# turpaultn/DCASE2019_task4

Measured on AMD Instinct MI355X. Metric: 10-s clips/sec mean-teacher train step (64-mel x 628), higher is better.
Workload: dtype f32

## Files before the change

dcase2019_task4_amd/csrc/common.h:

```cpp
#pragma once
#include <hip/hip_runtime.h>
#include <stdint.h>
#include <stddef.h>
#include "../../include/dcase_sed.h"

typedef __attribute__((ext_vector_type(16))) float f32x16;
typedef __attribute__((ext_vector_type(4))) float f32x4;

#define SED_C 64
#define SED_HID 64
#define SED_WAVE 64

void sed_set_error(const char* fmt, ...);
#define SED_CHECK_ARG(cond, msg)                                   \
    do {                                                           \
        if (!(cond)) {                                             \
            sed_set_error("%s:%d: %s", __FILE__, __LINE__, msg);   \
            return SED_ERR_BAD_ARG;                                \
        }                                                          \
    } while (0)
#define SED_CHECK_HIP(expr)                                                                 \
    do {                                                                                    \
        hipError_t _e = (expr);                                                             \
        if (_e != hipSuccess) {                                                             \
            sed_set_error("%s:%d: %s -> %s", __FILE__, __LINE__, #expr, hipGetErrorString(_e)); \
            return SED_ERR_LAUNCH;                                                          \
        }                                                                                   \
    } while (0)
#define SED_CHECK_LAUNCH() SED_CHECK_HIP(hipGetLastError())
struct SedAttrOnce {
    bool done[64] = {};
    bool need() {
        int d = 0;
        if (hipGetDevice(&d) != hipSuccess || d < 0 || d >= 64) return true;
        if (done[d]) return false;
        done[d] = true;
        return true;
    }
};
#define SED_TRY(expr)               \
    do {                            \
        int _s = (expr);            \
        if (_s != SED_OK) return _s; \
    } while (0)

struct Geo {
    int B, T, F, C, H, NC, L;
    int mode;
    bool f16;
    bool generic;
    int H1, W1;
    int H2, W2;
    int T3;
    float p, eps, mom;
};
static inline Geo make_geo(const sed_dims* d) {
    Geo g;
    g.B = d->B; g.T = d->T; g.F = d->F; g.C = d->C; g.H = d->H; g.NC = d->nclass; g.L = d->n_layers_rnn;
    g.f16 = d->dtype == SED_DTYPE_F16;
    g.mode = g.f16 ? SED_DTYPE_BF16 : d->dtype;
    g.generic = !(d->C == 64 && d->H == 64 && d->dtype == SED_DTYPE_F32);
    g.H1 = g.T / 2; g.W1 = g.F / 4;
    g.H2 = g.H1 / 2; g.W2 = g.W1 / 4;
    g.T3 = g.H2 / 2;
    g.p = d->p_drop; g.eps = d->bn_eps; g.mom = d->bn_momentum;
    return g;
}
int sed_validate_dims(const sed_dims* d);

struct ParamOff {
    int64_t conv_w[3], conv_b[3], bn_g[3], bn_b[3], glu_w[3], glu_b[3];
    int64_t w_ih[2][2], w_hh[2][2], b_ih[2][2], b_hh[2][2];
    int64_t dense_w, dense_b, soft_w, soft_b;
    int64_t total;
    int count;
};
ParamOff make_param_off(const Geo& g, int64_t* offsets_out );

struct CtxLayout {
    size_t acc0;
    size_t mom0, wz0, wl0, bn0;
    size_t mompart;
    size_t wpkT1, wpkT2;
    size_t p0;
    size_t wpk1, y1, stat1, bn1, p1;
    size_t wpk2, y2, stat2, bn2, p2;
    size_t gates[2], out[2];
    size_t logits_s, strong_sv, weak_sv, den_sv;
    size_t mask0, mask1, mask2;
    size_t total;
};
CtxLayout make_ctx_layout(const Geo& g);

struct WsLayout {
    size_t d_out, dgi[2], dgh[2], hprev[2], d_in, heads_part;
    size_t dz2, dp1, dz1, dp0, dp2;
    size_t bwd_acc;
    size_t bnb, gluacc1, gluacc2, coef[3], wg_part, de0, gemm_part;
    size_t total;
    int wgrad_blocks;
};
WsLayout make_ws_layout(const Geo& g);
#define SED_WGRAD_MAX_BLOCKS 256
#ifndef SED_GRU_SPLITK
#define SED_GRU_SPLITK 16
#endif
#define SED_GLUACC_N 4296
#define SED_WINO_OFF (9 * 4096)

__device__ __forceinline__ float wave_sum(float v) {
#pragma unroll
    for (int o = 32; o > 0; o >>= 1) v += __shfl_xor(v, o);
    return v;
}
__device__ __forceinline__ float wave_max(float v) {
#pragma unroll
    for (int o = 32; o > 0; o >>= 1) v = fmaxf(v, __shfl_xor(v, o));
    return v;
}
__device__ __forceinline__ void lds_barrier() { asm volatile("s_waitcnt lgkmcnt(0)\n\ts_barrier" ::: "memory"); }
__device__ __forceinline__ float rcp_fast(float x) { return __builtin_amdgcn_rcpf(x); }
__device__ __forceinline__ float sigmoidf_fast(float x) { return rcp_fast(1.0f + __expf(-x)); }
#define SED_NEG_LOG2E (-1.4426950408889634f)
__device__ __forceinline__ float sigmoid_from_scaled(float e) { return rcp_fast(1.0f + __builtin_amdgcn_exp2f(e)); }
struct TileWalk { int first, end, step; };
__device__ __forceinline__ TileWalk xcd_walk(int n_tiles) {
    const int w = blockIdx.x, g = (int)gridDim.x;
#ifndef SED_NO_XCD_ORDER
    if ((g & 7) == 0) {
        const int chunk = (n_tiles + 7) >> 3, lo = (w & 7) * chunk, hi = lo + chunk < n_tiles ? lo + chunk : n_tiles;
        return {lo + (w >> 3), hi, g >> 3};
    }
#endif
    return {w, n_tiles, g};
}
extern int g_sed_debug;

__device__ __forceinline__ f32x16 mfma32(float a, float b, f32x16 c) {
    return __builtin_amdgcn_mfma_f32_32x32x2f32(a, b, c, 0, 0, 0);
}
__device__ __forceinline__ int mfma32_row(int r, int lane) { return (r & 3) + 8 * (r >> 2) + 4 * (lane >> 5); }


#ifdef SED_TS
#define SED_TS_DEFINE(tag)                                                                                          \
    static __device__ unsigned long long g_ts[1024 * 16];                                                           \
    extern "C" int sed_debug_ts_##tag(unsigned long long* out, int n) {                                             \
        return (int)hipMemcpyFromSymbol(out, HIP_SYMBOL(g_ts), sizeof(unsigned long long) * (n < 1024 * 16 ? n : 1024 * 16)); \
    }
#define TS(k) do { if (threadIdx.x == 0 && blockIdx.x < 1024 && blockIdx.y == 0) g_ts[blockIdx.x * 16 + (k)] = wall_clock64(); } while (0)
#define TSC(k) do { if (threadIdx.x == 0 && blockIdx.x < 1024 && blockIdx.y == 0) g_ts[blockIdx.x * 16 + (k)] = clock64(); } while (0)
#else
#define SED_TS_DEFINE(tag)
#define TS(k) do { } while (0)
#define TSC(k) do { } while (0)
#endif
```

dcase2019_task4_amd/csrc/conv.hip:

```cpp
#include <type_traits>
#include "common.h"
#include "kernels.h"
SED_TS_DEFINE(conv)

template <int TW>
struct ConvCfg {
    static constexpr int TH = 128 / TW;
    static constexpr int HW = TW + 2;
    static constexpr int HH = TH + 2;
    static constexpr int PS = 65;
    static constexpr int RS = HW * PS + (((TW - HW * PS) % 32) + 32) % 32;
    static constexpr int HALO_FLOATS = HH * RS;
    static constexpr int W_FLOATS = 64 * 64;
    static constexpr size_t LDS_BYTES = (size_t)(HALO_FLOATS + 2 * W_FLOATS) * 4;
};

__global__ __launch_bounds__(256) void k_conv_pack(ConvPackArgs a) { conv_pack_body(a, blockIdx.x * 256 + threadIdx.x); }

template <int TW, int MODE, int NS>
__global__ __launch_bounds__(256) void k_conv3x3(const float* __restrict__ in0, const float* __restrict__ in1,
                                                  const float* __restrict__ coef, const float* __restrict__ wpk,
                                                  const float* __restrict__ bias, float* __restrict__ out,
                                                  double* __restrict__ stat, int B, int H, int tiles_per_clip) {
    using Cfg = ConvCfg<TW>;
    constexpr int TH = Cfg::TH, HW = Cfg::HW, HH = Cfg::HH, PS = Cfg::PS, RS = Cfg::RS;
    extern __shared__ __attribute__((aligned(16))) float smem[];
    float* halo = smem;
    float* Ws = smem + Cfg::HALO_FLOATS;
    const int tid = threadIdx.x, lane = tid & 63, wv = tid >> 6;
    const int n = lane & 31, kh = lane >> 5;
    const int b = blockIdx.x / tiles_per_clip, y0 = (blockIdx.x % tiles_per_clip) * TH;
    const int W = TW;
    const int nh = (NS == 2) ? blockIdx.y : 0;

    for (int f = tid; f < HH * HW * 16; f += 256) {
        const int pix = f >> 4, c4 = (f & 15) * 4;
        const int hy = pix / HW, hx = pix % HW;
        const int iy = y0 - 1 + hy, ix = hx - 1;
        float4 v = make_float4(0.f, 0.f, 0.f, 0.f);
        if (iy >= 0 && iy < H && ix >= 0 && ix < W) {
            const size_t g = (((size_t)b * H + iy) * W + ix) * 64 + c4;
            v = *(const float4*)(in0 + g);
            if (MODE == 1) {
                const float4 yv = *(const float4*)(in1 + g);
                const float4 ca = *(const float4*)(coef + c4);
                const float4 cb = *(const float4*)(coef + 64 + c4);
                const float4 cc = *(const float4*)(coef + 128 + c4);
                v.x = ca.x * v.x + cb.x * yv.x + cc.x;
                v.y = ca.y * v.y + cb.y * yv.y + cc.y;
                v.z = ca.z * v.z + cb.z * yv.z + cc.z;
                v.w = ca.w * v.w + cb.w * yv.w + cc.w;
            }
        }
        float* dst = halo + hy * RS + hx * PS + c4;
        dst[0] = v.x; dst[1] = v.y; dst[2] = v.z; dst[3] = v.w;
    }
#pragma unroll
    for (int it = 0; it < 4; ++it) {
        const int f = tid + 256 * it;
        *(float4*)(Ws + f * 4) = *(const float4*)(wpk + f * 4);
    }
    __syncthreads();

    const int m = 32 * wv + n;
    const int ty = m / TW, tx = m % TW;
    const float* Ab = halo + (ty + 1) * RS + (tx + 1) * PS + kh;
    f32x16 acc0, acc1;
#pragma unroll
    for (int r = 0; r < 16; ++r) { acc0[r] = 0.f; acc1[r] = 0.f; }

    for (int tap = 0; tap < 9; ++tap) {
        float4 pre[4];
        if (tap < 8) {
#pragma unroll
            for (int it = 0; it < 4; ++it) pre[it] = *(const float4*)(wpk + (tap + 1) * 4096 + (tid + 256 * it) * 4);
        }
        const int dy = tap / 3 - 1, dx = tap % 3 - 1;
        const float* A = Ab + dy * RS + dx * PS;
        const float* Bw = Ws + (tap & 1) * 4096 + kh * 64 + n + 32 * nh;
#pragma unroll
        for (int s = 0; s < 32; ++s) {
            const float a = A[2 * s];
            const float b0 = Bw[2 * s * 64];
            acc0 = mfma32(a, b0, acc0);
            if (NS == 1) {
                const float b1 = Bw[2 * s * 64 + 32];
                acc1 = mfma32(a, b1, acc1);
            }
        }
        if (tap < 8) {
            float* Wn = Ws + ((tap + 1) & 1) * 4096;
#pragma unroll
            for (int it = 0; it < 4; ++it) *(float4*)(Wn + (tid + 256 * it) * 4) = pre[it];
        }
        lds_barrier();
    }

    float s1[2] = {0.f, 0.f}, s2[2] = {0.f, 0.f};
    const float bia0 = (MODE == 0) ? bias[32 * nh + n] : 0.f, bia1 = (MODE == 0 && NS == 1) ? bias[32 + n] : 0.f;
#pragma unroll
    for (int r = 0; r < 16; ++r) {
        const int mm = 32 * wv + mfma32_row(r, lane);
        const int yy = y0 + mm / TW, xx = mm % TW;
        if (yy < H) {
            const size_t g = (((size_t)b * H + yy) * W + xx) * 64;
            const float v0 = acc0[r] + bia0, v1 = acc1[r] + bia1;
            out[g + 32 * nh + n] = v0;
            if (NS == 1) out[g + 32 + n] = v1;
            if (MODE == 0) { s1[0] += v0; s2[0] += v0 * v0; s1[1] += v1; s2[1] += v1 * v1; }
        }
    }
    if (MODE == 0 && stat != nullptr) {
        float* red = smem;
#pragma unroll
        for (int h = 0; h < 2; ++h) {
            float a = s1[h] + __shfl_xor(s1[h], 32);
            float q = s2[h] + __shfl_xor(s2[h], 32);
            if (kh == 0) { red[(wv * 2 + 0) * 64 + 32 * h + n] = a; red[(wv * 2 + 1) * 64 + 32 * h + n] = q; }
        }
        __syncthreads();
        if (tid < 128) {
            const int which = tid >> 6, c = tid & 63;
            double v = 0;
#pragma unroll
            for (int w2 = 0; w2 < 4; ++w2) v += (double)red[(w2 * 2 + which) * 64 + c];
            if (NS == 1) atomicAdd(&stat[which * 64 + c], v);
            else if (c < 32) atomicAdd(&stat[which * 64 + 32 * nh + c], v);
        }
    }
}


typedef float f32x4_t __attribute__((ext_vector_type(4)));
struct Ws16 {
    static constexpr int TH = 8, TW = 16, HW = 18, HH = 10, PS = 66, RS = HW * PS;
    static constexpr int HALO_FLOATS = HH * RS;
    static constexpr size_t LDS_BYTES = (size_t)2 * HALO_FLOATS * 4;
};
struct Ws16x2 {
    static constexpr int NLD = (Ws16::HH * Ws16::HW * 16 + 511) / 512;
};
template <int MODE>
__global__ __launch_bounds__(512, 1) void k_conv16_ws2(const float* __restrict__ in0, const float* __restrict__ in1,
                                                       const float* __restrict__ coef, const float* __restrict__ wpk,
                                                       const float* __restrict__ bias, float* __restrict__ out,
                                                       double* __restrict__ stat, int H, int tiles_per_clip, int n_tiles) {
    using C = Ws16;
    constexpr int NLD = Ws16x2::NLD;
    extern __shared__ __attribute__((aligned(16))) float smem[];
    const int tid = threadIdx.x, lane = tid & 63, wave = tid >> 6;
    const int cg = wave & 3, rh = wave >> 2;
    const int p16 = lane & 15, kq = lane >> 4;
    float st1 = 0.f, st2 = 0.f;
    constexpr int NH = (MODE == 1) ? NLD / 2 : NLD;
    f32x4_t pre0[NH], pre1[MODE == 1 ? NH : 1];
// ... 717 lines not shown
            Vd[(4 * i2 + 3) * 64] = T[i2][1] - T[i2][3];
        }
    };
    auto transform_m = [&](int y0, int ks, int slot, float* Ms) {
        float dy[4];
#pragma unroll
        for (int q = 0; q < 4; ++q) {
            const float v = fmaf(ca, dzr[slot][q], fmaf(cb, yr[slot][q], cc));
            dy[q] = v * ((y0 + 2 * (C::br_ks(ks) + cg_br) + (q >> 1) < H) ? 1.f : 0.f);
        }
        const float R[4][2] = {{dy[0], dy[1]}, {dy[0] + dy[2], dy[1] + dy[3]}, {dy[0] - dy[2], dy[1] - dy[3]}, {-dy[2], -dy[3]}};
        float* Md = Ms + cg * C::SM + 4 * (lane & 15) + (lane >> 4);
#pragma unroll
        for (int i2 = 0; i2 < 4; ++i2) {
            Md[(4 * i2 + 0) * 64] = R[i2][0];
            Md[(4 * i2 + 1) * 64] = R[i2][0] + R[i2][1];
            Md[(4 * i2 + 2) * 64] = R[i2][0] - R[i2][1];
            Md[(4 * i2 + 3) * 64] = -R[i2][1];
        }
    };
    auto mma = [&](const float* Vs, const float* Ms) {
        const float* Ab = Ms + kq * C::SM + 4 * i16 + 256 * (1 + ph);
        const float* Bb = Vs + kq * C::SV + 16 * cg + i16 + 256 * (1 + ph);
        const int xo = ph ? 256 : -256;
#pragma unroll
        for (int p8 = 0; p8 < 8; ++p8) {
            const int po = (p8 < 4 ? xo : 0) + (p8 & 3) * 64;
            const f32x4_t a4 = *(const f32x4_t*)(Ab + po);
            const float bv = Bb[po];
#pragma unroll
            for (int m = 0; m < 4; ++m) acc[p8][m] = __builtin_amdgcn_mfma_f32_16x16x4f32(a4[m], bv, acc[p8][m], 0, 0, 0);
        }
    };
    const TileWalk walk = xcd_walk(n_tiles);
    int tile = walk.first;
    TS(0);
    int it_ts = 0;
    int tb = tile / tiles_per_clip, ty0 = (tile % tiles_per_clip) * C::TH;
    if (tile < walk.end) {
        f32x4_t first[NITEMS];
#pragma unroll
        for (int hy = 0; hy < NITEMS; ++hy) load_row(tb, ty0, hy, first[hy]);
        if (ph) { load_dy(tb, ty0, 0, 0); load_dy(tb, ty0, 1, 1); }
#pragma unroll
        for (int hy = 0; hy < NITEMS; ++hy) store_row(smem, ty0, hy, first[hy]);
    }
    __syncthreads();
    if (tile < walk.end) {
        if (ph == 0) transform_v(smem, 0, ops);
        else transform_m(ty0, 0, 0, ops + 4 * C::SV);
    }
    __syncthreads();
    TS(1);
#pragma unroll
    for (int p8 = 0; p8 < 8; ++p8)
#pragma unroll
        for (int m = 0; m < 4; ++m) acc[p8][m] = (f32x4_t){0.f, 0.f, 0.f, 0.f};
    int cur = 0;
    for (; tile < walk.end; tile += walk.step) {
        const int nxt = (tile + walk.step < walk.end) ? tile + walk.step : tile;
        const int nb_ = nxt / tiles_per_clip, ny0 = (nxt % tiles_per_clip) * C::TH;
        const float* halo = smem + cur * C::HALO_FLOATS;
        float* halo_nxt = smem + (cur ^ 1) * C::HALO_FLOATS;
        constexpr int NKS = C::NKS, NPIECE = (NITEMS + NH - 1) / NH;
#pragma unroll
        for (int ks = 0; ks < NKS; ++ks) {
            f32x4_t held[NH];
            if (ks >= 1 && ks <= NPIECE) {
#pragma unroll
                for (int k2 = 0; k2 < NH; ++k2) held[k2] = pre[k2];
            }
            if (ks < NPIECE) {
#pragma unroll
                for (int k2 = 0; k2 < NH; ++k2)
                    if (NH * ks + k2 < NITEMS) load_row(nb_, ny0, NH * ks + k2, pre[k2]);
            }
            float* nb = ops + ((ks + 1) & 1) * C::OPS_FLOATS;
            const float* cb2 = ops + (ks & 1) * C::OPS_FLOATS;
            if (ph == 0) {
                if (ks < NKS - 1) transform_v(halo, ks + 1, nb); else transform_v(halo_nxt, 0, nb);
            }
            if (it_ts == 0 && ks == 2) { TS(3); TSW4(7); }
            mma(cb2, cb2 + 4 * C::SV);
            if (it_ts == 0 && ks == 2) { TS(4); TSW4(8); }
            if (ph == 1) {
                if (ks < NKS - 2) load_dy(tb, ty0, ks + 2, ks & 1); else load_dy(nb_, ny0, ks - (NKS - 2), ks & 1);
                if (ks < NKS - 1) transform_m(ty0, ks + 1, (ks + 1) & 1, nb + 4 * C::SV); else transform_m(ny0, 0, 0, nb + 4 * C::SV);
            }
            if (ks >= 1 && ks <= NPIECE) {
#pragma unroll
                for (int k2 = 0; k2 < NH; ++k2)
                    if (NH * (ks - 1) + k2 < NITEMS) store_row(halo_nxt, ny0, NH * (ks - 1) + k2, held[k2]);
            }
            if (it_ts == 0 && ks == 2) { TS(5); TSW4(9); }
            lds_barrier();
            if (it_ts == 0 && ks == 1) { TS(2); TSW4(6); }
        }
        if (it_ts == 0) TS(10);
        ++it_ts;
        cur ^= 1;
        tb = nb_; ty0 = ny0;
    }
    TS(11);
    __syncthreads();
    float* ob = smem;
#pragma unroll
    for (int round = 0; round < 2; ++round) {
        if (ph == round) {
#pragma unroll
            for (int m = 0; m < 4; ++m)
#pragma unroll
                for (int r = 0; r < 4; ++r) {
                    float wx[3], wy[3];
                    {
                        const float u0 = acc[0][m][r], u1 = acc[1][m][r], u2 = acc[2][m][r], u3 = acc[3][m][r];
                        const float h = 0.5f * (u1 + u2);
                        wx[0] = u0 + h; wx[1] = 0.5f * (u1 - u2); wx[2] = h + u3;
                    }
                    {
                        const float u0 = acc[4][m][r], u1 = acc[5][m][r], u2 = acc[6][m][r], u3 = acc[7][m][r];
                        const float h = 0.5f * (u1 + u2);
                        wy[0] = 0.5f * (u0 + h); wy[1] = 0.25f * (u1 - u2); wy[2] = 0.5f * (h + u3);
                    }
                    float* o = ob + (16 * m + 4 * kq + r) * C::OUT_STRIDE + 16 * cg + i16;
#pragma unroll
                    for (int b2 = 0; b2 < 3; ++b2) {
                        const float g0 = ph ? wy[b2] : wx[b2] + wy[b2];
                        const float g1 = ph ? -wy[b2] : wy[b2];
                        const float g2 = ph ? wx[b2] + wy[b2] : wy[b2];
                        if (round == 0) {
                            o[(0 + b2) * 64 * C::OUT_STRIDE] = g0; o[(3 + b2) * 64 * C::OUT_STRIDE] = g1; o[(6 + b2) * 64 * C::OUT_STRIDE] = g2;
                        } else {
                            o[(0 + b2) * 64 * C::OUT_STRIDE] += g0; o[(3 + b2) * 64 * C::OUT_STRIDE] += g1; o[(6 + b2) * 64 * C::OUT_STRIDE] += g2;
                        }
                    }
                }
        }
        __syncthreads();
    }
    TS(12);
    float* dst = part + (size_t)blockIdx.x * 9 * 4096;
    for (int idx = tid; idx < 9 * 64 * 16; idx += 512) {
        const int row = idx >> 4, c4 = (idx & 15) * 4;
        *(f32x4_t*)(dst + row * 64 + c4) = *(const f32x4_t*)(ob + row * C::OUT_STRIDE + c4);
    }
    TS(13);
}

#define WG4_RUNS 64
struct Wg4Os {
    static constexpr int SV4 = 4 * 64 + 16, SM4 = 4 * 64, OPS4 = 4 * SV4 + 4 * SM4;
    static constexpr size_t LDS_BYTES = (size_t)(2 * WgW<4>::HALO_FLOATS + 2 * OPS4) * 4;
};
__global__ __launch_bounds__(512, 1) void k_wgrad4_os(const float* __restrict__ dz, const float* __restrict__ yin,
                                                       const float* __restrict__ coef, const float* __restrict__ xin,
                                                       float* __restrict__ part, int H, int tiles_per_clip, int n_tiles, int n_runs,
                                                       BnBwdPrepArgs prep) {
    using C = WgW<4>;
    constexpr int SV4 = Wg4Os::SV4, SM4 = Wg4Os::SM4, OPS4 = Wg4Os::OPS4;
    extern __shared__ __attribute__((aligned(16))) float smem[];
    float* ops = smem + 2 * C::HALO_FLOATS;
    const int tid = threadIdx.x, lane = tid & 63, wave = __builtin_amdgcn_readfirstlane(tid >> 6);
    const int cg = wave & 3, jh = wave >> 2;
    const int w = blockIdx.x, run = (w & 7) + 8 * (w >> 5), ti = (w >> 3) & 3;
    const int cg_br = cg >> 1, cg_bc = cg & 1;
    const int i16 = lane & 15, kq = lane >> 4;
    const int vp = (ti == 0) ? 0 : (ti == 2 ? 2 : 1), vq = (ti == 3) ? 3 : (ti == 2 ? 1 : 2);
    const float sv = (ti == 1) ? 1.f : -1.f;
    const float ma = (ti == 3) ? 0.f : 1.f, mb = (ti == 0) ? 0.f : (ti == 1 ? 1.f : -1.f);
    float ca, cb, cc;
    if (prep.acc != nullptr) bn_bwd_coef(prep, lane, ca, cb, cc);
    else { ca = coef[lane]; cb = coef[64 + lane]; cc = coef[128 + lane]; }
    constexpr int NITEMS = C::NITEMS, NH = 2;
    f32x4_t pre[NH];
    const int td = tid < C::RPI * C::RW ? tid : tid - 480;
    const int r_in = td / C::RW, hx = (td % C::RW) >> 4, c4 = (td & 15) * 4;
    const int ixc = hx - 1 < 0 ? 0 : (hx - 1 > C::TW - 1 ? C::TW - 1 : hx - 1);
    const uint32_t goff4 = (uint32_t)(ixc * 64 + c4) * 4u;
    const bool colok = hx >= 1 && hx <= C::TW;
    const int lds_off = hx * C::PS + c4;
    auto load_row = [&](int b, int y0, int it, f32x4_t& d0) {
        const int hy = it * C::RPI + r_in < C::HH ? it * C::RPI + r_in : C::HH - 1;
        const int iy = y0 - 1 + hy;
        const int iyc = iy < 0 ? 0 : (iy > H - 1 ? H - 1 : iy);
        const float* rowp = xin + (size_t)(b * H + iyc) * (C::TW * 64);
        d0 = *(const f32x4_t*)((const char*)rowp + goff4);
    };
    auto store_row = [&](float* halo, int y0, int it, const f32x4_t& s0) {
        const int hy = it * C::RPI + r_in < C::HH ? it * C::RPI + r_in : C::HH - 1;
        const int iy = y0 - 1 + hy;
        const bool ok = colok && iy >= 0 && iy < H;
        const f32x4_t z4 = {0.f, 0.f, 0.f, 0.f};
        const f32x4_t v = ok ? s0 : z4;
        float* d = halo + hy * C::RS + lds_off;
        *(float2*)d = make_float2(v[0], v[1]);
        *(float2*)(d + 2) = make_float2(v[2], v[3]);
    };
    f32x4_t acc[2][4];
    float dzr[2][4], yr[2][4];
    const int img_bytes = (n_tiles / tiles_per_clip) * H * (C::TW * 64 * 4);
    const auto rs_dz = __builtin_amdgcn_make_buffer_rsrc((void*)dz, (short)0, img_bytes, 0x00020000);
    const auto rs_y = __builtin_amdgcn_make_buffer_rsrc((void*)yin, (short)0, img_bytes, 0x00020000);
    const int lane4 = 4 * lane;
    auto load_dy = [&](int b, int y0, int ks, int slot) {
#pragma unroll
        for (int q = 0; q < 4; ++q) {
            const int yy = y0 + 2 * (C::br_ks(ks) + cg_br) + (q >> 1), xx = 2 * (C::bc_ks(ks) + cg_bc) + (q & 1);
            const int yc = yy < H ? yy : H - 1;
            const int so = ((b * H + yc) * C::TW + xx) * 256;
            dzr[slot][q] = __uint_as_float(__builtin_amdgcn_raw_buffer_load_b32(rs_dz, lane4, so, 0));
            yr[slot][q] = __uint_as_float(__builtin_amdgcn_raw_buffer_load_b32(rs_y, lane4, so, 0));
        }
    };
    auto transform_v = [&](const float* halo, int ks, float* Vs) {
        const float* P = halo + (2 * cg_br) * C::RS + (2 * cg_bc) * C::PS + lane + ((2 * C::br_ks(ks)) * C::RS + (2 * C::bc_ks(ks)) * C::PS);
        const float* Pp = P + vp * C::RS;
        const float* Pq = P + vq * C::RS;
        float T[4];
#pragma unroll
        for (int b2 = 0; b2 < 4; ++b2) T[b2] = fmaf(sv, Pq[b2 * C::PS], Pp[b2 * C::PS]);
        float* Vd = Vs + cg * SV4 + lane;
        Vd[0] = T[0] - T[2]; Vd[64] = T[1] + T[2]; Vd[128] = T[2] - T[1]; Vd[192] = T[1] - T[3];
    };
    auto transform_m = [&](int y0, int ks, int slot, float* Ms) {
        float dy[4];
#pragma unroll
        for (int q = 0; q < 4; ++q) {
            const float v = fmaf(ca, dzr[slot][q], fmaf(cb, yr[slot][q], cc));
            dy[q] = v * ((y0 + 2 * (C::br_ks(ks) + cg_br) + (q >> 1) < H) ? 1.f : 0.f);
        }
        const float R0 = ma * dy[0] + mb * dy[2], R1 = ma * dy[1] + mb * dy[3];
        float* Md = Ms + cg * SM4 + 4 * (lane & 15) + (lane >> 4);
        Md[0] = R0; Md[64] = R0 + R1; Md[128] = R0 - R1; Md[192] = -R1;
    };
    auto mma = [&](const float* Vs, const float* Ms) {
        const float* Ab = Ms + kq * SM4 + 4 * i16 + 128 * jh;
        const float* Bb = Vs + kq * SV4 + 16 * cg + i16 + 128 * jh;
#pragma unroll
        for (int j2 = 0; j2 < 2; ++j2) {
            const f32x4_t a4 = *(const f32x4_t*)(Ab + 64 * j2);
            const float bv = Bb[64 * j2];
#pragma unroll
            for (int m = 0; m < 4; ++m) acc[j2][m] = __builtin_amdgcn_mfma_f32_16x16x4f32(a4[m], bv, acc[j2][m], 0, 0, 0);
        }
    };
    int tile = run;
    int tb = tile / tiles_per_clip, ty0 = (tile % tiles_per_clip) * C::TH;
    if (tile < n_tiles) {
        f32x4_t first[NITEMS];
#pragma unroll
        for (int hy = 0; hy < NITEMS; ++hy) load_row(tb, ty0, hy, first[hy]);
        if (jh) { load_dy(tb, ty0, 0, 0); load_dy(tb, ty0, 1, 1); }
#pragma unroll
        for (int hy = 0; hy < NITEMS; ++hy) store_row(smem, ty0, hy, first[hy]);
    }
    __syncthreads();
    if (tile < n_tiles) {
        if (jh == 0) transform_v(smem, 0, ops);
        else transform_m(ty0, 0, 0, ops + 4 * SV4);
    }
    __syncthreads();
#pragma unroll
    for (int j2 = 0; j2 < 2; ++j2)
#pragma unroll
        for (int m = 0; m < 4; ++m) acc[j2][m] = (f32x4_t){0.f, 0.f, 0.f, 0.f};
    int cur = 0;
    for (; tile < n_tiles; tile += n_runs) {
        const int nxt = (tile + n_runs < n_tiles) ? tile + n_runs : tile;
        const int nb_ = nxt / tiles_per_clip, ny0 = (nxt % tiles_per_clip) * C::TH;
        const float* halo = smem + cur * C::HALO_FLOATS;
        float* halo_nxt = smem + (cur ^ 1) * C::HALO_FLOATS;
        constexpr int NKS = C::NKS, NPIECE = (NITEMS + NH - 1) / NH;
#pragma unroll
        for (int ks = 0; ks < NKS; ++ks) {
            f32x4_t held[NH];
            if (ks >= 1 && ks <= NPIECE) {
#pragma unroll
                for (int k2 = 0; k2 < NH; ++k2) held[k2] = pre[k2];
            }
            if (ks < NPIECE) {
#pragma unroll
                for (int k2 = 0; k2 < NH; ++k2)
                    if (NH * ks + k2 < NITEMS) load_row(nb_, ny0, NH * ks + k2, pre[k2]);
            }
            float* nb = ops + ((ks + 1) & 1) * OPS4;
            const float* cb2 = ops + (ks & 1) * OPS4;
            if (jh == 0) {
                if (ks < NKS - 1) transform_v(halo, ks + 1, nb); else transform_v(halo_nxt, 0, nb);
            }
            mma(cb2, cb2 + 4 * SV4);
            if (jh == 1) {
                if (ks < NKS - 2) load_dy(tb, ty0, ks + 2, ks & 1); else load_dy(nb_, ny0, ks - (NKS - 2), ks & 1);
                if (ks < NKS - 1) transform_m(ty0, ks + 1, (ks + 1) & 1, nb + 4 * SV4); else transform_m(ny0, 0, 0, nb + 4 * SV4);
            }
            if (ks >= 1 && ks <= NPIECE) {
#pragma unroll
                for (int k2 = 0; k2 < NH; ++k2)
                    if (NH * (ks - 1) + k2 < NITEMS) store_row(halo_nxt, ny0, NH * (ks - 1) + k2, held[k2]);
            }
            lds_barrier();
        }
        cur ^= 1;
        tb = nb_; ty0 = ny0;
    }
    __syncthreads();
    float* xb = smem + (size_t)cg * 48 * 64 + lane;
    if (jh == 1) {
#pragma unroll
        for (int m = 0; m < 4; ++m)
#pragma unroll
            for (int r = 0; r < 4; ++r) {
                const float u2 = acc[0][m][r], u3 = acc[1][m][r];
                xb[((m * 4 + r) * 3 + 0) * 64] = 0.5f * u2;
                xb[((m * 4 + r) * 3 + 1) * 64] = -0.5f * u2;
                xb[((m * 4 + r) * 3 + 2) * 64] = 0.5f * u2 + u3;
            }
    }
    __syncthreads();
    if (jh == 0) {
        float* dst = part + ((size_t)run * 4 + ti) * 3 * 4096 + 16 * cg + i16;
#pragma unroll
        for (int m = 0; m < 4; ++m)
#pragma unroll
            for (int r = 0; r < 4; ++r) {
                const float u0 = acc[0][m][r], u1 = acc[1][m][r];
                const int co = 16 * m + 4 * kq + r;
                dst[(0 * 64 + co) * 64] = (u0 + 0.5f * u1) + xb[((m * 4 + r) * 3 + 0) * 64];
                dst[(1 * 64 + co) * 64] = 0.5f * u1 + xb[((m * 4 + r) * 3 + 1) * 64];
                dst[(2 * 64 + co) * 64] = 0.5f * u1 + xb[((m * 4 + r) * 3 + 2) * 64];
            }
    }
}

__global__ __launch_bounds__(256) void k_wgrad4_os_reduce(const float* __restrict__ part, int n_runs, float* __restrict__ g_w) {
    __shared__ __attribute__((aligned(16))) float red[16][12][64];
    __shared__ float S[12][64];
    const int c = threadIdx.x & 15, grp = threadIdx.x >> 4;
    const f32x4_t* P = (const f32x4_t*)part + blockIdx.x * 16 + c;
    f32x4_t s[12];
#pragma unroll
    for (int pl = 0; pl < 12; ++pl) s[pl] = (f32x4_t){0.f, 0.f, 0.f, 0.f};
    for (int r = grp; r < n_runs; r += 16) {
#pragma unroll
        for (int pl = 0; pl < 12; ++pl) s[pl] += P[((size_t)r * 12 + pl) * 1024];
    }
#pragma unroll
    for (int pl = 0; pl < 12; ++pl) *(f32x4_t*)&red[grp][pl][4 * c] = s[pl];
    __syncthreads();
    for (int o = threadIdx.x; o < 12 * 64; o += 256) {
        const int pl = o >> 6, e = o & 63;
        float v = 0.f;
#pragma unroll
        for (int g2 = 0; g2 < 16; ++g2) v += red[g2][pl][e];
        S[pl][e] = v;
    }
    __syncthreads();
    for (int o = threadIdx.x; o < 64 * 9; o += 256) {
        const int e = o / 9, tap = o % 9, a = tap / 3, b = tap % 3;
        const float w0 = S[0 + b][e], w1 = S[3 + b][e], w2 = S[6 + b][e], w3 = S[9 + b][e];
        const float v = a == 0 ? w0 + 0.5f * (w1 + w2) : (a == 1 ? 0.5f * (w1 - w2) : 0.5f * (w1 + w2) + w3);
        g_w[(size_t)blockIdx.x * 64 * 9 + o] = v;
    }
}

__global__ __launch_bounds__(256) void k_wgrad_reduce(const float* __restrict__ part, int n_blocks, float* __restrict__ g_w) {
    __shared__ __attribute__((aligned(16))) float red[16][64];
    const int c = threadIdx.x & 15, grp = threadIdx.x >> 4;
    const int i4 = blockIdx.x * 16 + c;
    const f32x4_t* P = (const f32x4_t*)part + i4;
    constexpr int SLAB4 = 9 * 4096 / 4;
    f32x4_t s[8];
#pragma unroll
    for (int u = 0; u < 8; ++u) s[u] = (f32x4_t){0.f, 0.f, 0.f, 0.f};
    int k = grp;
    for (; k + 16 * 7 < n_blocks; k += 16 * 8) {
#pragma unroll
        for (int u = 0; u < 8; ++u) s[u] += P[(size_t)(k + 16 * u) * SLAB4];
    }
    for (; k < n_blocks; k += 16) s[0] += P[(size_t)k * SLAB4];
    *(f32x4_t*)&red[grp][4 * c] = ((s[0] + s[1]) + (s[2] + s[3])) + ((s[4] + s[5]) + (s[6] + s[7]));
    __syncthreads();
    if (threadIdx.x < 64) {
        float v = 0.f;
#pragma unroll
        for (int g2 = 0; g2 < 16; ++g2) v += red[g2][threadIdx.x];
        const int i = blockIdx.x * 64 + threadIdx.x;
        const int tap = i / 4096, co = (i / 64) % 64, ci = i % 64;
        g_w[(co * 64 + ci) * 9 + tap] = v;
    }
}

int launch_conv_pack(const ConvPackArgs& a, hipStream_t st) {
    k_conv_pack<<<SED_PACK_BLOCKS, 256, 0, st>>>(a);
    SED_CHECK_LAUNCH();
    return SED_OK;
}

template <int TW, int MODE, int NS>
static int conv_launch_t(const float* in0, const float* in1, const float* coef, const float* wpk, const float* bias,
                         float* out, double* stat, int B, int H, hipStream_t st) {
    using Cfg = ConvCfg<TW>;
    static thread_local SedAttrOnce attr_done;
    if (attr_done.need()) {
        SED_CHECK_HIP(hipFuncSetAttribute((const void*)k_conv3x3<TW, MODE, NS>, hipFuncAttributeMaxDynamicSharedMemorySize,
                                          (int)Cfg::LDS_BYTES));
    }
    const int tpc = (H + Cfg::TH - 1) / Cfg::TH;
    k_conv3x3<TW, MODE, NS><<<dim3(B * tpc, NS), 256, Cfg::LDS_BYTES, st>>>(in0, in1, coef, wpk, bias, out, stat, B, H, tpc);
    SED_CHECK_LAUNCH();
    return SED_OK;
}

#ifdef SED_AB
#define SED_AB_FLAGS(mask) (g_sed_debug & (mask))
#else
#define SED_AB_FLAGS(mask) 0
#endif
extern "C" int sed_build_flags(void) {
#ifdef SED_AB
    return 1;
#else
    return 0;
#endif
}

int launch_conv_fwd(const float* in, const float* wpk, const float* bias, float* y, double* stat, int zero_stat, int B,
                    int H, int W, hipStream_t st) {
    if (stat && zero_stat) SED_CHECK_HIP(hipMemsetAsync(stat, 0, 128 * sizeof(double), st));
#ifdef SED_AB
    const bool direct = (g_sed_debug & (2 | 64)) != 0;
    if (direct && W == 16) return (g_sed_debug & 2) ? conv_launch_t<16, 0, 1>(in, nullptr, nullptr, wpk, bias, y, stat, B, H, st)
                                                    : conv16_ws_launch<0>(in, nullptr, nullptr, wpk, bias, y, stat, B, H, st);
    if (direct && W == 4) return conv_launch_t<4, 0, 2>(in, nullptr, nullptr, wpk, bias, y, stat, B, H, st);
#endif
    if (W == 16) return conv_wino_launch<16, 0>(in, nullptr, nullptr, wpk, bias, y, stat, B, H, nullptr, st);
    if (W == 4) return conv_wino_launch<4, 0>(in, nullptr, nullptr, wpk, bias, y, stat, B, H, nullptr, st);
    sed_set_error("conv: unsupported width %d", W);
    return SED_ERR_UNSUPPORTED;
}

int launch_conv_dgrad(const float* dz, const float* yin, const float* coef, const float* wpkT, float* dx, int B, int H,
                      int W, const BnBwdPrepArgs* prep, hipStream_t st) {
#ifdef SED_AB
    const bool direct = (g_sed_debug & (4 | 64)) != 0;
    SED_CHECK_ARG(!(direct && prep), "conv dgrad: in-kernel BatchNorm-backward coefficients need the Winograd kernel");
    if (direct && W == 16) return (g_sed_debug & 4) ? conv_launch_t<16, 1, 1>(dz, yin, coef, wpkT, nullptr, dx, nullptr, B, H, st)
                                                    : conv16_ws_launch<1>(dz, yin, coef, wpkT, nullptr, dx, nullptr, B, H, st);
    if (direct && W == 4) return conv_launch_t<4, 1, 2>(dz, yin, coef, wpkT, nullptr, dx, nullptr, B, H, st);
#endif
    if (W == 16) return conv_wino_launch<16, 1>(dz, yin, coef, wpkT, nullptr, dx, nullptr, B, H, prep, st);
    if (W == 4) return conv_wino_launch<4, 1>(dz, yin, coef, wpkT, nullptr, dx, nullptr, B, H, prep, st);
    sed_set_error("conv dgrad: unsupported width %d", W);
    return SED_ERR_UNSUPPORTED;
}

template <int TW, int TS>
static int wgrad_launch_t(const float* dz, const float* yin, const float* coef, const float* xin, float* part,
                          int n_blocks, float* g_w, int B, int H, const BnBwdPrepArgs* prep, hipStream_t st) {
    BnBwdPrepArgs pa = {};
    if (prep) pa = *prep;
#ifdef SED_AB
    using Cfg = WgCfg<TW>;
    static thread_local SedAttrOnce attr_done;
    if (attr_done.need()) {
        SED_CHECK_HIP(hipFuncSetAttribute((const void*)k_conv3x3_wgrad<TW, TS>, hipFuncAttributeMaxDynamicSharedMemorySize,
                                          (int)Cfg::LDS_BYTES));
    }
    const int tpc = (H + Cfg::TH - 1) / Cfg::TH, nt = B * tpc;
    int nb = nt < n_blocks ? nt : n_blocks;
#else
    int nb = 0;
#endif
    if (TW == 4 && !SED_AB_FLAGS(8 | 128) && !(g_sed_debug & 67108864)) {
        using CW = WgW<4>;
        static thread_local SedAttrOnce attro;
        if (attro.need()) {
            SED_CHECK_HIP(hipFuncSetAttribute((const void*)k_wgrad4_os, hipFuncAttributeMaxDynamicSharedMemorySize, (int)Wg4Os::LDS_BYTES));
        }
        SED_CHECK_ARG((size_t)B * H * TW * 64 < ((size_t)1 << 31), "wgrad: image too large for 32-bit offsets");
        const int tpcw = (H + CW::TH - 1) / CW::TH, ntw = B * tpcw;
        int n_runs = (ntw + 7) & ~7;
        if (n_runs > WG4_RUNS) n_runs = WG4_RUNS;
        SED_CHECK_ARG(n_runs * 4 <= n_blocks * 3, "wgrad: partial buffer too small");
        k_wgrad4_os<<<4 * n_runs, 512, Wg4Os::LDS_BYTES, st>>>(dz, yin, coef, xin, part, H, tpcw, ntw, n_runs, pa);
        SED_CHECK_LAUNCH();
        k_wgrad4_os_reduce<<<4096 / 64, 256, 0, st>>>(part, n_runs, g_w);
        SED_CHECK_LAUNCH();
        return SED_OK;
    }
    if (!SED_AB_FLAGS(8 | 128)) {
        using CW = WgW<TW>;
        static thread_local SedAttrOnce attrw;
        if (attrw.need()) {
            SED_CHECK_HIP(hipFuncSetAttribute((const void*)k_wgrad_wino<TW>, hipFuncAttributeMaxDynamicSharedMemorySize, (int)CW::LDS_BYTES));
        }
        SED_CHECK_ARG((size_t)B * H * TW * 64 < ((size_t)1 << 31), "wgrad: image too large for 32-bit offsets");
        const int tpcw = (H + CW::TH - 1) / CW::TH, ntw = B * tpcw;
        nb = ntw < n_blocks ? ntw : n_blocks;
        k_wgrad_wino<TW><<<nb, 512, CW::LDS_BYTES, st>>>(dz, yin, coef, xin, part, H, tpcw, ntw, pa);
    }
#ifdef SED_AB
    else if (TW == 16 && TS == 1 && !(g_sed_debug & 8)) {
        static thread_local SedAttrOnce attr16;
        if (attr16.need()) {
            SED_CHECK_HIP(hipFuncSetAttribute((const void*)k_wgrad16_db, hipFuncAttributeMaxDynamicSharedMemorySize, (int)Wg16::LDS_BYTES));
        }
        k_wgrad16_db<<<nb, 256, Wg16::LDS_BYTES, st>>>(dz, yin, coef, xin, part, H, tpc, nt);
    } else {
        k_conv3x3_wgrad<TW, TS><<<dim3(nb, TS), 256, Cfg::LDS_BYTES, st>>>(dz, yin, coef, xin, part, B, H, tpc, nt, pa);
    }
#endif
    SED_CHECK_LAUNCH();
    k_wgrad_reduce<<<9 * 4096 / 64, 256, 0, st>>>(part, nb, g_w);
    SED_CHECK_LAUNCH();
    return SED_OK;
}

int launch_conv_wgrad(const float* dz, const float* yin, const float* coef, const float* xin, float* part, int n_blocks,
                      float* g_w, int B, int H, int W, const BnBwdPrepArgs* prep, hipStream_t st) {
    SED_CHECK_ARG(!(prep && W == 16 && SED_AB_FLAGS(8 | 128)), "conv wgrad: in-kernel BatchNorm-backward coefficients need the default kernels");
    if (W == 16) return wgrad_launch_t<16, 1>(dz, yin, coef, xin, part, n_blocks, g_w, B, H, prep, st);
    if (W == 4) return wgrad_launch_t<4, 3>(dz, yin, coef, xin, part, n_blocks, g_w, B, H, prep, st);
    sed_set_error("conv wgrad: unsupported width %d", W);
    return SED_ERR_UNSUPPORTED;
}
```

dcase2019_task4_amd/csrc/crnn.hip:

```cpp
#include <stdarg.h>
#include <map>
#include <mutex>
#include <utility>
#include <stdio.h>
#include <string.h>
#include "common.h"
#include "kernels.h"
#include "gkernels.h"

static thread_local char g_err[512] = "";
void sed_set_error(const char* fmt, ...) {
    va_list ap;
    va_start(ap, fmt);
    vsnprintf(g_err, sizeof(g_err), fmt, ap);
    va_end(ap);
}
extern "C" const char* sed_last_error(void) { return g_err; }
extern "C" int sed_version(void) { return 100; }
int g_sed_debug = 0;
extern "C" int sed_debug_set(int flags) { const int old = g_sed_debug; g_sed_debug = flags; return old; }

int sed_validate_dims(const sed_dims* d) {
    SED_CHECK_ARG(d != nullptr, "null dims");
    if (d->F != 64 || (d->C != 64 && d->C != 128) || (d->H != 64 && d->H != 256) ||
        (d->dtype != SED_DTYPE_F32 && d->dtype != SED_DTYPE_BF16 && d->dtype != SED_DTYPE_BF16X3 && d->dtype != SED_DTYPE_F16)) {
        sed_set_error("supported: F = 64, C in {64, 128}, H in {64, 256}, dtype in {f32, bf16, bf16x3, f16} (got F=%d C=%d H=%d dtype=%d)",
                      d->F, d->C, d->H, d->dtype);
        return SED_ERR_UNSUPPORTED;
    }
    SED_CHECK_ARG(d->B >= 1 && d->T >= 16, "need B >= 1 and T >= 16");
    SED_CHECK_ARG(d->nclass >= 1 && d->nclass <= 16, "nclass must be in [1, 16]");
    SED_CHECK_ARG(d->n_layers_rnn == 1 || d->n_layers_rnn == 2, "n_layers_rnn must be 1 or 2");
    SED_CHECK_ARG(d->p_drop >= 0.f && d->p_drop < 1.f, "p_drop must be in [0, 1)");
    SED_CHECK_ARG((int64_t)d->B * d->T * d->F * d->C < (1ll << 31), "batch too large for 32-bit pixel indices");
    return SED_OK;
}

ParamOff make_param_off(const Geo& g, int64_t* out) {
    ParamOff P;
    int64_t o = 0;
    int k = 0;
    auto put = [&](int64_t& field, int64_t n) {
        field = o;
        if (out) out[k] = o;
        ++k;
        o += n;
    };
    for (int i = 0; i < 3; ++i) {
        const int cin = (i == 0) ? 1 : g.C;
        put(P.conv_w[i], (int64_t)g.C * cin * 9);
        put(P.conv_b[i], g.C);
        put(P.bn_g[i], g.C);
        put(P.bn_b[i], g.C);
        put(P.glu_w[i], (int64_t)g.C * g.C);
        put(P.glu_b[i], g.C);
    }
    for (int l = 0; l < g.L; ++l) {
        const int nin = (l == 0) ? g.C : 2 * g.H;
        for (int dir = 0; dir < 2; ++dir) {
            put(P.w_ih[l][dir], (int64_t)3 * g.H * nin);
            put(P.w_hh[l][dir], (int64_t)3 * g.H * g.H);
            put(P.b_ih[l][dir], 3 * g.H);
            put(P.b_hh[l][dir], 3 * g.H);
        }
    }
    put(P.dense_w, (int64_t)g.NC * 2 * g.H);
    put(P.dense_b, g.NC);
    put(P.soft_w, (int64_t)g.NC * 2 * g.H);
    put(P.soft_b, g.NC);
    P.total = o;
    P.count = k;
    if (out) out[k] = o;
    return P;
}

static inline size_t al(size_t x) { return (x + 255) & ~(size_t)255; }

CtxLayout make_ctx_layout(const Geo& g) {
    CtxLayout L;
    size_t o = 0;
    auto put = [&](size_t& f, size_t bytes) { f = o; o = al(o + bytes); };
    const size_t n0 = (size_t)g.B * g.H1 * g.W1 * 64, n1 = (size_t)g.B * g.H2 * g.W2 * 64, n2 = (size_t)g.B * g.T3 * 64;
    put(L.acc0, 320 * sizeof(double));
    L.mom0 = L.acc0; L.stat1 = L.acc0 + 64 * sizeof(double); L.stat2 = L.acc0 + 192 * sizeof(double);
    put(L.wz0, 64 * 12 * 4); put(L.wl0, 64 * 12 * 4); put(L.bn0, 256 * 4);
    put(L.mompart, (size_t)x_moments_parts(g) * 54 * sizeof(double));
    put(L.p0, n0 * 4);
    put(L.wpk1, (9 + 16) * 4096 * 4); put(L.wpkT1, (9 + 16) * 4096 * 4); put(L.y1, n0 * 4); put(L.bn1, 256 * 4); put(L.p1, n1 * 4);
    put(L.wpk2, (9 + 16) * 4096 * 4); put(L.wpkT2, (9 + 16) * 4096 * 4); put(L.y2, n1 * 4); put(L.bn2, 256 * 4); put(L.p2, n2 * 4);
    const size_t bt = (size_t)g.B * g.T3;
    for (int l = 0; l < 2; ++l) {
        put(L.gates[l], bt * 512 * 4); put(L.out[l], bt * 128 * 4);
    }
    put(L.logits_s, bt * g.NC * 4); put(L.strong_sv, bt * g.NC * 4);
    put(L.weak_sv, (size_t)g.B * g.NC * 4); put(L.den_sv, (size_t)g.B * g.NC * 4);
    auto mask_bytes = [](size_t Q) { return ((Q + 3) / 4) * 2 * 64 * sizeof(uint16_t); };
    put(L.mask0, mask_bytes((size_t)g.B * g.H1 * g.W1)); put(L.mask1, mask_bytes((size_t)g.B * g.H2 * g.W2));
    put(L.mask2, mask_bytes((size_t)g.B * g.T3));
    L.total = o;
    return L;
}

WsLayout make_ws_layout(const Geo& g) {
    WsLayout W;
    size_t o = 0;
    auto put = [&](size_t& f, size_t bytes) { f = o; o = al(o + bytes); };
    const size_t n0 = (size_t)g.B * g.H1 * g.W1 * 64, n1 = (size_t)g.B * g.H2 * g.W2 * 64, bt = (size_t)g.B * g.T3;
    put(W.d_out, bt * 128 * 4);
    for (int l = 0; l < 2; ++l) { put(W.dgi[l], bt * 384 * 4); put(W.dgh[l], bt * 384 * 4); put(W.hprev[l], bt * 128 * 4); }
    put(W.d_in, 2 * bt * 128 * 4); put(W.heads_part, (size_t)g.B * 2 * (g.NC * 128 + g.NC) * 4);
    put(W.dp2, 2 * bt * 64 * 4); put(W.dz2, n1 * 4); put(W.dp1, n1 * 4); put(W.dz1, n0 * 4); put(W.dp0, n0 * 4);
    put(W.bnb, 256 * sizeof(double)); W.coef[0] = 0; put(W.coef[1], 192 * 4); put(W.coef[2], 192 * 4);
    put(W.bwd_acc, (2 * SED_GLUACC_N + 2 * 64 * 10) * sizeof(double));
    W.gluacc1 = W.bwd_acc; W.gluacc2 = W.bwd_acc + SED_GLUACC_N * sizeof(double); W.de0 = W.bwd_acc + 2 * SED_GLUACC_N * sizeof(double);
    W.wgrad_blocks = SED_WGRAD_MAX_BLOCKS;
    put(W.wg_part, (size_t)W.wgrad_blocks * 9 * 4096 * 4);
    put(W.gemm_part, gemm_part_floats(4, SED_GRU_SPLITK, 192, 129) * 4);
    W.total = o;
    return W;
}

extern "C" int sed_param_count(const sed_dims* d) {
    if (sed_validate_dims(d) != SED_OK) return -1;
    const Geo g = make_geo(d);
    return make_param_off(g, nullptr).count;
}
extern "C" int sed_param_layout(const sed_dims* d, int64_t* offsets) {
    SED_TRY(sed_validate_dims(d));
    SED_CHECK_ARG(offsets != nullptr, "null offsets");
    const Geo g = make_geo(d);
    make_param_off(g, offsets);
    return SED_OK;
}
extern "C" size_t sed_crnn_ctx_bytes(const sed_dims* d) {
    if (sed_validate_dims(d) != SED_OK) return 0;
    const Geo g = make_geo(d);
    return g.generic ? gen_ctx_bytes(g) : make_ctx_layout(g).total;
}
extern "C" size_t sed_crnn_bwd_ws_bytes(const sed_dims* d) {
    if (sed_validate_dims(d) != SED_OK) return 0;
    const Geo g = make_geo(d);
    return g.generic ? gen_ws_bytes(g) : make_ws_layout(g).total;
}

extern "C" int sed_crnn_buffers_init(const sed_dims* d, void* ctx, size_t ctx_bytes, void* ws, size_t ws_bytes, void* stream) {
    SED_TRY(sed_validate_dims(d));
    const Geo g = make_geo(d);
    if (g.generic) return gen_buffers_init(g, ctx, ctx_bytes, ws, ws_bytes, (hipStream_t)stream);
    return SED_OK;
}

extern "C" int sed_crnn_ctx_view(const sed_dims* d, const char* name, size_t* offset, size_t* bytes) {
    SED_TRY(sed_validate_dims(d));
    SED_CHECK_ARG(name && offset && bytes, "null argument");
    const Geo g = make_geo(d);
    if (g.generic) return gen_ctx_view(g, name, offset, bytes);
    const CtxLayout L = make_ctx_layout(g);
    const size_t n0 = (size_t)g.B * g.H1 * g.W1 * 64 * 4, n1 = (size_t)g.B * g.H2 * g.W2 * 64 * 4, bt = (size_t)g.B * g.T3;
    struct { const char* n; size_t o, b; } tab[] = {
        {"mom0", L.mom0, 64 * 8}, {"wz0", L.wz0, 64 * 12 * 4}, {"wl0", L.wl0, 64 * 12 * 4}, {"bn0", L.bn0, 1024},
        {"p0", L.p0, n0}, {"y1", L.y1, n0}, {"stat1", L.stat1, 1024}, {"bn1", L.bn1, 1024}, {"p1", L.p1, n1},
        {"y2", L.y2, n1}, {"stat2", L.stat2, 1024}, {"bn2", L.bn2, 1024}, {"p2", L.p2, bt * 64 * 4},
        {"gates0", L.gates[0], bt * 512 * 4}, {"gates1", L.gates[1], bt * 512 * 4},
        {"gru0", L.out[0], bt * 128 * 4}, {"gru1", L.out[1], bt * 128 * 4},
        {"logits_s", L.logits_s, bt * g.NC * 4}, {"den", L.den_sv, (size_t)g.B * g.NC * 4},
    };
    for (auto& t : tab)
        if (strcmp(t.n, name) == 0) { *offset = t.o; *bytes = t.b; return SED_OK; }
    sed_set_error("sed_crnn_ctx_view: unknown buffer '%s'", name);
    return SED_ERR_BAD_ARG;
}

struct SideStream {
    hipStream_t s = nullptr;
    hipEvent_t fork = nullptr, join = nullptr;
    hipStream_t s2 = nullptr;
    hipEvent_t join2 = nullptr;
    bool ok = false;
};
static std::mutex g_side_mu;
static std::map<std::pair<int, hipStream_t>, SideStream*> g_side;
struct ForkHook { void (*fn)(void*) = nullptr; void* user = nullptr; };
static std::map<std::pair<int, hipStream_t>, ForkHook> g_fork_hooks;
static SideStream& side_stream(hipStream_t caller) {
    static SideStream none;
    int dev = 0;
    if (hipGetDevice(&dev) != hipSuccess) return none;
    std::lock_guard<std::mutex> lk(g_side_mu);
    SideStream*& slot = g_side[std::make_pair(dev, caller)];
    if (slot == nullptr) {
        slot = new SideStream();
        if (hipStreamCreateWithFlags(&slot->s, hipStreamNonBlocking) == hipSuccess &&
            hipEventCreateWithFlags(&slot->fork, hipEventDisableTiming) == hipSuccess &&
            hipEventCreateWithFlags(&slot->join, hipEventDisableTiming) == hipSuccess &&
            hipStreamCreateWithFlags(&slot->s2, hipStreamNonBlocking) == hipSuccess &&
            hipEventCreateWithFlags(&slot->join2, hipEventDisableTiming) == hipSuccess)
            slot->ok = true;
    }
    return *slot;
}
extern "C" int sed_stream_prepare(void* stream) {
    SideStream& sd = side_stream((hipStream_t)stream);
    if (!sd.ok) {
        sed_set_error("sed_stream_prepare: could not create the helper stream / events");
        return SED_ERR_LAUNCH;
    }
    return SED_OK;
}
extern "C" int sed_stream_release(void* stream) {
    int dev = 0;
    SED_CHECK_HIP(hipGetDevice(&dev));
    SideStream* sd = nullptr;
    {
        std::lock_guard<std::mutex> lk(g_side_mu);
        const auto key = std::make_pair(dev, (hipStream_t)stream);
        auto it = g_side.find(key);
        if (it != g_side.end()) { sd = it->second; g_side.erase(it); }
        g_fork_hooks.erase(key);
    }
    if (sd == nullptr) return SED_OK;
    int rc = SED_OK;
    auto note = [&](hipError_t e) { if (e != hipSuccess && rc == SED_OK) { sed_set_error("sed_stream_release: %s", hipGetErrorString(e)); rc = SED_ERR_LAUNCH; } };
    if (sd->s) { note(hipStreamSynchronize(sd->s)); note(hipStreamDestroy(sd->s)); }
    if (sd->s2) { note(hipStreamSynchronize(sd->s2)); note(hipStreamDestroy(sd->s2)); }
    if (sd->fork) note(hipEventDestroy(sd->fork));
    if (sd->join) note(hipEventDestroy(sd->join));
    if (sd->join2) note(hipEventDestroy(sd->join2));
    delete sd;
    return rc;
}
extern "C" int sed_crnn_fork_callback(void* stream, void (*fn)(void*), void* user) {
    int dev = 0;
    SED_CHECK_HIP(hipGetDevice(&dev));
    std::lock_guard<std::mutex> lk(g_side_mu);
    const auto key = std::make_pair(dev, (hipStream_t)stream);
    if (fn == nullptr) { g_fork_hooks.erase(key); return SED_OK; }
    ForkHook& h = g_fork_hooks[key];
    h.fn = fn;
    h.user = user;
    return SED_OK;
}
int sed_fork_point(hipStream_t st) {
    int dev = 0;
    if (hipGetDevice(&dev) != hipSuccess) return SED_OK;
    ForkHook h;
    {
        std::lock_guard<std::mutex> lk(g_side_mu);
        auto it = g_fork_hooks.find(std::make_pair(dev, st));
        if (it == g_fork_hooks.end()) return SED_OK;
        h = it->second;
        g_fork_hooks.erase(it);
    }
    if (h.fn) h.fn(h.user);
    return SED_OK;
}
#define SIDE_FORK(main_st)                                          \
    do {                                                            \
        SED_CHECK_HIP(hipEventRecord(sd.fork, (main_st)));          \
        SED_CHECK_HIP(hipStreamWaitEvent(sd.s, sd.fork, 0));        \
    } while (0)
#define SIDE_JOIN(main_st)                                          \
    do {                                                            \
        SED_CHECK_HIP(hipEventRecord(sd.join, sd.s));               \
        SED_CHECK_HIP(hipStreamWaitEvent((main_st), sd.join, 0));   \
    } while (0)

#define CTXF(off) ((float*)((char*)ctx + (off)))
#define CTXD(off) ((double*)((char*)ctx + (off)))
#define WSF(off) ((float*)((char*)ws + (off)))
#define WSD(off) ((double*)((char*)ws + (off)))
#define CTXM(off) ((uint16_t*)((char*)ctx + (off)))

extern "C" int sed_crnn_forward(const sed_dims* d, const float* params, float* bn_running, int64_t* bn_tracked,
                                const float* x, int train, int update_bn, const uint64_t* seed_dev, void* ctx,
                                size_t ctx_bytes, float* strong, float* weak, void* stream) {
    SED_TRY(sed_validate_dims(d));
    SED_CHECK_ARG(params && bn_running && x && ctx, "sed_crnn_forward: null argument");
    const int mom_ready = (train & 4) ? 1 : 0;
    train &= 3;
    SED_CHECK_ARG((strong && weak) || (!strong && !weak && train), "sed_crnn_forward: strong and weak must both be given (or both NULL in train mode: heads deferred)");
    const Geo g = make_geo(d);
    const ParamOff P = make_param_off(g, nullptr);
    if (g.generic) {
        SED_CHECK_ARG(!(train && g.p > 0.f) || seed_dev, "sed_crnn_forward: dropout enabled but seed_dev is null");
        hipStream_t st0 = (hipStream_t)stream;
        SideStream& sd0 = side_stream(st0);
        return gen_forward(g, P, params, bn_running, bn_tracked, x, train | (mom_ready ? 4 : 0), update_bn, seed_dev, ctx, ctx_bytes, strong,
                           weak, st0, sd0.ok ? sd0.s : st0, sd0.fork, sd0.join);
    }
    const CtxLayout L = make_ctx_layout(g);
    if (ctx_bytes < L.total) {
        sed_set_error("sed_crnn_forward: ctx has %zu bytes, needs %zu", ctx_bytes, L.total);
        return SED_ERR_WORKSPACE;
    }
    const int use_drop = (train && g.p > 0.f) ? 1 : 0;
    SED_CHECK_ARG(!use_drop || seed_dev, "sed_crnn_forward: dropout enabled but seed_dev is null");
    hipStream_t st = (hipStream_t)stream;
    const int upd = (train && update_bn) ? 1 : 0;
    int64_t* trk[3] = {bn_tracked ? bn_tracked + 0 : nullptr, bn_tracked ? bn_tracked + 1 : nullptr,
                       bn_tracked ? bn_tracked + 2 : nullptr};

    const ConvPackArgs pack = {params + P.conv_w[1], params + P.conv_w[2], CTXF(L.wpk1), CTXF(L.wpk2),
                               train ? CTXF(L.wpkT1) : nullptr, train ? CTXF(L.wpkT2) : nullptr, CTXD(L.stat1), train ? 256 : 0};
    SED_TRY(launch_blk0_forward(g, x, params + P.conv_w[0], params + P.conv_b[0], params + P.bn_g[0], params + P.bn_b[0],
                                params + P.glu_w[0], params + P.glu_b[0], bn_running + 0, bn_running + 64, trk[0], train,
                                upd, seed_dev, CTXD(L.mom0), CTXD(L.mompart), CTXF(L.wz0), CTXF(L.wl0), CTXF(L.bn0), CTXF(L.p0),
                                use_drop ? CTXM(L.mask0) : nullptr, train ? &pack : nullptr, st, 0, nullptr, nullptr, mom_ready));
    if (!train) SED_TRY(launch_conv_pack(pack, st));
    const float* in = CTXF(L.p0);
    const size_t wpk[3] = {0, L.wpk1, L.wpk2}, yo[3] = {0, L.y1, L.y2}, so[3] = {0, L.stat1, L.stat2},
                 bo[3] = {0, L.bn1, L.bn2}, po[3] = {0, L.p1, L.p2}, mo[3] = {L.mask0, L.mask1, L.mask2};
    const int Hs[3] = {0, g.H1, g.H2}, Ws[3] = {0, g.W1, g.W2};
    for (int i = 1; i <= 2; ++i) {
        SED_TRY(launch_conv_fwd(in, CTXF(wpk[i]), params + P.conv_b[i], CTXF(yo[i]), train ? CTXD(so[i]) : nullptr, 0, g.B,
                                Hs[i], Ws[i], st));
        SED_TRY(launch_glu_pool_fwd(CTXF(yo[i]), CTXD(so[i]), (double)g.B * Hs[i] * Ws[i], params + P.bn_g[i], params + P.bn_b[i],
                                    bn_running + (2 * i) * 64, bn_running + (2 * i + 1) * 64, trk[i], train, upd, g.eps, g.mom,
                                    CTXF(bo[i]), params + P.glu_w[i], params + P.glu_b[i], CTXF(po[i]), g.B, Hs[i], Ws[i], i,
                                    use_drop, g.p, seed_dev, use_drop ? CTXM(mo[i]) : nullptr, st));
        in = CTXF(po[i]);
    }
    SED_TRY(sed_fork_point(st));
    int nin = 64;
    for (int l = 0; l < g.L; ++l) {
        SED_TRY(launch_gru_fwd(in, nin, params + P.w_ih[l][0], params + P.w_ih[l][1], params + P.b_ih[l][0], params + P.b_ih[l][1],
                               params + P.w_hh[l][0], params + P.w_hh[l][1], params + P.b_hh[l][0], params + P.b_hh[l][1],
                               CTXF(L.out[l]), train ? CTXF(L.gates[l]) : nullptr, g.B, g.T3, st));
        in = CTXF(L.out[l]);
        nin = 128;
    }
    if (strong == nullptr) return SED_OK;
    SED_TRY(launch_heads_fwd(in, params + P.dense_w, params + P.dense_b, params + P.soft_w, params + P.soft_b, strong, weak,
                             train ? CTXF(L.strong_sv) : nullptr, train ? CTXF(L.weak_sv) : nullptr, CTXF(L.logits_s),
                             CTXF(L.den_sv), g.B, g.T3, g.NC, use_drop, g.p, seed_dev, st));
    return SED_OK;
}

extern "C" int sed_crnn_moments(const sed_dims* d, const float* x, void* ctx, size_t ctx_bytes, void* stream) {
    SED_TRY(sed_validate_dims(d));
    SED_CHECK_ARG(x && ctx, "sed_crnn_moments: null argument");
    const Geo g = make_geo(d);
    double* mompart = nullptr;
    if (g.generic) {
        SED_TRY(gen_mompart(g, ctx, ctx_bytes, &mompart));
    } else {
        const CtxLayout L = make_ctx_layout(g);
        if (ctx_bytes < L.total) {
            sed_set_error("sed_crnn_moments: ctx has %zu bytes, needs %zu", ctx_bytes, L.total);
            return SED_ERR_WORKSPACE;
        }
        mompart = CTXD(L.mompart);
    }
    return launch_x_moments(g, x, mompart, nullptr, (hipStream_t)stream);
}

static int crnn_backward_impl(const sed_dims* d, const float* params, const float* x, const uint64_t* seed_dev,
                              void* ctx, size_t ctx_bytes, const float* d_strong, const float* d_weak, float* grads,
                              void* ws, size_t ws_bytes, int parts, void* stream, const HeadsLoss* hl,
                              const HeadsOut* ho = nullptr) {
    SED_TRY(sed_validate_dims(d));
    SED_CHECK_ARG(params && x && ctx && (hl || (d_strong && d_weak)) && grads && ws, "sed_crnn_backward: null argument");
    SED_CHECK_ARG(parts == 1 || parts == 2 || parts == 3 || parts == 5 || parts == 8,
                  "sed_crnn_backward: parts must be 1, 2, 3, 5 or 8");
    const Geo g = make_geo(d);
    const ParamOff P = make_param_off(g, nullptr);
    if (g.generic) {
        SED_CHECK_ARG(!(g.p > 0.f) || seed_dev, "sed_crnn_backward: dropout enabled but seed_dev is null");
        hipStream_t st0 = (hipStream_t)stream;
        SideStream& sd0 = side_stream(st0);
        return gen_backward(g, P, params, x, seed_dev, ctx, ctx_bytes, d_strong, d_weak, grads, ws, ws_bytes, parts, st0,
                            (sd0.ok && !(g_sed_debug & 1073741824)) ? sd0.s : st0, sd0.fork, sd0.join, (sd0.ok && (g_sed_debug & 2048)) ? sd0.s2 : nullptr, sd0.join2, hl, ho);
    }
    const CtxLayout L = make_ctx_layout(g);
    const WsLayout W = make_ws_layout(g);
    if (ctx_bytes < L.total || ws_bytes < W.total) {
        sed_set_error("sed_crnn_backward: ctx %zu/%zu bytes, ws %zu/%zu bytes", ctx_bytes, L.total, ws_bytes, W.total);
        return SED_ERR_WORKSPACE;
    }
    const int use_drop = (g.p > 0.f) ? 1 : 0;
    SED_CHECK_ARG(!use_drop || seed_dev, "sed_crnn_backward: dropout enabled but seed_dev is null");
    hipStream_t st = (hipStream_t)stream;
    const int BT = g.B * g.T3;
    SideStream& sd = side_stream(st);
    hipStream_t ss = (sd.ok && !(g_sed_debug & 1073741824)) ? sd.s : st;
    const bool defer_gru_w = (parts & 4) != 0;
    bool forked = false, forked2 = false;

    auto gru_weight_grads_layer = [&](int l, hipStream_t s2) -> int {
        const int nin = (l == 0) ? 64 : 128;
        const float* input = (l == 0) ? CTXF(L.p2) : CTXF(L.out[l - 1]);
        GemmBatch gb;
        gb.n_prob = 4; gb.splits = SED_GRU_SPLITK; gb.part = WSF(W.gemm_part); gb.part_floats = gemm_part_floats(4, SED_GRU_SPLITK, 192, 129); gb.part_stride = 0;
        for (int dir = 0; dir < 2; ++dir) {
            gb.p[2 * dir] = gemm_prob(WSF(W.dgi[l]) + dir * 192, 1, 384, input, nin, 1, grads + P.w_ih[l][dir], nin, 192, nin, BT);
            gb.p[2 * dir].Cones = grads + P.b_ih[l][dir];
            gb.p[2 * dir + 1] = gemm_prob(WSF(W.dgh[l]) + dir * 192, 1, 384, WSF(W.hprev[l]) + dir * 64, 128, 1,
                                          grads + P.w_hh[l][dir], 64, 192, 64, BT);
            gb.p[2 * dir + 1].Cones = grads + P.b_hh[l][dir];
        }
        return launch_gemm_batch(gb, s2);
    };
    auto gru_weight_grads = [&](hipStream_t s2) -> int {
        for (int l = g.L - 1; l >= 0; --l) SED_TRY(gru_weight_grads_layer(l, s2));
        return SED_OK;
    };
    const bool early_gru_w = parts == 3 && sd.ok && (g_sed_debug & 16384);

    const int head_cols = 2 * (g.NC * 128 + g.NC);
    const bool fuse = ho && hl && (parts & 1) && heads_fusable(64, g.T3) && !(g_sed_debug & 16777216) && !hl->d_strong_out && !hl->d_weak_out;
    auto heads_colsum = [&](hipStream_t s2) -> int {
        if (fuse) return launch_heads_fin(WSF(W.heads_part), grads + P.dense_w, g.B, g.T3, g.NC, head_cols, *hl, s2);
        return launch_heads_colsum(WSF(W.heads_part), grads + P.dense_w, g.B, g.NC, s2);
    };
    const bool defer_colsum = ((parts & 2) && sd.ok) || defer_gru_w;
    if (parts & 1) {
    const float* h_last = CTXF(L.out[g.L - 1]);
    if (ho && !fuse)
        SED_TRY(launch_heads_fwd(h_last, params + P.dense_w, params + P.dense_b, params + P.soft_w, params + P.soft_b, ho->strong, ho->weak,
                                 CTXF(L.strong_sv), CTXF(L.weak_sv), CTXF(L.logits_s), CTXF(L.den_sv), g.B, g.T3, g.NC, use_drop, g.p,
                                 seed_dev, st));
    if (!fuse)
    SED_TRY(launch_heads_bwd(h_last, params + P.dense_w, params + P.soft_w, CTXF(L.strong_sv), CTXF(L.weak_sv),
                             CTXF(L.logits_s), CTXF(L.den_sv), d_strong, d_weak, WSF(W.d_out), WSF(W.heads_part),
                             grads + P.dense_w, grads + P.dense_b, grads + P.soft_w, grads + P.soft_b, g.B, g.T3, g.NC,
                             use_drop, g.p, seed_dev, (parts & 2) ? WSD(W.bwd_acc) : nullptr, 2 * SED_GLUACC_N + 2 * 64 * 10,
                             defer_colsum ? 1 : 0, hl, st));
    const float* d_cur = WSF(W.d_out);
    const float* d_cur2 = nullptr;
    for (int l = g.L - 1; l >= 0; --l) {
        const int nin = (l == 0) ? 64 : 128;
        float* d_in = (l == 0) ? WSF(W.dp2) : WSF(W.d_in);
        if (fuse && l == g.L - 1) {
            HeadsFuse hf = {};
            hf.wd = params + P.dense_w; hf.strong = ho->strong; hf.weak = ho->weak; hf.part = WSF(W.heads_part);
            hf.NC = g.NC; hf.use_drop = use_drop; hf.p_drop = g.p; hf.seed = seed_dev;
            hf.zero = (parts & 2) ? WSD(W.bwd_acc) : nullptr; hf.n_zero = (parts & 2) ? 2 * SED_GLUACC_N + 2 * 64 * 10 : 0;
            hf.hl = *hl;
            SED_TRY(launch_gru_bwd_heads(CTXF(L.out[l]), CTXF(L.gates[l]), params + P.w_hh[l][0], params + P.w_hh[l][1],
                                         params + P.w_ih[l][0], params + P.w_ih[l][1], nin, WSF(W.dgi[l]), WSF(W.dgh[l]),
                                         WSF(W.hprev[l]), d_in, g.B, g.T3, hf, st));
            if (!defer_colsum) SED_TRY(heads_colsum(st));
            else if (defer_gru_w) SED_TRY(launch_heads_fin(WSF(W.heads_part), grads + P.dense_w, g.B, g.T3, g.NC, 0, *hl, st));
        } else
        SED_TRY(launch_gru_bwd(d_cur, d_cur2, CTXF(L.out[l]), CTXF(L.gates[l]), params + P.w_hh[l][0], params + P.w_hh[l][1],
                               params + P.w_ih[l][0], params + P.w_ih[l][1], nin, WSF(W.dgi[l]), WSF(W.dgh[l]),
                               WSF(W.hprev[l]), d_in, g.B, g.T3, st));
        d_cur = d_in;
        d_cur2 = d_in + (size_t)BT * nin;
        if (early_gru_w) {
            SIDE_FORK(st);
            forked = true;
            if (l == g.L - 1) SED_TRY(heads_colsum(ss));
            SED_TRY(gru_weight_grads_layer(l, ss));
        }
    }
    }
    if (parts == 1) SED_TRY(gru_weight_grads(st));
    if (parts == 8) {
        SED_TRY(launch_heads_colsum(WSF(W.heads_part), grads + P.dense_w, g.B, g.NC, st));
        SED_TRY(gru_weight_grads(st));
        return SED_OK;
    }
    if (!(parts & 2)) {
        if (forked) SIDE_JOIN(st);
        return SED_OK;
    }
    const size_t wpkT[3] = {0, L.wpkT1, L.wpkT2}, yo[3] = {0, L.y1, L.y2}, bo[3] = {0, L.bn1, L.bn2};
    const size_t pin[3] = {0, L.p0, L.p1}, gacc[3] = {0, W.gluacc1, W.gluacc2}, mo[3] = {L.mask0, L.mask1, L.mask2};
    const size_t dzo[3] = {0, W.dz1, W.dz2}, dpo[3] = {W.dp0, W.dp1, W.dp2};
    const int Hs[3] = {0, g.H1, g.H2}, Wd[3] = {0, g.W1, g.W2};
    if (!(parts & 1)) SED_CHECK_HIP(hipMemsetAsync(WSD(W.bwd_acc), 0, (2 * SED_GLUACC_N + 2 * 64 * 10) * sizeof(double), st));
#ifdef SED_AB
    const bool fuse_prep = (g_sed_debug & (4 | 8 | 64 | 128 | 512)) == 0;
#else
    const bool fuse_prep = (g_sed_debug & 512) == 0;
#endif
    BnBwdPrepArgs prep[3] = {};
    for (int i = 2; i >= 1; --i) {
        const BnBwdPrepArgs* pp = fuse_prep ? &prep[i] : nullptr;
        SED_TRY(launch_glu_pool_bwd(CTXF(yo[i]), CTXF(bo[i]), params + P.glu_w[i], params + P.glu_b[i], WSF(dpo[i]),
                                    i == 2 ? WSF(dpo[i]) + (size_t)BT * 64 : nullptr,
                                    WSF(dzo[i]), WSD(gacc[i]), 0, g.B, Hs[i], Wd[i], i, use_drop, g.p, CTXM(mo[i]),
                                    params + P.bn_g[i], WSF(W.coef[i]), grads + P.bn_g[i], grads + P.bn_b[i],
                                    grads + P.glu_w[i], grads + P.glu_b[i], grads + P.conv_b[i], fuse_prep ? &prep[i] : nullptr, st));
        if (i == 2) {
            if (sd.ok) SED_CHECK_HIP(hipEventRecord(sd.fork, st));
            SED_TRY(launch_conv_dgrad(WSF(dzo[i]), CTXF(yo[i]), WSF(W.coef[i]), CTXF(wpkT[i]), WSF(dpo[i - 1]), g.B, Hs[i], Wd[i], pp, st));
            if (sd.ok) { SED_CHECK_HIP(hipStreamWaitEvent(sd.s, sd.fork, 0)); forked = true; }
            SED_TRY(launch_conv_wgrad(WSF(dzo[i]), CTXF(yo[i]), WSF(W.coef[i]), CTXF(pin[i]), WSF(W.wg_part), W.wgrad_blocks,
                                      grads + P.conv_w[i], g.B, Hs[i], Wd[i], pp, ss));
            if (parts == 3 && !early_gru_w) {
                hipStream_t sg = ss;
                if (sd.ok && (g_sed_debug & 2048)) {
                    SED_CHECK_HIP(hipStreamWaitEvent(sd.s2, sd.fork, 0));
                    sg = sd.s2;
                    forked2 = true;
                }
                if (sd.ok) SED_TRY(heads_colsum(sg));
                SED_TRY(gru_weight_grads(sg));
            }
        } else {
            if (sd.ok) { SIDE_FORK(st); forked = true; }
            SED_TRY(launch_conv_dgrad(WSF(dzo[i]), CTXF(yo[i]), WSF(W.coef[i]), CTXF(wpkT[i]), WSF(dpo[i - 1]), g.B, Hs[i], Wd[i], pp, st));
            SED_TRY(launch_conv_wgrad(WSF(dzo[i]), CTXF(yo[i]), WSF(W.coef[i]), CTXF(pin[i]), WSF(W.wg_part), W.wgrad_blocks,
                                      grads + P.conv_w[i], g.B, Hs[i], Wd[i], pp, ss));
        }
    }
    SED_TRY(launch_blk0_backward(g, x, params + P.conv_w[0], params + P.conv_b[0], params + P.bn_g[0], params + P.bn_b[0],
                                 params + P.glu_w[0], CTXM(L.mask0), CTXD(L.mom0), CTXF(L.wz0), CTXF(L.wl0), CTXF(L.bn0),
                                 WSF(W.dp0), WSD(W.de0), 0, grads + P.conv_w[0], grads + P.conv_b[0], grads + P.bn_g[0],
                                 grads + P.bn_b[0], grads + P.glu_w[0], grads + P.glu_b[0], st));
    if (forked) SIDE_JOIN(st);
    if (forked2) {
        SED_CHECK_HIP(hipEventRecord(sd.join2, sd.s2));
        SED_CHECK_HIP(hipStreamWaitEvent(st, sd.join2, 0));
    }
    return SED_OK;
}

extern "C" int sed_crnn_backward(const sed_dims* d, const float* params, const float* x, const uint64_t* seed_dev,
                                 void* ctx, size_t ctx_bytes, const float* d_strong, const float* d_weak, float* grads,
                                 void* ws, size_t ws_bytes, int parts, void* stream) {
    return crnn_backward_impl(d, params, x, seed_dev, ctx, ctx_bytes, d_strong, d_weak, grads, ws, ws_bytes, parts, stream, nullptr);
}

extern "C" int sed_mt_loss_backward(const sed_dims* d, const float* params, const float* x, const uint64_t* seed_dev,
                                    void* ctx, size_t ctx_bytes, const float* strong_ema, const float* weak_ema,
                                    const float* target, int weak_lo, int weak_hi, int strong_lo, int strong_hi,
                                    sed_step_state* state_dev, int advance_state, float* losses, float* d_strong,
                                    float* d_weak, float* grads, void* ws, size_t ws_bytes, int parts, void* stream) {
    SED_CHECK_ARG(d && strong_ema && weak_ema && target && state_dev && losses, "sed_mt_loss_backward: null argument");
    SED_CHECK_ARG(parts == 1 || parts == 3 || parts == 5, "sed_mt_loss_backward: parts must include the heads (1, 3 or 5)");
    SED_CHECK_ARG(weak_lo >= 0 && weak_hi <= d->B && weak_lo <= weak_hi && strong_lo >= 0 && strong_hi <= d->B &&
                      strong_lo <= strong_hi, "sed_mt_loss_backward: bad mask range");
    HeadsLoss hl = {strong_ema, weak_ema, target, weak_lo, weak_hi, strong_lo, strong_hi, state_dev, losses, d_strong, d_weak,
                    advance_state ? state_dev : nullptr};
    return crnn_backward_impl(d, params, x, seed_dev, ctx, ctx_bytes, nullptr, nullptr, grads, ws, ws_bytes, parts, stream, &hl);
}

extern "C" int sed_mt_step_backward(const sed_dims* d, const float* params, const float* x, const uint64_t* seed_dev,
                                    void* ctx, size_t ctx_bytes, float* strong, float* weak, const float* strong_ema,
                                    const float* weak_ema, const float* target, int weak_lo, int weak_hi, int strong_lo,
                                    int strong_hi, sed_step_state* state_dev, int advance_state, float* losses, float* d_strong,
                                    float* d_weak, float* grads, void* ws, size_t ws_bytes, int parts, void* stream) {
    SED_CHECK_ARG(d && strong && weak && strong_ema && weak_ema && target && state_dev && losses, "sed_mt_step_backward: null argument");
    SED_CHECK_ARG(parts == 1 || parts == 3 || parts == 5, "sed_mt_step_backward: parts must include the heads (1, 3 or 5)");
    SED_CHECK_ARG(weak_lo >= 0 && weak_hi <= d->B && weak_lo <= weak_hi && strong_lo >= 0 && strong_hi <= d->B &&
                      strong_lo <= strong_hi, "sed_mt_step_backward: bad mask range");
    HeadsLoss hl = {strong_ema, weak_ema, target, weak_lo, weak_hi, strong_lo, strong_hi, state_dev, losses, d_strong, d_weak,
                    advance_state ? state_dev : nullptr};
    HeadsOut ho = {strong, weak};
    return crnn_backward_impl(d, params, x, seed_dev, ctx, ctx_bytes, nullptr, nullptr, grads, ws, ws_bytes, parts, stream, &hl, &ho);
}

extern "C" int sed_kernel_replay(const char* name, const sed_dims* d, const float* params, const float* x,
                                 const uint64_t* seed_dev, void* ctx, size_t ctx_bytes, float* grads, void* ws,
                                 size_t ws_bytes, void* stream) {
    SED_TRY(sed_validate_dims(d));
    SED_CHECK_ARG(name && params && x && ctx && grads && ws, "sed_kernel_replay: null argument");
    const Geo g = make_geo(d);
    if (g.generic) {
        sed_set_error("sed_kernel_replay: only the C = 64 / H = 64 / fp32 kernel set is replayable");
        return SED_ERR_UNSUPPORTED;
    }
    const ParamOff P = make_param_off(g, nullptr);
    const CtxLayout L = make_ctx_layout(g);
    const WsLayout W = make_ws_layout(g);
    if (ctx_bytes < L.total || ws_bytes < W.total) {
        sed_set_error("sed_kernel_replay: buffers too small");
        return SED_ERR_WORKSPACE;
    }
    hipStream_t st = (hipStream_t)stream;
    const int use_drop = (g.p > 0.f) ? 1 : 0;
    const int BT = g.B * g.T3;
    const size_t wpk[3] = {0, L.wpk1, L.wpk2}, wpkT[3] = {0, L.wpkT1, L.wpkT2}, yo[3] = {0, L.y1, L.y2},
                 so[3] = {0, L.stat1, L.stat2}, bo[3] = {0, L.bn1, L.bn2}, po[3] = {L.p0, L.p1, L.p2},
                 mo[3] = {L.mask0, L.mask1, L.mask2};
    const size_t dzo[3] = {0, W.dz1, W.dz2}, dpo[3] = {W.dp0, W.dp1, W.dp2}, gacc[3] = {0, W.gluacc1, W.gluacc2};
    const int Hs[3] = {0, g.H1, g.H2}, Wd[3] = {0, g.W1, g.W2};
    auto is = [&](const char* n) { return strcmp(name, n) == 0; };
    if (is("x_moments")) return launch_x_moments(g, x, CTXD(L.mompart), nullptr, st);
    if (is("blk0_fwd")) {
        const int tpc = (g.H1 + 3) / 4;
        (void)tpc;
        return launch_blk0_forward(g, x, params + P.conv_w[0], params + P.conv_b[0], params + P.bn_g[0], params + P.bn_b[0],
                                   params + P.glu_w[0], params + P.glu_b[0], WSF(W.coef[1]), WSF(W.coef[1]) + 64, nullptr, 1, 0,
                                   seed_dev, CTXD(L.mom0), CTXD(L.mompart), CTXF(L.wz0), CTXF(L.wl0), CTXF(L.bn0), CTXF(L.p0),
                                   use_drop ? CTXM(L.mask0) : nullptr, nullptr, st, 1);
    }
    for (int i = 1; i <= 2; ++i) {
        char nm[32];
        snprintf(nm, sizeof nm, "conv%d_fwd", i);
        if (is(nm)) return launch_conv_fwd(CTXF(po[i - 1]), CTXF(wpk[i]), params + P.conv_b[i], CTXF(yo[i]), CTXD(so[i]), 1, g.B, Hs[i], Wd[i], st);
        snprintf(nm, sizeof nm, "glu%d_fwd", i);
        if (is(nm)) return launch_glu_pool_fwd(CTXF(yo[i]), CTXD(so[i]), (double)g.B * Hs[i] * Wd[i], params + P.bn_g[i], params + P.bn_b[i],
                                               WSF(W.coef[1]), WSF(W.coef[1]) + 64, nullptr, 1, 0, g.eps, g.mom, CTXF(bo[i]),
                                               params + P.glu_w[i], params + P.glu_b[i], CTXF(po[i]), g.B, Hs[i], Wd[i], i, use_drop,
                                               g.p, seed_dev, use_drop ? CTXM(mo[i]) : nullptr, st);
        snprintf(nm, sizeof nm, "glu%d_bwd", i);
        if (is(nm)) return launch_glu_pool_bwd(CTXF(yo[i]), CTXF(bo[i]), params + P.glu_w[i], params + P.glu_b[i], WSF(dpo[i]), i == 2 ? WSF(dpo[i]) + (size_t)BT * 64 : nullptr, WSF(dzo[i]), WSD(gacc[i]), 1, g.B, Hs[i], Wd[i], i, use_drop, g.p, CTXM(mo[i]),
                                               params + P.bn_g[i], WSF(W.coef[i]), grads + P.bn_g[i], grads + P.bn_b[i], grads + P.glu_w[i], grads + P.glu_b[i], grads + P.conv_b[i], nullptr, st);
        snprintf(nm, sizeof nm, "conv%d_wgrad", i);
        if (is(nm)) return launch_conv_wgrad(WSF(dzo[i]), CTXF(yo[i]), WSF(W.coef[i]), CTXF(po[i - 1]), WSF(W.wg_part), W.wgrad_blocks, grads + P.conv_w[i], g.B, Hs[i], Wd[i], nullptr, st);
        snprintf(nm, sizeof nm, "conv%d_dgrad", i);
        if (is(nm)) return launch_conv_dgrad(WSF(dzo[i]), CTXF(yo[i]), WSF(W.coef[i]), CTXF(wpkT[i]), WSF(dpo[i - 1]), g.B, Hs[i], Wd[i], nullptr, st);
    }
    for (int l = 0; l < g.L; ++l) {
        char nm[32];
        snprintf(nm, sizeof nm, "gru%d_fwd", l);
        if (is(nm)) return launch_gru_fwd(l == 0 ? CTXF(L.p2) : CTXF(L.out[l - 1]), l == 0 ? 64 : 128, params + P.w_ih[l][0], params + P.w_ih[l][1],
                                          params + P.b_ih[l][0], params + P.b_ih[l][1], params + P.w_hh[l][0], params + P.w_hh[l][1],
                                          params + P.b_hh[l][0], params + P.b_hh[l][1], CTXF(L.out[l]), CTXF(L.gates[l]), g.B, g.T3, st);
        snprintf(nm, sizeof nm, "gru%d_bwd", l);
        if (is(nm)) {
            const int nin = (l == 0) ? 64 : 128;
            const bool top = (l == g.L - 1);
            return launch_gru_bwd(top ? WSF(W.d_out) : WSF(W.d_in), top ? nullptr : WSF(W.d_in) + (size_t)BT * 128, CTXF(L.out[l]),
                                  CTXF(L.gates[l]), params + P.w_hh[l][0], params + P.w_hh[l][1], params + P.w_ih[l][0],
                                  params + P.w_ih[l][1], nin, WSF(W.dgi[l]), WSF(W.dgh[l]), WSF(W.hprev[l]),
                                  l == 0 ? WSF(W.dp2) : WSF(W.d_in), g.B, g.T3, st);
        }
    }
    if (is("heads_fwd"))
        return launch_heads_fwd(CTXF(L.out[g.L - 1]), params + P.dense_w, params + P.dense_b, params + P.soft_w, params + P.soft_b,
                                CTXF(L.strong_sv), CTXF(L.weak_sv), nullptr, nullptr, CTXF(L.logits_s), CTXF(L.den_sv), g.B, g.T3, g.NC,
                                use_drop, g.p, seed_dev, st);
    if (is("blk0_bwd"))
        return launch_blk0_backward(g, x, params + P.conv_w[0], params + P.conv_b[0], params + P.bn_g[0], params + P.bn_b[0],
                                    params + P.glu_w[0], CTXM(L.mask0), CTXD(L.mom0), CTXF(L.wz0), CTXF(L.wl0), CTXF(L.bn0), WSF(W.dp0),
                                    WSD(W.de0), 1, grads + P.conv_w[0], grads + P.conv_b[0], grads + P.bn_g[0], grads + P.bn_b[0],
                                    grads + P.glu_w[0], grads + P.glu_b[0], st);
    (void)BT;
    sed_set_error("sed_kernel_replay: unknown kernel '%s'", name);
    return SED_ERR_BAD_ARG;
}
```

dcase2019_task4_amd/csrc/gemm.hip:

```cpp
#include "common.h"
#include "kernels.h"
SED_TS_DEFINE(gemm)

#define GT_M 64
#define GT_N 64
#define GT_K 64

typedef __attribute__((ext_vector_type(8))) __bf16 gemm_bf16x8;
__device__ __forceinline__ int prob_nx(const GemmProb& p) { return p.N + (p.Cones ? 1 : 0); }

template <int BF>
__global__ __launch_bounds__(256) void k_gemm_batched(GemmBatch gb) {
    extern __shared__ __attribute__((aligned(16))) float gsm[];
    float* As = gsm;
    float* Bs = gsm + GT_M * (GT_K + 1);
    int bx = blockIdx.x, by = blockIdx.y, bz = blockIdx.z;
#ifndef SED_NO_XCD_ORDER
    {
        const int gx = gridDim.x, gy = gridDim.y, total = gx * gy * (int)gridDim.z;
        if ((total & 7) == 0) {
            const int lin = bx + gx * (by + gy * bz), l2 = (lin & 7) * (total >> 3) + (lin >> 3);
            bx = l2 % gx; by = (l2 / gx) % gy; bz = l2 / (gx * gy);
        }
    }
#endif
    const int pi = bz / gb.splits, split = bz % gb.splits;
    const GemmProb& d = gb.p[pi];
    const int Nx = prob_nx(d);
    const int m0 = by * GT_M, n0 = bx * GT_N;
    if (m0 >= d.M || n0 >= d.N) return;
    const int tid = threadIdx.x, lane = tid & 63, wv = tid >> 6;
    const int n = lane & 31, kh = lane >> 5;
    const int wm = wv >> 1, wn = wv & 1;
    const bool ones_here = d.Cones != nullptr && bx == 0;
    float rowsum = 0.f;
    int kbeg = 0, kend = d.K;
    if (gb.splits > 1) {
        const int chunk = ((d.K + gb.splits - 1) / gb.splits + GT_K - 1) / GT_K * GT_K;
        kbeg = split * chunk;
        kend = min(d.K, kbeg + chunk);
    }
    f32x16 acc;
#pragma unroll
    for (int r = 0; r < 16; ++r) acc[r] = 0.f;
    constexpr int NG = (GT_M * GT_K) / 256 / 4;
    int am[NG], ak[NG], bk[NG], bn[NG];
    const bool a_kc = (d.sAk == 1), b_nc = (d.sBn == 1);
#pragma unroll
    for (int it = 0; it < NG; ++it) {
        const int e4 = (tid + 256 * it) * 4;
        if (a_kc) { am[it] = e4 / GT_K; ak[it] = e4 % GT_K; } else { am[it] = e4 % GT_M; ak[it] = e4 / GT_M; }
        if (b_nc) { bk[it] = e4 / GT_N; bn[it] = e4 % GT_N; } else { bk[it] = e4 % GT_K; bn[it] = e4 / GT_K; }
    }
    float ra[NG][4], rb[NG][4];
    const bool interior = d.vec_ok && m0 + GT_M <= d.M && n0 + GT_N <= d.N;
    (void)Nx;
    auto load_tile = [&](int k0) {
        if (interior && k0 + GT_K <= kend && (d.B2 == nullptr || k0 >= d.k2 || k0 + GT_K <= d.k2)) {
            const float* bbase = (d.B2 != nullptr && k0 >= d.k2) ? d.B2 - (int64_t)d.k2 * d.sBk : d.B;
#pragma unroll
            for (int it = 0; it < NG; ++it) {
                const f32x4 va = *(const f32x4*)(d.A + (int64_t)(m0 + am[it]) * d.sAm + (int64_t)(k0 + ak[it]) * d.sAk);
                const f32x4 vb = *(const f32x4*)(bbase + (int64_t)(k0 + bk[it]) * d.sBk + (int64_t)(n0 + bn[it]) * d.sBn);
#pragma unroll
                for (int q = 0; q < 4; ++q) { ra[it][q] = va[q]; rb[it][q] = vb[q]; }
            }
            return;
        }
#pragma unroll
        for (int it = 0; it < NG; ++it) {
            {
                const int m = m0 + am[it], k = k0 + ak[it];
                const float* p = d.A + (int64_t)m * d.sAm + (int64_t)k * d.sAk;
                const bool full = a_kc ? (m < d.M && k + 3 < kend) : (m + 3 < d.M && k < kend);
                if (full && (((uintptr_t)p & 15) == 0)) {
                    const float4 v = *(const float4*)p;
                    ra[it][0] = v.x; ra[it][1] = v.y; ra[it][2] = v.z; ra[it][3] = v.w;
                } else {
#pragma unroll
                    for (int q = 0; q < 4; ++q) {
                        const int mm = a_kc ? m : m + q, kk = a_kc ? k + q : k;
                        ra[it][q] = (mm < d.M && kk < kend) ? d.A[(int64_t)mm * d.sAm + (int64_t)kk * d.sAk] : 0.f;
                    }
                }
            }
            {
                const int kk0 = k0 + bk[it], nn0 = n0 + bn[it];
                const bool two = d.B2 != nullptr;
                const float* base = (two && kk0 >= d.k2) ? d.B2 - (int64_t)d.k2 * d.sBk : d.B;
                const float* p = base + (int64_t)kk0 * d.sBk + (int64_t)nn0 * d.sBn;
                const bool same_src = !two || b_nc || (kk0 >= d.k2) == (kk0 + 3 >= d.k2);
                const bool full = same_src && (b_nc ? (kk0 < kend && nn0 + 3 < d.N) : (kk0 + 3 < kend && nn0 < d.N));
                if (full && (((uintptr_t)p & 15) == 0)) {
                    const float4 v = *(const float4*)p;
                    rb[it][0] = v.x; rb[it][1] = v.y; rb[it][2] = v.z; rb[it][3] = v.w;
                } else {
#pragma unroll
                    for (int q = 0; q < 4; ++q) {
                        const int kk = b_nc ? kk0 : kk0 + q, nn = b_nc ? nn0 + q : nn0;
                        float w = 0.f;
                        if (kk < kend) {
                            if (nn < d.N) {
                                w = (two && kk >= d.k2) ? d.B2[(int64_t)(kk - d.k2) * d.sBk + (int64_t)nn * d.sBn]
                                                        : d.B[(int64_t)kk * d.sBk + (int64_t)nn * d.sBn];
                            }
                        }
                        rb[it][q] = w;
                    }
                }
            }
        }
    };
    if (kbeg < kend) load_tile(kbeg);
    for (int k0 = kbeg; k0 < kend; k0 += GT_K) {
#pragma unroll
        for (int it = 0; it < NG; ++it)
#pragma unroll
            for (int q = 0; q < 4; ++q) {
                As[(a_kc ? am[it] : am[it] + q) * (GT_K + 1) + (a_kc ? ak[it] + q : ak[it])] = ra[it][q];
                Bs[(b_nc ? bk[it] : bk[it] + q) * (GT_N + 1) + (b_nc ? bn[it] + q : bn[it])] = rb[it][q];
            }
        lds_barrier();
        if (k0 + GT_K < kend) load_tile(k0 + GT_K);
        if (ones_here) {
            const float* ar = As + (tid >> 2) * (GT_K + 1) + 16 * (tid & 3);
#pragma unroll
            for (int kk = 0; kk < 16; ++kk) rowsum += ar[kk];
        }
        if constexpr (BF != 0) {
#pragma unroll
            for (int s = 0; s < GT_K / 16; ++s) {
                gemm_bf16x8 a, b, al, bl;
#pragma unroll
                for (int e = 0; e < 8; ++e) {
                    const float av = As[(32 * wm + n) * (GT_K + 1) + 16 * s + 8 * kh + e];
                    const float bv = Bs[(16 * s + 8 * kh + e) * (GT_N + 1) + 32 * wn + n];
                    a[e] = (__bf16)av;
                    b[e] = (__bf16)bv;
                    if constexpr (BF == 2) { al[e] = (__bf16)(av - (float)a[e]); bl[e] = (__bf16)(bv - (float)b[e]); }
                }
                acc = __builtin_amdgcn_mfma_f32_32x32x16_bf16(a, b, acc, 0, 0, 0);
                if constexpr (BF == 2) {
                    acc = __builtin_amdgcn_mfma_f32_32x32x16_bf16(a, bl, acc, 0, 0, 0);
                    acc = __builtin_amdgcn_mfma_f32_32x32x16_bf16(al, b, acc, 0, 0, 0);
                }
            }
        } else {
#pragma unroll
            for (int s = 0; s < GT_K / 2; ++s) {
                const float a = As[(32 * wm + n) * (GT_K + 1) + 2 * s + kh];
                const float b = Bs[(2 * s + kh) * (GT_N + 1) + 32 * wn + n];
                acc = mfma32(a, b, acc);
            }
        }
        lds_barrier();
    }
    if (ones_here) {
        rowsum += __shfl_xor(rowsum, 1);
        rowsum += __shfl_xor(rowsum, 2);
        const int row = m0 + (tid >> 2);
        if ((tid & 3) == 0 && row < d.M) {
            if (gb.splits > 1) gb.part[(size_t)bz * gb.part_stride + (size_t)row * Nx + d.N] = rowsum;
            else d.Cones[row] = rowsum;
        }
    }
    const int col = n0 + 32 * wn + n;
    if (col >= d.N) return;
    if (gb.splits > 1) {
        float* P = gb.part + ((size_t)bz * gb.part_stride);
#pragma unroll
        for (int r = 0; r < 16; ++r) {
            const int row = m0 + 32 * wm + mfma32_row(r, lane);
            if (row < d.M) P[(size_t)row * Nx + col] = acc[r];
        }
        return;
    }
#pragma unroll
    for (int r = 0; r < 16; ++r) {
        const int row = m0 + 32 * wm + mfma32_row(r, lane);
        if (row >= d.M) continue;
        float* c = d.C + (int64_t)row * d.ldc + col;
        float v = acc[r] + (d.bias ? d.bias[col] : 0.f);
        if (d.accumulate) v += *c;
        *c = v;
    }
}

#define GP_M 32
#define GP_N 64
#define GP_KMAX 384
__global__ __launch_bounds__(256) void k_gemm_panel(GemmBatch gb) {
    extern __shared__ __attribute__((aligned(16))) float gsm[];
    const GemmProb& d = gb.p[blockIdx.z];
    const int m0 = blockIdx.y * GP_M, n0 = blockIdx.x * GP_N;
    if (m0 >= d.M || n0 >= d.N) return;
    const int K = d.K, SA = K + 1;
    float* As = gsm;
    float* Bs = gsm + GP_M * SA;
    const int tid = threadIdx.x, lane = tid & 63, wv = tid >> 6;
    const int n = lane & 31, kh = lane >> 5;
    const bool a_kc = (d.sAk == 1), b_nc = (d.sBn == 1);
    constexpr int NGA = GP_M * GP_KMAX / 4 / 256, NGB = GP_KMAX * GP_N / 4 / 256;
    const int nga = GP_M * K / 4 / 256, ngb = K * GP_N / 4 / 256;
    f32x4 ra[NGA], rb[NGB];
    const f32x4 z4 = {0.f, 0.f, 0.f, 0.f};
    TS(0); TSC(14);
#pragma unroll
    for (int it = 0; it < NGA; ++it) {
        ra[it] = z4;
        if (it < nga) {
            int m = m0 + (a_kc ? (tid >> 3) : (tid & 7) * 4);
            const int k = a_kc ? ((tid & 7) + 8 * it) * 4 : (tid >> 3) + 32 * it;
            if (a_kc) m = min(m, d.M - 1); else m = min(m, d.M - 4);
            ra[it] = *(const f32x4*)(d.A + (int64_t)m * d.sAm + (int64_t)k * d.sAk);
        }
    }
#pragma unroll
    for (int it = 0; it < NGB; ++it) {
        rb[it] = z4;
        if (it < ngb) {
            const int k = b_nc ? (tid >> 4) + 16 * it : ((tid & 3) + 4 * it) * 4, nn = n0 + (b_nc ? (tid & 15) * 4 : (tid >> 2));
            const float* base = (d.B2 != nullptr && k >= d.k2) ? d.B2 - (int64_t)d.k2 * d.sBk : d.B;
            rb[it] = *(const f32x4*)(base + (int64_t)k * d.sBk + (int64_t)nn * d.sBn);
        }
    }
#pragma unroll
    for (int it = 0; it < NGA; ++it) {
        if (it < nga) {
            const int ml = a_kc ? (tid >> 3) : (tid & 7) * 4, k = a_kc ? ((tid & 7) + 8 * it) * 4 : (tid >> 3) + 32 * it;
#pragma unroll
            for (int q = 0; q < 4; ++q) As[(a_kc ? ml : ml + q) * SA + (a_kc ? k + q : k)] = ra[it][q];
        }
    }
#pragma unroll
    for (int it = 0; it < NGB; ++it) {
        if (it < ngb) {
            const int k = b_nc ? (tid >> 4) + 16 * it : ((tid & 3) + 4 * it) * 4, nl = b_nc ? (tid & 15) * 4 : (tid >> 2);
#pragma unroll
            for (int q = 0; q < 4; ++q) Bs[(b_nc ? k : k + q) * (GP_N + 1) + (b_nc ? nl + q : nl)] = rb[it][q];
        }
    }
    TS(1);
    __syncthreads();
    TS(2);
    const int sub = wv & 1, khalf = wv >> 1;
    f32x16 acc;
#pragma unroll
    for (int r = 0; r < 16; ++r) acc[r] = 0.f;
    {
        const int kb = khalf * (K / 2);
        const float* Ap = As + n * SA + kb + kh;
        const float* Bp = Bs + (kb + kh) * (GP_N + 1) + 32 * sub + n;
        const int steps = K / 4;
        for (int s8 = 0; s8 < steps; s8 += 8) {
            float av[8], bv[8];
#pragma unroll
            for (int u = 0; u < 8; ++u) { av[u] = Ap[2 * (s8 + u)]; bv[u] = Bp[2 * (s8 + u) * (GP_N + 1)]; }
#pragma unroll
            for (int u = 0; u < 8; ++u) acc = mfma32(av[u], bv[u], acc);
        }
    }
    TS(3);
    __syncthreads();
    float* red = gsm;
    if (khalf == 1) {
#pragma unroll
        for (int r = 0; r < 16; ++r) red[(sub * 32 + mfma32_row(r, lane)) * 33 + n] = acc[r];
    }
    __syncthreads();
    if (khalf == 0) {
        const int col = n0 + 32 * sub + n;
        if (col < d.N) {
            const float bias = d.bias ? d.bias[col] : 0.f;
#pragma unroll
            for (int r = 0; r < 16; ++r) {
                const int rl = mfma32_row(r, lane), row = m0 + rl;
                if (row < d.M) {
                    float* c = d.C + (int64_t)row * d.ldc + col;
                    float v = acc[r] + red[(sub * 32 + rl) * 33 + n] + bias;
                    if (d.accumulate) v += *c;
                    *c = v;
                }
            }
        }
    }
    TS(4); TSC(15);
}

__global__ __launch_bounds__(256) void k_gemm_reduce(GemmBatch gb) {
    const int pi = blockIdx.y;
    const GemmProb& d = gb.p[pi];
    const int Nx = prob_nx(d);
    const int i = blockIdx.x * blockDim.x + threadIdx.x;
    if (i >= d.M * Nx) return;
    const float* P = gb.part + (size_t)pi * gb.splits * gb.part_stride + i;
    float s0 = 0.f, s1 = 0.f, s2 = 0.f, s3 = 0.f;
    int z = 0;
    for (; z + 4 <= gb.splits; z += 4) {
        s0 += P[(size_t)(z + 0) * gb.part_stride];
        s1 += P[(size_t)(z + 1) * gb.part_stride];
        s2 += P[(size_t)(z + 2) * gb.part_stride];
        s3 += P[(size_t)(z + 3) * gb.part_stride];
    }
    for (; z < gb.splits; ++z) s0 += P[(size_t)z * gb.part_stride];
    float v = (s0 + s1) + (s2 + s3);
    const int row = i / Nx, col = i % Nx;
    if (col < d.N) {
        float* c = d.C + (int64_t)row * d.ldc + col;
        v += d.bias ? d.bias[col] : 0.f;
        if (d.accumulate) v += *c;
        *c = v;
    } else {
        d.Cones[row] = v;
    }
}

__global__ __launch_bounds__(256) void k_colsum(const float* __restrict__ A, int M, int N, int64_t lda, float* __restrict__ out) {
    __shared__ float red[4][64];
    const int c = threadIdx.x & 63, r = threadIdx.x >> 6;
    const int col = blockIdx.x * 64 + c;
    float s = 0.f;
    if (col < N)
        for (int m = r; m < M; m += 4) s += A[(int64_t)m * lda + col];
    red[r][c] = s;
    __syncthreads();
    if (r == 0 && col < N) out[col] = red[0][c] + red[1][c] + red[2][c] + red[3][c];
}

size_t gemm_part_floats(int n_prob, int splits, int max_m, int max_nx) {
    return (size_t)n_prob * splits * max_m * max_nx;
}

int launch_gemm_batch(GemmBatch& gb, hipStream_t st) {
    int maxM = 0, maxNx = 0;
    for (int i = 0; i < gb.n_prob; ++i) {
        const int nx = gb.p[i].N + (gb.p[i].Cones ? 1 : 0);
        maxM = gb.p[i].M > maxM ? gb.p[i].M : maxM;
        maxNx = nx > maxNx ? nx : maxNx;
    }
    if (gb.splits < 1) gb.splits = 1;
    bool panel = (gb.splits == 1) && !gb.bf16;
    int maxK = 0, maxN = 0;
    for (int i = 0; i < gb.n_prob; ++i) {
        const GemmProb& q = gb.p[i];
        const bool a_kc = (q.sAk == 1), b_nc = (q.sBn == 1);
        panel = panel && q.K <= GP_KMAX && (q.K % 32) == 0 && q.Cones == nullptr && (q.B2 == nullptr || (q.k2 % 4) == 0) &&
                (q.N % GP_N) == 0 && q.M >= 4 && (q.M % 4) == 0 &&
                (a_kc ? (q.sAm % 4) == 0 : (q.sAm == 1 && (q.sAk % 4) == 0)) &&
                (b_nc ? (q.sBk % 4) == 0 : (q.sBk == 1 && (q.sBn % 4) == 0)) &&
                ((uintptr_t)q.A % 16) == 0 && ((uintptr_t)q.B % 16) == 0 && (q.B2 == nullptr || ((uintptr_t)q.B2 % 16) == 0);
        maxK = q.K > maxK ? q.K : maxK;
        maxN = q.N > maxN ? q.N : maxN;
    }
    if (panel) {
        const size_t lds = (size_t)(GP_M * (maxK + 1) + maxK * (GP_N + 1)) * sizeof(float);
        static size_t lds_set = 0;
        if (lds > lds_set) {
            SED_CHECK_HIP(hipFuncSetAttribute((const void*)k_gemm_panel, hipFuncAttributeMaxDynamicSharedMemorySize, (int)lds));
            lds_set = lds;
        }
        dim3 grid((maxN + GP_N - 1) / GP_N, (maxM + GP_M - 1) / GP_M, gb.n_prob);
        k_gemm_panel<<<grid, 256, lds, st>>>(gb);
        SED_CHECK_LAUNCH();
        return SED_OK;
    }
    for (int i = 0; i < gb.n_prob; ++i) {
        GemmProb& q = gb.p[i];
        const bool a_kc = (q.sAk == 1), b_nc = (q.sBn == 1);
        q.vec_ok = (a_kc ? (q.sAm % 4) == 0 : (q.sAm == 1 && (q.sAk % 4) == 0)) &&
                   (b_nc ? (q.sBk % 4) == 0 : (q.sBk == 1 && (q.sBn % 4) == 0)) &&
                   ((uintptr_t)q.A % 16) == 0 && ((uintptr_t)q.B % 16) == 0 && (q.B2 == nullptr || ((uintptr_t)q.B2 % 16) == 0);
    }
    if (gb.splits > 1) {
        SED_CHECK_ARG(gb.part != nullptr, "split-K gemm needs a partial buffer");
        gb.part_stride = (size_t)maxM * maxNx;
        if ((size_t)gb.n_prob * gb.splits * gb.part_stride > gb.part_floats) {
            sed_set_error("split-K gemm: partial buffer holds %zu floats, the batch needs %zu", gb.part_floats,
                          (size_t)gb.n_prob * gb.splits * gb.part_stride);
            return SED_ERR_WORKSPACE;
        }
    }
    dim3 grid((maxN + GT_N - 1) / GT_N, (maxM + GT_M - 1) / GT_M, gb.n_prob * gb.splits);
    const size_t lds = (size_t)(GT_M * (GT_K + 1) + GT_K * (GT_N + 1)) * sizeof(float);
    static thread_local SedAttrOnce attr_done;
    if (attr_done.need()) {
        SED_CHECK_HIP(hipFuncSetAttribute((const void*)k_gemm_batched<0>, hipFuncAttributeMaxDynamicSharedMemorySize, (int)lds));
        SED_CHECK_HIP(hipFuncSetAttribute((const void*)k_gemm_batched<1>, hipFuncAttributeMaxDynamicSharedMemorySize, (int)lds));
        SED_CHECK_HIP(hipFuncSetAttribute((const void*)k_gemm_batched<2>, hipFuncAttributeMaxDynamicSharedMemorySize, (int)lds));
    }
    if (gb.bf16 == 2) k_gemm_batched<2><<<grid, 256, lds, st>>>(gb);
    else if (gb.bf16) k_gemm_batched<1><<<grid, 256, lds, st>>>(gb);
    else k_gemm_batched<0><<<grid, 256, lds, st>>>(gb);
    SED_CHECK_LAUNCH();
    if (gb.splits > 1) {
        dim3 g2((maxM * maxNx + 255) / 256, gb.n_prob);
        k_gemm_reduce<<<g2, 256, 0, st>>>(gb);
        SED_CHECK_LAUNCH();
    }
    return SED_OK;
}

int launch_colsum(const float* A, int M, int N, int64_t lda, float* out, hipStream_t st) {
    k_colsum<<<(N + 63) / 64, 256, 0, st>>>(A, M, N, lda, out);
    SED_CHECK_LAUNCH();
    return SED_OK;
}
```

dcase2019_task4_amd/csrc/heads.hip:

```cpp
#include "common.h"
#include "philox.h"
#include "kernels.h"
#include "hfuse.h"

#define HD_THREADS 1024
#define HD_CONSTS(HF) constexpr int HD_F = (HF), HD_TC = ((HF) == 128 ? 128 : 32), HD_SF = (HF) + 4, HD_SB = (HF) + 16, HD_GPF = (HF) / 16; \
    (void)HD_F; (void)HD_TC; (void)HD_SF; (void)HD_SB; (void)HD_GPF
#define HD_MAXO 32
#define HD_SD 33

__device__ __forceinline__ f32x4 mfma16(float a, float b, f32x4 c) { return __builtin_amdgcn_mfma_f32_16x16x4f32(a, b, c, 0, 0, 0); }

template <int HF, int STRIDE>
__device__ __forceinline__ uint32_t heads_stage(const float* __restrict__ h, float* xs, int b, int T, int t0, int use_drop,
                                                uint64_t seed, uint32_t thr, float ks, int tid) {
    HD_CONSTS(HF);
    const int tl = tid / HD_GPF, f0 = (tid % HD_GPF) * 16, t = t0 + tl;
    float v[16];
    uint32_t keep = 0;
    if (t < T) {
        const size_t ge = (size_t)(b * T + t) * HD_F + f0;
#pragma unroll
        for (int q = 0; q < 4; ++q) {
            const float4 u = *(const float4*)(h + ge + 4 * q);
            v[4 * q] = u.x; v[4 * q + 1] = u.y; v[4 * q + 2] = u.z; v[4 * q + 3] = u.w;
        }
        keep = 0xffffu;
        if (use_drop) keep = philox_keep16(philox_stream((uint32_t)(ge >> 4), 8u, seed), thr);
    } else {
#pragma unroll
        for (int i = 0; i < 16; ++i) v[i] = 0.f;
    }
#pragma unroll
    for (int i = 0; i < 16; ++i) xs[tl * STRIDE + f0 + i] = ((keep >> i) & 1u) ? v[i] * ks : 0.f;
    return keep;
}
template <int HF, int STRIDE>
__device__ __forceinline__ void heads_stage_w(const float* __restrict__ wd, const float* __restrict__ ws, float* wsm, int NC, int tid) {
    HD_CONSTS(HF);
    constexpr int N4 = HD_MAXO * HD_F / 4, TRIPS = (N4 + HD_THREADS - 1) / HD_THREADS;
    f32x4 v[TRIPS];
#pragma unroll
    for (int i = 0; i < TRIPS; ++i) {
        const int e4 = tid + HD_THREADS * i, o = (4 * e4) / HD_F, f = (4 * e4) % HD_F;
        const int oc = o < 2 * NC ? o : 2 * NC - 1;
        const float* row = oc < NC ? wd + (size_t)oc * HD_F : ws + (size_t)(oc - NC) * HD_F;
        v[i] = *(const f32x4*)(row + (e4 < N4 ? f : 0));
    }
#pragma unroll
    for (int i = 0; i < TRIPS; ++i) {
        const int e4 = tid + HD_THREADS * i, o = (4 * e4) / HD_F, f = (4 * e4) % HD_F;
        if (e4 < N4) *(f32x4*)&wsm[o * STRIDE + f] = o < 2 * NC ? v[i] : (f32x4){0.f, 0.f, 0.f, 0.f};
    }
}

template <int HF>
__global__ __launch_bounds__(HD_THREADS) void k_heads_fwd(const float* __restrict__ h, const float* __restrict__ wd,
                                                    const float* __restrict__ bd, const float* __restrict__ ws,
                                                    const float* __restrict__ bs, float* __restrict__ strong,
                                                    float* __restrict__ weak, float* __restrict__ strong_sv,
                                                    float* __restrict__ weak_sv, float* __restrict__ logits_s,
                                                    float* __restrict__ den_out, int T, int NC, int use_drop, float p_drop,
                                                    const uint64_t* __restrict__ seed_ptr) {
    HD_CONSTS(HF);
    extern __shared__ __attribute__((aligned(16))) float hsm[];
    float* xs = hsm;
    float* wsm = xs + HD_TC * HD_SF;
    float* lg = wsm + HD_MAXO * HD_SF;
    float (*nums)[16] = (float (*)[16])(lg + HD_TC * HD_MAXO);
    float (*dens)[16] = (float (*)[16])(lg + HD_TC * HD_MAXO + HD_TC * 16);
    float* num_acc = lg + HD_TC * HD_MAXO + 2 * HD_TC * 16;
    float* den_acc = num_acc + 16;
    const int tid = threadIdx.x, b = blockIdx.x, lane = tid & 63, wv = tid >> 6;
    const uint64_t seed = use_drop ? seed_ptr[0] : 0ull;
    const uint32_t thr = drop_thresh8(p_drop);
    const float ks = use_drop ? drop_scale8(p_drop) : 1.0f;
    heads_stage_w<HF, HD_SF>(wd, ws, wsm, NC, tid);
    if (tid < 16) { num_acc[tid] = 0.f; den_acc[tid] = 0.f; }
    for (int t0 = 0; t0 < T; t0 += HD_TC) {
        __syncthreads();
        heads_stage<HF, HD_SF>(h, xs, b, T, t0, use_drop, seed, thr, ks, tid);
        __syncthreads();
        if (wv < 2 * (HD_TC / 16)) {
            const int rt = wv >> 1, ct = wv & 1, i = lane & 15, kq = lane >> 4;
            const float* A = xs + (16 * rt + i) * HD_SF + kq;
            const float* Bp = wsm + (16 * ct + i) * HD_SF + kq;
            f32x4 acc0 = {0.f, 0.f, 0.f, 0.f}, acc1 = {0.f, 0.f, 0.f, 0.f};
#pragma unroll 16
            for (int s4 = 0; s4 < HD_F / 4; s4 += 2) {
                acc0 = mfma16(A[4 * s4], Bp[4 * s4], acc0);
                acc1 = mfma16(A[4 * s4 + 4], Bp[4 * s4 + 4], acc1);
            }
            const int o = 16 * ct + i;
            const float bias = (o < NC) ? bd[o] : (o < 2 * NC ? bs[o - NC] : 0.f);
#pragma unroll
            for (int r = 0; r < 4; ++r) lg[(16 * rt + 4 * kq + r) * HD_MAXO + o] = acc0[r] + acc1[r] + bias;
        }
        __syncthreads();
        {
            const int tl = tid >> 3, sub = tid & 7, t = t0 + tl;
            auto red8_sum = [](float v) {
                v += __builtin_bit_cast(float, __builtin_amdgcn_update_dpp(0, __builtin_bit_cast(int, v), 0xB1, 0xF, 0xF, true));
                v += __builtin_bit_cast(float, __builtin_amdgcn_update_dpp(0, __builtin_bit_cast(int, v), 0x4E, 0xF, 0xF, true));
                v += __builtin_bit_cast(float, __builtin_amdgcn_update_dpp(0, __builtin_bit_cast(int, v), 0x141, 0xF, 0xF, true));
                return v;
            };
            auto red8_max = [](float v) {
                v = fmaxf(v, __builtin_bit_cast(float, __builtin_amdgcn_update_dpp(0, __builtin_bit_cast(int, v), 0xB1, 0xF, 0xF, true)));
                v = fmaxf(v, __builtin_bit_cast(float, __builtin_amdgcn_update_dpp(0, __builtin_bit_cast(int, v), 0x4E, 0xF, 0xF, true)));
                v = fmaxf(v, __builtin_bit_cast(float, __builtin_amdgcn_update_dpp(0, __builtin_bit_cast(int, v), 0x141, 0xF, 0xF, true)));
                return v;
            };
            const bool has[2] = {sub < NC, sub + 8 < NC};
            if (tl >= HD_TC) {
            } else if (t < T) {
                float ls[2], ex[2];
#pragma unroll
                for (int q = 0; q < 2; ++q) ls[q] = has[q] ? lg[tl * HD_MAXO + NC + sub + 8 * q] : -3.0e38f;
                const float mx = red8_max(fmaxf(ls[0], ls[1]));
#pragma unroll
                for (int q = 0; q < 2; ++q) ex[q] = has[q] ? __expf(ls[q] - mx) : 0.f;
                const float inv = rcp_fast(red8_sum(ex[0] + ex[1]));
#pragma unroll
                for (int q = 0; q < 2; ++q)
                    if (has[q]) {
                        const int c = sub + 8 * q;
                        const float sof = fminf(fmaxf(ex[q] * inv, 1e-7f), 1.0f);
                        const float sv = sigmoidf_fast(lg[tl * HD_MAXO + c]);
                        strong[(size_t)(b * T + t) * NC + c] = sv;
                        if (strong_sv) strong_sv[(size_t)(b * T + t) * NC + c] = sv;
                        logits_s[(size_t)(b * T + t) * NC + c] = ls[q];
                        nums[tl][c] = sv * sof;
                        dens[tl][c] = sof;
                    }
            } else {
#pragma unroll
                for (int q = 0; q < 2; ++q)
                    if (has[q]) { nums[tl][sub + 8 * q] = 0.f; dens[tl][sub + 8 * q] = 0.f; }
            }
        }
        __syncthreads();
        if (wv < NC) {
            float a = 0.f, d2 = 0.f;
#pragma unroll
            for (int tl2 = lane; tl2 < HD_TC; tl2 += 64) { a += nums[tl2][wv]; d2 += dens[tl2][wv]; }
            a = wave_sum(a); d2 = wave_sum(d2);
            if (lane == 0) { num_acc[wv] += a; den_acc[wv] += d2; }
        }
    }
    __syncthreads();
    if (tid < NC) {
        const float wk = num_acc[tid] / den_acc[tid];
        weak[b * NC + tid] = wk;
        if (weak_sv) weak_sv[b * NC + tid] = wk;
        den_out[b * NC + tid] = den_acc[tid];
    }
// ... 179 lines not shown
#pragma unroll
    for (int q = 0; q < TPW; ++q) {
        const int tile = wv * TPW + q, ot = tile / HD_GPF, ft = tile % HD_GPF, f = 16 * ft + i16;
#pragma unroll
        for (int r = 0; r < 4; ++r) {
            const int o = 16 * ot + 4 * kq + r;
            if (o < NC) pr[o * HD_F + f] = wacc[q][r];
            else if (o < NO) pr[NC * HD_F + NC + (o - NC) * HD_F + f] = wacc[q][r];
        }
    }
    if (tid < NC) pr[NC * HD_F + tid] = bacc;
    else if (tid < NO) pr[2 * NC * HD_F + NC + (tid - NC)] = bacc;
    if (!fused) return;
    __syncthreads();
    float* red = dl;
#pragma unroll
    for (int k = 0; k < 6; ++k) {
        const float v = wave_sum(lacc[k]);
        if (lane == 0) red[wv * 8 + k] = v;
    }
    __syncthreads();
    const int NP = B * NY;
    float* lpart = NY == 1 ? hl.losses + 8 : part + (size_t)NP * (2 * (NC * HD_F + NC));
    unsigned int* ticket = (unsigned int*)(hl.losses + 8 + 8 * B);
    __shared__ int is_last;
    if (tid < 6) {
        float s2 = 0.f;
        for (int w2 = 0; w2 < HD_THREADS / 64; ++w2) s2 += red[w2 * 8 + tid];
        lpart[8 * (b * NY + cy) + tid] = s2;
        __threadfence();
    }
    __syncthreads();
    if (tid == 0) is_last = (atomicAdd(ticket, 1u) == (unsigned int)(NP - 1));
    __syncthreads();
    if (!is_last) return;
    __threadfence();
    {
        float* stage = dl + 128;
        const bool staged = 8 * NP <= HD_TC * HD_SD - 128;
        if (staged)
            for (int e = tid; e < 8 * NP; e += HD_THREADS) stage[e] = __builtin_nontemporal_load(&lpart[e]);
        __syncthreads();
        if (tid < 6) {
            float s2 = 0.f;
            if (staged) for (int bb = 0; bb < NP; ++bb) s2 += stage[8 * bb + tid];
            else for (int bb = 0; bb < NP; ++bb) s2 += __builtin_nontemporal_load(&lpart[8 * bb + tid]);
            red[tid] = s2;
        }
    }
    __syncthreads();
    if (tid == 0) {
        const float wb = red[0] * inv_wb, sb = red[1] * inv_sb;
        const float cs = cw * red[2] * inv_nS, cwk = cw * red[3] * inv_nW;
        hl.losses[0] = wb + sb + cs + cwk;
        hl.losses[1] = wb; hl.losses[2] = sb; hl.losses[3] = cs; hl.losses[4] = cwk;
        hl.losses[5] = red[4] * inv_wb; hl.losses[6] = red[5] * inv_sb; hl.losses[7] = cw;
        *ticket = 0u;
        if (hl.advance) step_state_advance_early(hl.advance);
    }
}


#define LOSS_THREADS 1024
__global__ __launch_bounds__(LOSS_THREADS) void k_mt_loss(const float* __restrict__ strong, const float* __restrict__ weak,
                                                  const float* __restrict__ strong_ema, const float* __restrict__ weak_ema,
                                                  const float* __restrict__ target, int B, int T, int NC, int wlo, int whi,
                                                  int slo, int shi, const sed_step_state* __restrict__ state,
                                                  float* __restrict__ losses, float* __restrict__ d_strong,
                                                  float* __restrict__ d_weak) {
    __shared__ float red[LOSS_THREADS / 64][8];
    __shared__ float tmax[16];
    __shared__ int is_last;
    const int tid = threadIdx.x, lane = tid & 63, wv = tid >> 6, b = blockIdx.x;
    const float cw = state->cons_weight;
    float acc[6] = {0.f, 0.f, 0.f, 0.f, 0.f, 0.f};
    const float inv_nS = 1.0f / (float)(B * T * NC), inv_nW = 1.0f / (float)(B * NC);
    const float inv_sb = (shi > slo) ? 1.0f / (float)((shi - slo) * T * NC) : 0.f;
    const float inv_wb = (whi > wlo) ? 1.0f / (float)((whi - wlo) * NC) : 0.f;
    const bool in_s = (b >= slo && b < shi), in_w = (b >= wlo && b < whi);
    const size_t base = (size_t)b * T * NC;
    if (in_w && wv < NC) {
        float t = -3.0e38f;
        for (int tt = lane; tt < T; tt += 64) t = fmaxf(t, target[base + (size_t)tt * NC + wv]);
        t = wave_max(t);
        if (lane == 0) tmax[wv] = t;
    }
    for (int e = tid; e < T * NC; e += LOSS_THREADS) {
        const float p = strong[base + e], pe = strong_ema[base + e];
        const float diff = p - pe;
        acc[2] += diff * diff;
        float g = cw * 2.0f * diff * inv_nS;
        if (in_s) {
            const float t = target[base + e];
            acc[1] += bce_term(p, t);
            acc[5] += bce_term(pe, t);
            g += bce_grad(p, t) * inv_sb;
        }
        d_strong[base + e] = g;
    }
    __syncthreads();
    if (tid < NC) {
        const int e = b * NC + tid;
        const float p = weak[e], pe = weak_ema[e];
        const float diff = p - pe;
        acc[3] += diff * diff;
        float g = cw * 2.0f * diff * inv_nW;
        if (in_w) {
            const float t = tmax[tid];
            acc[0] += bce_term(p, t);
            acc[4] += bce_term(pe, t);
            g += bce_grad(p, t) * inv_wb;
        }
        d_weak[e] = g;
    }
#pragma unroll
    for (int k = 0; k < 6; ++k) {
        const float v = wave_sum(acc[k]);
        if (lane == 0) red[wv][k] = v;
    }
    __syncthreads();
    float* part = losses + 8;
    unsigned int* ticket = (unsigned int*)(losses + 8 + 8 * B);
    if (tid < 6) {
        float s2 = 0.f;
        for (int w2 = 0; w2 < LOSS_THREADS / 64; ++w2) s2 += red[w2][tid];
        part[8 * b + tid] = s2;
        __threadfence();
    }
    __syncthreads();
    if (tid == 0) is_last = (atomicAdd(ticket, 1u) == (unsigned int)(B - 1));
    __syncthreads();
    if (!is_last) return;
    __threadfence();
    if (tid < 6) {
        float s2 = 0.f;
        for (int bb = 0; bb < B; ++bb) s2 += __builtin_nontemporal_load(&part[8 * bb + tid]);
        red[0][tid] = s2;
    }
    __syncthreads();
    if (tid == 0) {
        const float* s6 = red[0];
        const float wb = s6[0] * inv_wb, sb = s6[1] * inv_sb;
        const float cs = cw * s6[2] * inv_nS, cwk = cw * s6[3] * inv_nW;
        losses[0] = wb + sb + cs + cwk;
        losses[1] = wb; losses[2] = sb; losses[3] = cs; losses[4] = cwk;
        losses[5] = s6[4] * inv_wb; losses[6] = s6[5] * inv_sb; losses[7] = cw;
        *ticket = 0u;
    }
}

__global__ __launch_bounds__(256) void k_heads_fin(const float* __restrict__ part, int B, int N, float* __restrict__ out, HeadsLoss hl,
                                                   int T, int NC) {
    __shared__ float red[4][64];
    if (blockIdx.x + 1 < gridDim.x) {
        const int c = threadIdx.x & 63, r = threadIdx.x >> 6;
        const int col = blockIdx.x * 64 + c;
        float s = 0.f;
        if (col < N)
            for (int m = r; m < B; m += 4) s += part[(int64_t)m * N + col];
        red[r][c] = s;
        __syncthreads();
        if (r == 0 && col < N) out[col] = red[0][c] + red[1][c] + red[2][c] + red[3][c];
        return;
    }
    const int tid = threadIdx.x;
    const float* lpart = hl.losses + 8;
    if (tid < 6) {
        float s2 = 0.f;
        for (int bb = 0; bb < B; ++bb) s2 += lpart[8 * bb + tid];
        red[0][tid] = s2;
    }
    __syncthreads();
    if (tid == 0) {
        const float cw = hl.state->cons_weight;
        const float inv_nS = 1.0f / (float)(B * T * NC), inv_nW = 1.0f / (float)(B * NC);
        const float inv_sb = (hl.shi > hl.slo) ? 1.0f / (float)((hl.shi - hl.slo) * T * NC) : 0.f;
        const float inv_wb = (hl.whi > hl.wlo) ? 1.0f / (float)((hl.whi - hl.wlo) * NC) : 0.f;
        const float* s6 = red[0];
        const float wb = s6[0] * inv_wb, sb = s6[1] * inv_sb;
        const float cs = cw * s6[2] * inv_nS, cwk = cw * s6[3] * inv_nW;
        hl.losses[0] = wb + sb + cs + cwk;
        hl.losses[1] = wb; hl.losses[2] = sb; hl.losses[3] = cs; hl.losses[4] = cwk;
        hl.losses[5] = s6[4] * inv_wb; hl.losses[6] = s6[5] * inv_sb; hl.losses[7] = cw;
        if (hl.advance) step_state_advance_early(hl.advance);
    }
}
int launch_heads_fin(const float* part, float* g_wd, int B, int T, int NC, int n_cols, const HeadsLoss& hl, hipStream_t st) {
    k_heads_fin<<<(n_cols + 63) / 64 + 1, 256, 0, st>>>(part, B, n_cols, g_wd, hl, T, NC);
    SED_CHECK_LAUNCH();
    return SED_OK;
}

template <int HF>
static int heads_fwd_launch(const float* h, const float* wd, const float* bd, const float* ws, const float* bs, float* strong,
                            float* weak, float* strong_sv, float* weak_sv, float* logits_s, float* den, int B, int T, int NC,
                            int use_drop, float p_drop, const uint64_t* seed, hipStream_t st) {
    HD_CONSTS(HF);
    const size_t lds = (size_t)(HD_TC * HD_SF + HD_MAXO * HD_SF + HD_TC * HD_MAXO + 2 * HD_TC * 16 + 32) * sizeof(float);
    static thread_local SedAttrOnce attr_done;
    if (attr_done.need()) {
        SED_CHECK_HIP(hipFuncSetAttribute((const void*)k_heads_fwd<HF>, hipFuncAttributeMaxDynamicSharedMemorySize, (int)lds));
    }
    k_heads_fwd<HF><<<B, HD_THREADS, lds, st>>>(h, wd, bd, ws, bs, strong, weak, strong_sv, weak_sv, logits_s, den, T, NC, use_drop,
                                                p_drop, seed);
    SED_CHECK_LAUNCH();
    return SED_OK;
}
int launch_heads_fwd(const float* h, const float* wd, const float* bd, const float* ws, const float* bs, float* strong,
                     float* weak, float* strong_sv, float* weak_sv, float* logits_s, float* den, int B, int T, int NC,
                     int use_drop, float p_drop, const uint64_t* seed, hipStream_t st, int HF) {
    if (HF == 128) return heads_fwd_launch<128>(h, wd, bd, ws, bs, strong, weak, strong_sv, weak_sv, logits_s, den, B, T, NC, use_drop, p_drop, seed, st);
    if (HF == 512) return heads_fwd_launch<512>(h, wd, bd, ws, bs, strong, weak, strong_sv, weak_sv, logits_s, den, B, T, NC, use_drop, p_drop, seed, st);
    sed_set_error("heads: unsupported feature width %d (2 x n_RNN_cell must be 128 or 512)", HF);
    return SED_ERR_UNSUPPORTED;
}

int launch_heads_colsum(const float* part, float* g_wd, int B, int NC, hipStream_t st, int HF) {
    return launch_colsum(part, B, 2 * (NC * HF + NC), 2 * (NC * HF + NC), g_wd, st);
}

template <int HF>
static int heads_bwd_launch(const float* h, const float* wd, const float* ws, const float* strong, const float* weak,
                            const float* logits_s, const float* den, const float* d_strong, const float* d_weak, float* dh,
                            float* part, int B, int T, int NC, int use_drop, float p_drop, const uint64_t* seed, double* zero,
                            int n_zero, const HeadsLoss& hl0, hipStream_t st) {
    HD_CONSTS(HF);
    const size_t lds = (size_t)(HD_TC * HD_SB + HD_MAXO * HD_SB + HD_TC * HD_SD + 32 + HD_THREADS) * sizeof(float);
    static thread_local SedAttrOnce attr_done;
    if (attr_done.need()) {
        SED_CHECK_HIP(hipFuncSetAttribute((const void*)k_heads_bwd<HF>, hipFuncAttributeMaxDynamicSharedMemorySize, (int)lds));
    }
    k_heads_bwd<HF><<<dim3(B, heads_bwd_chunks(HF, T)), HD_THREADS, lds, st>>>(h, wd, ws, strong, weak, logits_s, den, d_strong, d_weak, dh,
                                                                               part, T, NC, use_drop, p_drop, seed, zero, zero ? n_zero : 0, hl0);
    SED_CHECK_LAUNCH();
    return SED_OK;
}

int launch_heads_bwd(const float* h, const float* wd, const float* ws, const float* strong, const float* weak,
                     const float* logits_s, const float* den, const float* d_strong, const float* d_weak, float* dh,
                     float* part, float* g_wd, float* g_bd, float* g_ws, float* g_bs, int B, int T, int NC, int use_drop,
                     float p_drop, const uint64_t* seed, double* zero, int n_zero, int defer_colsum, const HeadsLoss* hl,
                     hipStream_t st, int HF) {
    (void)g_bd; (void)g_ws; (void)g_bs;
    HeadsLoss hl0 = {};
    if (hl) hl0 = *hl;
    int rc;
    if (HF == 128) rc = heads_bwd_launch<128>(h, wd, ws, strong, weak, logits_s, den, d_strong, d_weak, dh, part, B, T, NC, use_drop, p_drop, seed, zero, n_zero, hl0, st);
    else if (HF == 512) rc = heads_bwd_launch<512>(h, wd, ws, strong, weak, logits_s, den, d_strong, d_weak, dh, part, B, T, NC, use_drop, p_drop, seed, zero, n_zero, hl0, st);
    else {
        sed_set_error("heads: unsupported feature width %d (2 x n_RNN_cell must be 128 or 512)", HF);
        return SED_ERR_UNSUPPORTED;
    }
    if (rc != SED_OK || defer_colsum) return rc;
    return launch_heads_colsum(part, g_wd, B * heads_bwd_chunks(HF, T), NC, st, HF);
}

extern "C" int sed_mt_loss(const sed_dims* d, const float* strong, const float* weak, const float* strong_ema,
                           const float* weak_ema, const float* target, int weak_lo, int weak_hi, int strong_lo,
                           int strong_hi, const sed_step_state* state_dev, float* losses, float* d_strong, float* d_weak,
                           void* stream) {
    SED_CHECK_ARG(d && strong && weak && strong_ema && weak_ema && target && state_dev && losses && d_strong && d_weak,
                  "sed_mt_loss: null argument");
    SED_TRY(sed_validate_dims(d));
    const Geo g = make_geo(d);
    SED_CHECK_ARG(weak_lo >= 0 && weak_hi <= g.B && weak_lo <= weak_hi && strong_lo >= 0 && strong_hi <= g.B &&
                      strong_lo <= strong_hi, "sed_mt_loss: bad mask range");
    k_mt_loss<<<g.B, LOSS_THREADS, 0, (hipStream_t)stream>>>(strong, weak, strong_ema, weak_ema, target, g.B, g.T3, g.NC, weak_lo,
                                                  weak_hi, strong_lo, strong_hi, state_dev, losses, d_strong, d_weak);
    SED_CHECK_LAUNCH();
    return SED_OK;
}
```

dcase2019_task4_amd/csrc/kernels.h:

```cpp
#pragma once
#include "common.h"

struct ConvPackArgs;
int x_moments_parts(const Geo& g);
struct GenAuxPack;
int launch_x_moments(const Geo& g, const float* x, double* mompart, const ConvPackArgs* pack, hipStream_t st,
                     const GenAuxPack* aux = nullptr);
int launch_blk0_forward(const Geo& g, const float* x, const float* w0, const float* b0, const float* gamma,
                        const float* beta, const float* wglu, const float* bglu, float* run_mean, float* run_var,
                        int64_t* tracked, int train, int update, const uint64_t* seed, double* mom, double* mompart,
                        float* wz, float* wl, float* bn, float* p0, uint16_t* mask_out, const ConvPackArgs* pack ,
                        hipStream_t st,
                        int main_kernel_only = 0, const GenAuxPack* aux = nullptr,
                        void* p0_b16 = nullptr ,
                        int mom_ready = 0 ,
                        void* sg_out = nullptr );
int launch_blk0_backward(const Geo& g, const float* x, const float* w0, const float* b0, const float* gamma,
                         const float* beta, const float* wglu, const uint16_t* mask_in, const double* mom,
                         const float* wz, const float* wl, const float* bn, const float* dp0, double* de, int zero_de,
                         float* g_w0, float* g_b0, float* g_gamma, float* g_beta, float* g_wglu, float* g_bglu,
                         hipStream_t st, const void* sg_in = nullptr );

struct ConvPackArgs {
    const float *w1, *w2;
// ... 75 lines not shown
__device__ __forceinline__ void bn_bwd_prep_body(const BnBwdPrepArgs& a, int tid, int nthreads) {
    if (tid < 64) {
        const int c = tid;
        const double mean = a.bn[c], invstd = a.bn[64 + c];
        const double Sdz = a.acc[4160 + c], Sdzy = a.acc[4224 + c];
        a.g_beta[c] = (float)Sdz;
        a.g_gamma[c] = (float)(invstd * (Sdzy - mean * Sdz));
        float ca, cb, cc;
        bn_bwd_coef(a, c, ca, cb, cc);
        a.coef[c] = ca; a.coef[64 + c] = cb; a.coef[128 + c] = cc;
        a.g_bglu[c] = (float)a.acc[4096 + c];
        a.g_convb[c] = 0.f;
    }
    for (int e = tid; e < 4096; e += nthreads) a.g_wglu[e] = (float)a.acc[e];
}
#endif
int launch_conv_dgrad(const float* dz, const float* yin, const float* coef , const float* wpkT, float* dx,
                      int B, int H, int W, const BnBwdPrepArgs* prep, hipStream_t st);
int launch_conv_wgrad(const float* dz, const float* yin, const float* coef, const float* xin, float* part, int n_blocks,
                      float* g_w , int B, int H, int W, const BnBwdPrepArgs* prep, hipStream_t st);

int launch_glu_pool_fwd(const float* y, const double* stat, double N, const float* gamma, const float* beta, float* run_mean,
                        float* run_var, int64_t* tracked, int train, int update, float eps, float momentum, float* bn ,
                        const float* wglu, const float* bglu, float* p, int B, int H, int W, int block_id, int use_drop,
                        float p_drop, const uint64_t* seed, uint16_t* mask_out, hipStream_t st);
int launch_glu_pool_bwd(const float* y, const float* bn, const float* wglu, const float* bglu, const float* dp, const float* dp_b, float* dz,
                        double* acc, int zero_acc, int B, int H, int W, int block_id, int use_drop, float p_drop,
                        const uint16_t* mask_in, const float* gamma, float* coef, float* g_gamma, float* g_beta, float* g_wglu,
                        float* g_bglu, float* g_convb, BnBwdPrepArgs* prep_out ,
                        hipStream_t st);

struct GemmProb {
    const float* A; int64_t sAm, sAk;
    const float* B; int64_t sBk, sBn;
    const float* B2; int k2;
    float* C; int64_t ldc;
    const float* bias;
    float* Cones;
    int M, N, K;
    int accumulate;
    int vec_ok;
};
struct GemmBatch {
    GemmProb p[4];
    int n_prob;
    int splits;
    float* part;
    size_t part_floats;
    size_t part_stride;
    int bf16 = 0;
};
static inline GemmProb gemm_prob(const float* A, int64_t sAm, int64_t sAk, const float* B, int64_t sBk, int64_t sBn, float* C,
                                 int64_t ldc, int M, int N, int K) {
    GemmProb q;
    q.A = A; q.sAm = sAm; q.sAk = sAk; q.B = B; q.sBk = sBk; q.sBn = sBn; q.B2 = nullptr; q.k2 = 0;
    q.C = C; q.ldc = ldc; q.bias = nullptr; q.Cones = nullptr; q.M = M; q.N = N; q.K = K; q.accumulate = 0; q.vec_ok = 0;
    return q;
}
size_t gemm_part_floats(int n_prob, int splits, int max_m, int max_nx);
int launch_gemm_batch(GemmBatch& gb, hipStream_t st);
int launch_colsum(const float* A, int M, int N, int64_t lda, float* out, hipStream_t st);

int sed_fork_point(hipStream_t st);
int launch_gru_fwd(const float* x, int nin, const float* w_ih_f, const float* w_ih_r, const float* b_ih_f, const float* b_ih_r,
                   const float* w_hh_f, const float* w_hh_r, const float* b_hh_f, const float* b_hh_r, float* out, float* gates,
                   int B, int T, hipStream_t st);
int launch_gru_bwd(const float* d_out, const float* d_out2, const float* out, const float* gates, const float* w_hh_f,
                   const float* w_hh_r, const float* w_ih_f, const float* w_ih_r, int nin, float* dgi, float* dgh, float* hprev,
                   float* dx_planes, int B, int T, hipStream_t st);

int launch_heads_fwd(const float* h , const float* wd, const float* bd, const float* ws, const float* bs,
                     float* strong, float* weak, float* strong_sv, float* weak_sv, float* logits_s, float* den, int B, int T,
                     int NC, int use_drop, float p_drop, const uint64_t* seed, hipStream_t st, int HF = 128);
int launch_heads_colsum(const float* part, float* g_wd, int B, int NC, hipStream_t st, int HF = 128);
#ifdef __HIPCC__
__device__ __forceinline__ uint64_t splitmix64(uint64_t x) {
    x += 0x9E3779B97F4A7C15ull;
    x = (x ^ (x >> 30)) * 0xBF58476D1CE4E5B9ull;
    x = (x ^ (x >> 27)) * 0x94D049BB133111EBull;
    return x ^ (x >> 31);
}
__device__ __forceinline__ void step_state_derive_forward(sed_step_state* s) {
    const int64_t gs = s->global_step;
    double r = 1.0;
    if (gs < s->rampup_length && s->rampup_length > 0) {
        double cur = (double)gs;
        if (cur < 0) cur = 0;
        const double phase = 1.0 - cur / (double)s->rampup_length;
        r = exp(-5.0 * phase * phase);
    }
    s->cons_weight = (float)(s->max_cons_cost * r);
    s->seed_student = splitmix64(s->base_seed + 2ull * (uint64_t)gs * 0x9E3779B97F4A7C15ull + 1ull);
    s->seed_teacher = splitmix64(s->base_seed + (2ull * (uint64_t)gs + 1ull) * 0x9E3779B97F4A7C15ull + 1ull);
}
__device__ __forceinline__ void step_state_derive_update(sed_step_state* s) {
    const int64_t gs = s->global_step;
    const double a = 1.0 - 1.0 / ((double)(gs + 1) + 1.0);
    s->ema_alpha = (float)(a < s->ema_decay ? a : s->ema_decay);
    const double bc1 = 1.0 - pow(s->beta1, (double)s->opt_step);
    const double bc2 = 1.0 - pow(s->beta2, (double)s->opt_step);
    s->adam_step_size = (float)(s->lr / bc1);
    s->adam_sqrt_bc2 = (float)sqrt(bc2);
}
__device__ __forceinline__ void step_state_derive(sed_step_state* s) {
    step_state_derive_forward(s);
    step_state_derive_update(s);
}
__device__ __forceinline__ void step_state_advance_early(sed_step_state* s) {
    step_state_derive_update(s);
    s->global_step += 1;
    s->opt_step += 1;
    step_state_derive_forward(s);
}
#endif

struct HeadsLoss {
    const float* strong_ema; const float* weak_ema; const float* target;
    int wlo, whi, slo, shi;
    const sed_step_state* state;
    float* losses; float* d_strong_out; float* d_weak_out;
    sed_step_state* advance;
};
int launch_heads_bwd(const float* h, const float* wd, const float* ws, const float* strong, const float* weak,
                     const float* logits_s, const float* den, const float* d_strong, const float* d_weak, float* dh,
                     float* part, float* g_wd, float* g_bd, float* g_ws, float* g_bs, int B, int T, int NC, int use_drop,
                     float p_drop, const uint64_t* seed, double* zero, int n_zero, int defer_colsum, const HeadsLoss* hl, hipStream_t st,
                     int HF = 128);

struct HeadsFuse {
    const float* wd;
    float *strong, *weak;
    float* part;
    int NC, use_drop;
    float p_drop;
    const uint64_t* seed;
    double* zero; int n_zero;
    HeadsLoss hl;
};
static inline int heads_bwd_chunks(int HF, int T3) {
    if (HF != 512) return 1;
    const int n = (T3 + 31) / 32;
    return n < 1 ? 1 : (n > 8 ? 8 : n);
}
static inline size_t heads_part_floats(int B, int T3, int NC, int HF) {
    const int ny = heads_bwd_chunks(HF, T3);
    return (size_t)B * ny * 2 * (NC * HF + NC) + (size_t)8 * B * ny;
}
struct HeadsOut { float *strong, *weak; };
static inline bool heads_fusable(int H, int T3) { return H == 64 && T3 <= 128; }
int launch_gru_bwd_heads(const float* out, const float* gates, const float* w_hh_f, const float* w_hh_r, const float* w_ih_f,
                         const float* w_ih_r, int nin, float* dgi, float* dgh, float* hprev, float* dx_planes, int B, int T,
                         const HeadsFuse& hf, hipStream_t st);
int launch_heads_fin(const float* part, float* g_wd, int B, int T, int NC, int n_cols, const HeadsLoss& hl, hipStream_t st);
```

Before: 33540.

## Fuse GRU weight-gradient GEMM tiles and heads finalize into conv wgrad kernels

Folds the GRU weight-gradient split-K GEMM tiles for both layers into the block-2 conv weight-gradient kernel as extra workgroups, sharing its LDS. The GEMM split-K reduction and the heads dense-weight finalize are folded into the wgrad reduce kernel. This removes several separate side-stream launches and their tail latency in the backward pass. The cost is a doubled GEMM partial buffer, launch bounds relaxed to two blocks per CU, and more complex dispatch logic.

```diff
diff --git a/dcase2019_task4_amd/csrc/common.h b/dcase2019_task4_amd/csrc/common.h
--- a/dcase2019_task4_amd/csrc/common.h
+++ b/dcase2019_task4_amd/csrc/common.h
@@ -105,6 +105,9 @@
 #ifndef SED_GRU_SPLITK
 #define SED_GRU_SPLITK 16
 #endif
+#ifndef SED_GRU_GEMM_FIRST
+#define SED_GRU_GEMM_FIRST 0
+#endif
 #define SED_GLUACC_N 4296
 #define SED_WINO_OFF (9 * 4096)
 
diff --git a/dcase2019_task4_amd/csrc/conv.hip b/dcase2019_task4_amd/csrc/conv.hip
--- a/dcase2019_task4_amd/csrc/conv.hip
+++ b/dcase2019_task4_amd/csrc/conv.hip
@@ -1,6 +1,7 @@
 #include <type_traits>
 #include "common.h"
 #include "kernels.h"
+#include "gemmtile.h"
 SED_TS_DEFINE(conv)
 
 template <int TW>
@@ -1024,17 +1025,16 @@
     static constexpr int SV4 = 4 * 64 + 16, SM4 = 4 * 64, OPS4 = 4 * SV4 + 4 * SM4;
     static constexpr size_t LDS_BYTES = (size_t)(2 * WgW<4>::HALO_FLOATS + 2 * OPS4) * 4;
 };
-__global__ __launch_bounds__(512, 1) void k_wgrad4_os(const float* __restrict__ dz, const float* __restrict__ yin,
-                                                       const float* __restrict__ coef, const float* __restrict__ xin,
-                                                       float* __restrict__ part, int H, int tiles_per_clip, int n_tiles, int n_runs,
-                                                       BnBwdPrepArgs prep) {
+__device__ __forceinline__ void wgrad4_os_block(const float* __restrict__ dz, const float* __restrict__ yin,
+                                                const float* __restrict__ coef, const float* __restrict__ xin,
+                                                float* __restrict__ part, int H, int tiles_per_clip, int n_tiles, int n_runs,
+                                                const BnBwdPrepArgs& prep, int w, float* smem) {
     using C = WgW<4>;
     constexpr int SV4 = Wg4Os::SV4, SM4 = Wg4Os::SM4, OPS4 = Wg4Os::OPS4;
-    extern __shared__ __attribute__((aligned(16))) float smem[];
     float* ops = smem + 2 * C::HALO_FLOATS;
     const int tid = threadIdx.x, lane = tid & 63, wave = __builtin_amdgcn_readfirstlane(tid >> 6);
     const int cg = wave & 3, jh = wave >> 2;
-    const int w = blockIdx.x, run = (w & 7) + 8 * (w >> 5), ti = (w >> 3) & 3;
+    const int run = (w & 7) + 8 * (w >> 5), ti = (w >> 3) & 3;
     const int cg_br = cg >> 1, cg_bc = cg & 1;
     const int i16 = lane & 15, kq = lane >> 4;
     const int vp = (ti == 0) ? 0 : (ti == 2 ? 2 : 1), vq = (ti == 3) ? 3 : (ti == 2 ? 1 : 2);
@@ -1204,11 +1204,18 @@
     }
 }
 
-__global__ __launch_bounds__(256) void k_wgrad4_os_reduce(const float* __restrict__ part, int n_runs, float* __restrict__ g_w) {
-    __shared__ __attribute__((aligned(16))) float red[16][12][64];
-    __shared__ float S[12][64];
+__global__ __launch_bounds__(512, 1) void k_wgrad4_os(const float* __restrict__ dz, const float* __restrict__ yin,
+                                                       const float* __restrict__ coef, const float* __restrict__ xin,
+                                                       float* __restrict__ part, int H, int tiles_per_clip, int n_tiles, int n_runs,
+                                                       BnBwdPrepArgs prep) {
+    extern __shared__ __attribute__((aligned(16))) float smem[];
+    wgrad4_os_block(dz, yin, coef, xin, part, H, tiles_per_clip, n_tiles, n_runs, prep, blockIdx.x, smem);
+}
+
+__device__ __forceinline__ void wgrad4_os_reduce_block(const float* __restrict__ part, int n_runs, float* __restrict__ g_w, int blk,
+                                                       float (*red)[12][64], float (*S)[64]) {
     const int c = threadIdx.x & 15, grp = threadIdx.x >> 4;
-    const f32x4_t* P = (const f32x4_t*)part + blockIdx.x * 16 + c;
+    const f32x4_t* P = (const f32x4_t*)part + blk * 16 + c;
     f32x4_t s[12];
 #pragma unroll
     for (int pl = 0; pl < 12; ++pl) s[pl] = (f32x4_t){0.f, 0.f, 0.f, 0.f};
@@ -1231,8 +1238,53 @@
         const int e = o / 9, tap = o % 9, a = tap / 3, b = tap % 3;
         const float w0 = S[0 + b][e], w1 = S[3 + b][e], w2 = S[6 + b][e], w3 = S[9 + b][e];
         const float v = a == 0 ? w0 + 0.5f * (w1 + w2) : (a == 1 ? 0.5f * (w1 - w2) : 0.5f * (w1 + w2) + w3);
-        g_w[(size_t)blockIdx.x * 64 * 9 + o] = v;
-    }
+        g_w[(size_t)blk * 64 * 9 + o] = v;
+    }
+}
+__global__ __launch_bounds__(256) void k_wgrad4_os_reduce(const float* __restrict__ part, int n_runs, float* __restrict__ g_w) {
+    __shared__ __attribute__((aligned(16))) float red[16][12][64];
+    __shared__ float S[12][64];
+    wgrad4_os_reduce_block(part, n_runs, g_w, blockIdx.x, red, S);
+}
+
+static_assert(2 * (GT_M * (GT_K + 1) + GT_K * (GT_N + 1)) * 4 <= (int)Wg4Os::LDS_BYTES, "two GEMM tiles must fit in the wgrad's LDS");
+__device__ __forceinline__ void gru_wgrad_tiles(const GruWgradArgs& ga, int w, float* smem) {
+    constexpr int TILE = GT_M * (GT_K + 1) + GT_K * (GT_N + 1);
+    const int h = __builtin_amdgcn_readfirstlane(threadIdx.x >> 6) >> 2;
+    const int t = 2 * w + h, split = t / ga.tiles_per_split, e = ga.tile[t - split * ga.tiles_per_split];
+    const int l = e >> 24, pi = (e >> 16) & 255, by = (e >> 8) & 255, bx = e & 255;
+    float* As = smem + h * TILE;
+    gemm_batched_tile<0>(ga.gb[l], bx, by, pi * ga.gb[l].splits + split, threadIdx.x & 255, As, As + GT_M * (GT_K + 1));
+}
+__global__ __launch_bounds__(512, 2) void k_wgrad4_os_gru(const float* __restrict__ dz, const float* __restrict__ yin,
+                                                          const float* __restrict__ coef, const float* __restrict__ xin,
+                                                          float* __restrict__ part, int H, int tiles_per_clip, int n_tiles, int n_runs,
+                                                          BnBwdPrepArgs prep, GruWgradArgs ga) {
+    extern __shared__ __attribute__((aligned(16))) float smem[];
+    const int w = blockIdx.x, nw = 4 * n_runs;
+    if (ga.gemm_first) {
+        if (w < ga.n_gemm_wg) { gru_wgrad_tiles(ga, w, smem); return; }
+        wgrad4_os_block(dz, yin, coef, xin, part, H, tiles_per_clip, n_tiles, n_runs, prep, w - ga.n_gemm_wg, smem);
+    } else {
+        if (w >= nw) { gru_wgrad_tiles(ga, w - nw, smem); return; }
+        wgrad4_os_block(dz, yin, coef, xin, part, H, tiles_per_clip, n_tiles, n_runs, prep, w, smem);
+    }
+}
+__global__ __launch_bounds__(256) void k_wgrad4_os_reduce_gru(const float* __restrict__ part, int n_runs, float* __restrict__ g_w,
+                                                              GruWgradArgs ga) {
+    __shared__ __attribute__((aligned(16))) float red[16][12][64];
+    __shared__ float S[12][64];
+    int w = blockIdx.x;
+    if (w < 4096 / 64) { wgrad4_os_reduce_block(part, n_runs, g_w, w, red, S); return; }
+    w -= 4096 / 64;
+    if (w < ga.n_fin_wg) {
+        heads_fin_block(ga.fin_part, ga.fin_B, ga.fin_N, ga.fin_out, ga.fin_hl, ga.fin_T, ga.fin_NC, w, ga.n_fin_wg, S);
+        return;
+    }
+    w -= ga.n_fin_wg;
+    const int n0 = ga.red_wg[0] * ga.gb[0].n_prob, l = w >= n0 ? 1 : 0;
+    w -= l * n0;
+    gemm_reduce_elem(ga.gb[l], w / ga.red_wg[l], (w % ga.red_wg[l]) * 256 + threadIdx.x);
 }
 
 __global__ __launch_bounds__(256) void k_wgrad_reduce(const float* __restrict__ part, int n_blocks, float* __restrict__ g_w) {
@@ -1388,6 +1440,34 @@
     return SED_OK;
 }
 
+bool conv_wgrad4_os_default() { return !SED_AB_FLAGS(8 | 128) && !(g_sed_debug & 67108864); }
+
+int launch_conv_wgrad_gru(const float* dz, const float* yin, const float* coef, const float* xin, float* part, int n_blocks,
+                          float* g_w, int B, int H, const BnBwdPrepArgs* prep, GruWgradArgs& ga, hipStream_t st) {
+    SED_CHECK_ARG(conv_wgrad4_os_default(), "conv wgrad + GRU: the block-2 wgrad must be k_wgrad4_os (debug bits 3, 7, 26 are off)");
+    SED_CHECK_ARG(ga.n_batch >= 1 && ga.n_batch <= 2 && ga.tiles_per_split > 0 && ga.tiles_per_split <= SED_GRU_TILES_MAX &&
+                      (ga.tiles_per_split & 1) == 0 && 2 * ga.n_gemm_wg == ga.gb[0].splits * ga.tiles_per_split,
+                  "conv wgrad + GRU: bad GEMM tiling");
+    for (int l = 0; l < ga.n_batch; ++l) SED_CHECK_ARG(ga.gb[l].splits == ga.gb[0].splits, "conv wgrad + GRU: batches split K alike");
+    BnBwdPrepArgs pa = {};
+    if (prep) pa = *prep;
+    using CW = WgW<4>;
+    static thread_local SedAttrOnce attro;
+    if (attro.need()) {
+        SED_CHECK_HIP(hipFuncSetAttribute((const void*)k_wgrad4_os_gru, hipFuncAttributeMaxDynamicSharedMemorySize, (int)Wg4Os::LDS_BYTES));
+    }
+    SED_CHECK_ARG((size_t)B * H * 4 * 64 < ((size_t)1 << 31), "wgrad: image too large for 32-bit offsets");
+    const int tpcw = (H + CW::TH - 1) / CW::TH, ntw = B * tpcw;
+    int n_runs = (ntw + 7) & ~7;
+    if (n_runs > WG4_RUNS) n_runs = WG4_RUNS;
+    SED_CHECK_ARG(n_runs * 4 <= n_blocks * 3, "wgrad: partial buffer too small");
+    k_wgrad4_os_gru<<<4 * n_runs + ga.n_gemm_wg, 512, Wg4Os::LDS_BYTES, st>>>(dz, yin, coef, xin, part, H, tpcw, ntw, n_runs, pa, ga);
+    SED_CHECK_LAUNCH();
+    k_wgrad4_os_reduce_gru<<<4096 / 64 + ga.n_fin_wg + ga.n_red_wg, 256, 0, st>>>(part, n_runs, g_w, ga);
+    SED_CHECK_LAUNCH();
+    return SED_OK;
+}
+
 int launch_conv_wgrad(const float* dz, const float* yin, const float* coef, const float* xin, float* part, int n_blocks,
                       float* g_w, int B, int H, int W, const BnBwdPrepArgs* prep, hipStream_t st) {
     SED_CHECK_ARG(!(prep && W == 16 && SED_AB_FLAGS(8 | 128)), "conv wgrad: in-kernel BatchNorm-backward coefficients need the default kernels");
diff --git a/dcase2019_task4_amd/csrc/crnn.hip b/dcase2019_task4_amd/csrc/crnn.hip
--- a/dcase2019_task4_amd/csrc/crnn.hip
+++ b/dcase2019_task4_amd/csrc/crnn.hip
@@ -7,6 +7,7 @@
 #include "common.h"
 #include "kernels.h"
 #include "gkernels.h"
+#include "gemmtile.h"
 
 static thread_local char g_err[512] = "";
 void sed_set_error(const char* fmt, ...) {
@@ -115,7 +116,7 @@
     W.gluacc1 = W.bwd_acc; W.gluacc2 = W.bwd_acc + SED_GLUACC_N * sizeof(double); W.de0 = W.bwd_acc + 2 * SED_GLUACC_N * sizeof(double);
     W.wgrad_blocks = SED_WGRAD_MAX_BLOCKS;
     put(W.wg_part, (size_t)W.wgrad_blocks * 9 * 4096 * 4);
-    put(W.gemm_part, gemm_part_floats(4, SED_GRU_SPLITK, 192, 129) * 4);
+    put(W.gemm_part, 2 * gemm_part_floats(4, SED_GRU_SPLITK, 192, 129) * 4);
     W.total = o;
     return W;
 }
@@ -386,11 +387,11 @@
     const bool defer_gru_w = (parts & 4) != 0;
     bool forked = false, forked2 = false;
 
-    auto gru_weight_grads_layer = [&](int l, hipStream_t s2) -> int {
+    auto gru_weight_grads_batch = [&](int l, float* part) -> GemmBatch {
         const int nin = (l == 0) ? 64 : 128;
         const float* input = (l == 0) ? CTXF(L.p2) : CTXF(L.out[l - 1]);
         GemmBatch gb;
-        gb.n_prob = 4; gb.splits = SED_GRU_SPLITK; gb.part = WSF(W.gemm_part); gb.part_floats = gemm_part_floats(4, SED_GRU_SPLITK, 192, 129); gb.part_stride = 0;
+        gb.n_prob = 4; gb.splits = SED_GRU_SPLITK; gb.part = part; gb.part_floats = gemm_part_floats(4, SED_GRU_SPLITK, 192, 129); gb.part_stride = 0;
         for (int dir = 0; dir < 2; ++dir) {
             gb.p[2 * dir] = gemm_prob(WSF(W.dgi[l]) + dir * 192, 1, 384, input, nin, 1, grads + P.w_ih[l][dir], nin, 192, nin, BT);
             gb.p[2 * dir].Cones = grads + P.b_ih[l][dir];
@@ -398,6 +399,10 @@
                                           grads + P.w_hh[l][dir], 64, 192, 64, BT);
             gb.p[2 * dir + 1].Cones = grads + P.b_hh[l][dir];
         }
+        return gb;
+    };
+    auto gru_weight_grads_layer = [&](int l, hipStream_t s2) -> int {
+        GemmBatch gb = gru_weight_grads_batch(l, WSF(W.gemm_part));
         return launch_gemm_batch(gb, s2);
     };
     auto gru_weight_grads = [&](hipStream_t s2) -> int {
@@ -475,6 +480,34 @@
 #else
     const bool fuse_prep = (g_sed_debug & 512) == 0;
 #endif
+    const bool side_fused = parts == 3 && sd.ok && !early_gru_w && !(g_sed_debug & (2048 | 33554432)) && conv_wgrad4_os_default();
+    auto gru_wgrad_args = [&](GruWgradArgs& ga) -> int {
+        ga.n_batch = g.L;
+        ga.tiles_per_split = 0;
+        for (int l = 0; l < g.L; ++l) {
+            ga.gb[l] = gru_weight_grads_batch(l, WSF(W.gemm_part) + (size_t)l * gemm_part_floats(4, SED_GRU_SPLITK, 192, 129));
+            GemmBatch& gb = ga.gb[l];
+            SED_TRY(gemm_batch_prepare(gb));
+            for (int pi = 0; pi < gb.n_prob; ++pi) {
+                const GemmProb& q = gb.p[pi];
+                for (int by = 0; by < (q.M + GT_M - 1) / GT_M; ++by)
+                    for (int bx = 0; bx < (q.N + GT_N - 1) / GT_N; ++bx) {
+                        SED_CHECK_ARG(ga.tiles_per_split < SED_GRU_TILES_MAX, "GRU weight gradients: too many GEMM tiles");
+                        ga.tile[ga.tiles_per_split++] = (l << 24) | (pi << 16) | (by << 8) | bx;
+                    }
+            }
+            ga.red_wg[l] = (int)((gb.part_stride + 255) / 256);
+            ga.n_red_wg += ga.red_wg[l] * gb.n_prob;
+        }
+        ga.n_gemm_wg = SED_GRU_SPLITK * ga.tiles_per_split / 2;
+        ga.gemm_first = SED_GRU_GEMM_FIRST;
+        if (fuse) {
+            ga.fin_part = WSF(W.heads_part); ga.fin_out = grads + P.dense_w; ga.fin_B = g.B; ga.fin_N = head_cols;
+            ga.fin_T = g.T3; ga.fin_NC = g.NC; ga.fin_hl = *hl;
+            ga.n_fin_wg = (head_cols + 63) / 64 + 1;
+        }
+        return SED_OK;
+    };
     BnBwdPrepArgs prep[3] = {};
     for (int i = 2; i >= 1; --i) {
         const BnBwdPrepArgs* pp = fuse_prep ? &prep[i] : nullptr;
@@ -487,9 +520,17 @@
             if (sd.ok) SED_CHECK_HIP(hipEventRecord(sd.fork, st));
             SED_TRY(launch_conv_dgrad(WSF(dzo[i]), CTXF(yo[i]), WSF(W.coef[i]), CTXF(wpkT[i]), WSF(dpo[i - 1]), g.B, Hs[i], Wd[i], pp, st));
             if (sd.ok) { SED_CHECK_HIP(hipStreamWaitEvent(sd.s, sd.fork, 0)); forked = true; }
+            if (side_fused) {
+                if (!fuse) SED_TRY(heads_colsum(ss));
+                GruWgradArgs ga{};
+                SED_TRY(gru_wgrad_args(ga));
+                SED_TRY(launch_conv_wgrad_gru(WSF(dzo[i]), CTXF(yo[i]), WSF(W.coef[i]), CTXF(pin[i]), WSF(W.wg_part), W.wgrad_blocks,
+                                              grads + P.conv_w[i], g.B, Hs[i], pp, ga, ss));
+            } else {
             SED_TRY(launch_conv_wgrad(WSF(dzo[i]), CTXF(yo[i]), WSF(W.coef[i]), CTXF(pin[i]), WSF(W.wg_part), W.wgrad_blocks,
                                       grads + P.conv_w[i], g.B, Hs[i], Wd[i], pp, ss));
-            if (parts == 3 && !early_gru_w) {
+            }
+            if (parts == 3 && !early_gru_w && !side_fused) {
                 hipStream_t sg = ss;
                 if (sd.ok && (g_sed_debug & 2048)) {
                     SED_CHECK_HIP(hipStreamWaitEvent(sd.s2, sd.fork, 0));
diff --git a/dcase2019_task4_amd/csrc/gemm.hip b/dcase2019_task4_amd/csrc/gemm.hip
--- a/dcase2019_task4_amd/csrc/gemm.hip
+++ b/dcase2019_task4_amd/csrc/gemm.hip
@@ -1,19 +1,11 @@
 #include "common.h"
 #include "kernels.h"
+#include "gemmtile.h"
 SED_TS_DEFINE(gemm)
-
-#define GT_M 64
-#define GT_N 64
-#define GT_K 64
-
-typedef __attribute__((ext_vector_type(8))) __bf16 gemm_bf16x8;
-__device__ __forceinline__ int prob_nx(const GemmProb& p) { return p.N + (p.Cones ? 1 : 0); }
 
 template <int BF>
 __global__ __launch_bounds__(256) void k_gemm_batched(GemmBatch gb) {
     extern __shared__ __attribute__((aligned(16))) float gsm[];
-    float* As = gsm;
-    float* Bs = gsm + GT_M * (GT_K + 1);
     int bx = blockIdx.x, by = blockIdx.y, bz = blockIdx.z;
 #ifndef SED_NO_XCD_ORDER
     {
@@ -24,166 +16,7 @@
         }
     }
 #endif
-    const int pi = bz / gb.splits, split = bz % gb.splits;
-    const GemmProb& d = gb.p[pi];
-    const int Nx = prob_nx(d);
-    const int m0 = by * GT_M, n0 = bx * GT_N;
-    if (m0 >= d.M || n0 >= d.N) return;
-    const int tid = threadIdx.x, lane = tid & 63, wv = tid >> 6;
-    const int n = lane & 31, kh = lane >> 5;
-    const int wm = wv >> 1, wn = wv & 1;
-    const bool ones_here = d.Cones != nullptr && bx == 0;
-    float rowsum = 0.f;
-    int kbeg = 0, kend = d.K;
-    if (gb.splits > 1) {
-        const int chunk = ((d.K + gb.splits - 1) / gb.splits + GT_K - 1) / GT_K * GT_K;
-        kbeg = split * chunk;
-        kend = min(d.K, kbeg + chunk);
-    }
-    f32x16 acc;
-#pragma unroll
-    for (int r = 0; r < 16; ++r) acc[r] = 0.f;
-    constexpr int NG = (GT_M * GT_K) / 256 / 4;
-    int am[NG], ak[NG], bk[NG], bn[NG];
-    const bool a_kc = (d.sAk == 1), b_nc = (d.sBn == 1);
-#pragma unroll
-    for (int it = 0; it < NG; ++it) {
-        const int e4 = (tid + 256 * it) * 4;
-        if (a_kc) { am[it] = e4 / GT_K; ak[it] = e4 % GT_K; } else { am[it] = e4 % GT_M; ak[it] = e4 / GT_M; }
-        if (b_nc) { bk[it] = e4 / GT_N; bn[it] = e4 % GT_N; } else { bk[it] = e4 % GT_K; bn[it] = e4 / GT_K; }
-    }
-    float ra[NG][4], rb[NG][4];
-    const bool interior = d.vec_ok && m0 + GT_M <= d.M && n0 + GT_N <= d.N;
-    (void)Nx;
-    auto load_tile = [&](int k0) {
-        if (interior && k0 + GT_K <= kend && (d.B2 == nullptr || k0 >= d.k2 || k0 + GT_K <= d.k2)) {
-            const float* bbase = (d.B2 != nullptr && k0 >= d.k2) ? d.B2 - (int64_t)d.k2 * d.sBk : d.B;
-#pragma unroll
-            for (int it = 0; it < NG; ++it) {
-                const f32x4 va = *(const f32x4*)(d.A + (int64_t)(m0 + am[it]) * d.sAm + (int64_t)(k0 + ak[it]) * d.sAk);
-                const f32x4 vb = *(const f32x4*)(bbase + (int64_t)(k0 + bk[it]) * d.sBk + (int64_t)(n0 + bn[it]) * d.sBn);
-#pragma unroll
-                for (int q = 0; q < 4; ++q) { ra[it][q] = va[q]; rb[it][q] = vb[q]; }
-            }
-            return;
-        }
-#pragma unroll
-        for (int it = 0; it < NG; ++it) {
-            {
-                const int m = m0 + am[it], k = k0 + ak[it];
-                const float* p = d.A + (int64_t)m * d.sAm + (int64_t)k * d.sAk;
-                const bool full = a_kc ? (m < d.M && k + 3 < kend) : (m + 3 < d.M && k < kend);
-                if (full && (((uintptr_t)p & 15) == 0)) {
-                    const float4 v = *(const float4*)p;
-                    ra[it][0] = v.x; ra[it][1] = v.y; ra[it][2] = v.z; ra[it][3] = v.w;
-                } else {
-#pragma unroll
-                    for (int q = 0; q < 4; ++q) {
-                        const int mm = a_kc ? m : m + q, kk = a_kc ? k + q : k;
-                        ra[it][q] = (mm < d.M && kk < kend) ? d.A[(int64_t)mm * d.sAm + (int64_t)kk * d.sAk] : 0.f;
-                    }
-                }
-            }
-            {
-                const int kk0 = k0 + bk[it], nn0 = n0 + bn[it];
-                const bool two = d.B2 != nullptr;
-                const float* base = (two && kk0 >= d.k2) ? d.B2 - (int64_t)d.k2 * d.sBk : d.B;
-                const float* p = base + (int64_t)kk0 * d.sBk + (int64_t)nn0 * d.sBn;
-                const bool same_src = !two || b_nc || (kk0 >= d.k2) == (kk0 + 3 >= d.k2);
-                const bool full = same_src && (b_nc ? (kk0 < kend && nn0 + 3 < d.N) : (kk0 + 3 < kend && nn0 < d.N));
-                if (full && (((uintptr_t)p & 15) == 0)) {
-                    const float4 v = *(const float4*)p;
-                    rb[it][0] = v.x; rb[it][1] = v.y; rb[it][2] = v.z; rb[it][3] = v.w;
-                } else {
-#pragma unroll
-                    for (int q = 0; q < 4; ++q) {
-                        const int kk = b_nc ? kk0 : kk0 + q, nn = b_nc ? nn0 + q : nn0;
-                        float w = 0.f;
-                        if (kk < kend) {
-                            if (nn < d.N) {
-                                w = (two && kk >= d.k2) ? d.B2[(int64_t)(kk - d.k2) * d.sBk + (int64_t)nn * d.sBn]
-                                                        : d.B[(int64_t)kk * d.sBk + (int64_t)nn * d.sBn];
-                            }
-                        }
-                        rb[it][q] = w;
-                    }
-                }
-            }
-        }
-    };
-    if (kbeg < kend) load_tile(kbeg);
-    for (int k0 = kbeg; k0 < kend; k0 += GT_K) {
-#pragma unroll
-        for (int it = 0; it < NG; ++it)
-#pragma unroll
-            for (int q = 0; q < 4; ++q) {
-                As[(a_kc ? am[it] : am[it] + q) * (GT_K + 1) + (a_kc ? ak[it] + q : ak[it])] = ra[it][q];
-                Bs[(b_nc ? bk[it] : bk[it] + q) * (GT_N + 1) + (b_nc ? bn[it] + q : bn[it])] = rb[it][q];
-            }
-        lds_barrier();
-        if (k0 + GT_K < kend) load_tile(k0 + GT_K);
-        if (ones_here) {
-            const float* ar = As + (tid >> 2) * (GT_K + 1) + 16 * (tid & 3);
-#pragma unroll
-            for (int kk = 0; kk < 16; ++kk) rowsum += ar[kk];
-        }
-        if constexpr (BF != 0) {
-#pragma unroll
-            for (int s = 0; s < GT_K / 16; ++s) {
-                gemm_bf16x8 a, b, al, bl;
-#pragma unroll
-                for (int e = 0; e < 8; ++e) {
-                    const float av = As[(32 * wm + n) * (GT_K + 1) + 16 * s + 8 * kh + e];
-                    const float bv = Bs[(16 * s + 8 * kh + e) * (GT_N + 1) + 32 * wn + n];
-                    a[e] = (__bf16)av;
-                    b[e] = (__bf16)bv;
-                    if constexpr (BF == 2) { al[e] = (__bf16)(av - (float)a[e]); bl[e] = (__bf16)(bv - (float)b[e]); }
-                }
-                acc = __builtin_amdgcn_mfma_f32_32x32x16_bf16(a, b, acc, 0, 0, 0);
-                if constexpr (BF == 2) {
-                    acc = __builtin_amdgcn_mfma_f32_32x32x16_bf16(a, bl, acc, 0, 0, 0);
-                    acc = __builtin_amdgcn_mfma_f32_32x32x16_bf16(al, b, acc, 0, 0, 0);
-                }
-            }
-        } else {
-#pragma unroll
-            for (int s = 0; s < GT_K / 2; ++s) {
-                const float a = As[(32 * wm + n) * (GT_K + 1) + 2 * s + kh];
-                const float b = Bs[(2 * s + kh) * (GT_N + 1) + 32 * wn + n];
-                acc = mfma32(a, b, acc);
-            }
-        }
-        lds_barrier();
-    }
-    if (ones_here) {
-        rowsum += __shfl_xor(rowsum, 1);
-        rowsum += __shfl_xor(rowsum, 2);
-        const int row = m0 + (tid >> 2);
-        if ((tid & 3) == 0 && row < d.M) {
-            if (gb.splits > 1) gb.part[(size_t)bz * gb.part_stride + (size_t)row * Nx + d.N] = rowsum;
-            else d.Cones[row] = rowsum;
-        }
-    }
-    const int col = n0 + 32 * wn + n;
-    if (col >= d.N) return;
-    if (gb.splits > 1) {
-        float* P = gb.part + ((size_t)bz * gb.part_stride);
-#pragma unroll
-        for (int r = 0; r < 16; ++r) {
-            const int row = m0 + 32 * wm + mfma32_row(r, lane);
-            if (row < d.M) P[(size_t)row * Nx + col] = acc[r];
-        }
-        return;
-    }
-#pragma unroll
-    for (int r = 0; r < 16; ++r) {
-        const int row = m0 + 32 * wm + mfma32_row(r, lane);
-        if (row >= d.M) continue;
-        float* c = d.C + (int64_t)row * d.ldc + col;
-        float v = acc[r] + (d.bias ? d.bias[col] : 0.f);
-        if (d.accumulate) v += *c;
-        *c = v;
-    }
+    gemm_batched_tile<BF>(gb, bx, by, bz, threadIdx.x, gsm, gsm + GT_M * (GT_K + 1));
 }
 
 #define GP_M 32
@@ -288,31 +121,7 @@
 }
 
 __global__ __launch_bounds__(256) void k_gemm_reduce(GemmBatch gb) {
-    const int pi = blockIdx.y;
-    const GemmProb& d = gb.p[pi];
-    const int Nx = prob_nx(d);
-    const int i = blockIdx.x * blockDim.x + threadIdx.x;
-    if (i >= d.M * Nx) return;
-    const float* P = gb.part + (size_t)pi * gb.splits * gb.part_stride + i;
-    float s0 = 0.f, s1 = 0.f, s2 = 0.f, s3 = 0.f;
-    int z = 0;
-    for (; z + 4 <= gb.splits; z += 4) {
-        s0 += P[(size_t)(z + 0) * gb.part_stride];
-        s1 += P[(size_t)(z + 1) * gb.part_stride];
-        s2 += P[(size_t)(z + 2) * gb.part_stride];
-        s3 += P[(size_t)(z + 3) * gb.part_stride];
-    }
-    for (; z < gb.splits; ++z) s0 += P[(size_t)z * gb.part_stride];
-    float v = (s0 + s1) + (s2 + s3);
-    const int row = i / Nx, col = i % Nx;
-    if (col < d.N) {
-        float* c = d.C + (int64_t)row * d.ldc + col;
-        v += d.bias ? d.bias[col] : 0.f;
-        if (d.accumulate) v += *c;
-        *c = v;
-    } else {
-        d.Cones[row] = v;
-    }
+    gemm_reduce_elem(gb, blockIdx.y, blockIdx.x * blockDim.x + threadIdx.x);
 }
 
 __global__ __launch_bounds__(256) void k_colsum(const float* __restrict__ A, int M, int N, int64_t lda, float* __restrict__ out) {
@@ -331,13 +140,40 @@
     return (size_t)n_prob * splits * max_m * max_nx;
 }
 
-int launch_gemm_batch(GemmBatch& gb, hipStream_t st) {
-    int maxM = 0, maxNx = 0;
+static void gemm_batch_dims(const GemmBatch& gb, int& maxM, int& maxNx) {
+    maxM = 0; maxNx = 0;
     for (int i = 0; i < gb.n_prob; ++i) {
         const int nx = gb.p[i].N + (gb.p[i].Cones ? 1 : 0);
         maxM = gb.p[i].M > maxM ? gb.p[i].M : maxM;
         maxNx = nx > maxNx ? nx : maxNx;
     }
+}
+
+int gemm_batch_prepare(GemmBatch& gb) {
+    int maxM, maxNx;
+    gemm_batch_dims(gb, maxM, maxNx);
+    for (int i = 0; i < gb.n_prob; ++i) {
+        GemmProb& q = gb.p[i];
+        const bool a_kc = (q.sAk == 1), b_nc = (q.sBn == 1);
+        q.vec_ok = (a_kc ? (q.sAm % 4) == 0 : (q.sAm == 1 && (q.sAk % 4) == 0)) &&
+                   (b_nc ? (q.sBk % 4) == 0 : (q.sBk == 1 && (q.sBn % 4) == 0)) &&
+                   ((uintptr_t)q.A % 16) == 0 && ((uintptr_t)q.B % 16) == 0 && (q.B2 == nullptr || ((uintptr_t)q.B2 % 16) == 0);
+    }
+    if (gb.splits > 1) {
+        SED_CHECK_ARG(gb.part != nullptr, "split-K gemm needs a partial buffer");
+        gb.part_stride = (size_t)maxM * maxNx;
+        if ((size_t)gb.n_prob * gb.splits * gb.part_stride > gb.part_floats) {
+            sed_set_error("split-K gemm: partial buffer holds %zu floats, the batch needs %zu", gb.part_floats,
+                          (size_t)gb.n_prob * gb.splits * gb.part_stride);
+            return SED_ERR_WORKSPACE;
+        }
+    }
+    return SED_OK;
+}
+
+int launch_gemm_batch(GemmBatch& gb, hipStream_t st) {
+    int maxM, maxNx;
+    gemm_batch_dims(gb, maxM, maxNx);
     if (gb.splits < 1) gb.splits = 1;
     bool panel = (gb.splits == 1) && !gb.bf16;
     int maxK = 0, maxN = 0;
@@ -364,22 +200,7 @@
         SED_CHECK_LAUNCH();
         return SED_OK;
     }
-    for (int i = 0; i < gb.n_prob; ++i) {
-        GemmProb& q = gb.p[i];
-        const bool a_kc = (q.sAk == 1), b_nc = (q.sBn == 1);
-        q.vec_ok = (a_kc ? (q.sAm % 4) == 0 : (q.sAm == 1 && (q.sAk % 4) == 0)) &&
-                   (b_nc ? (q.sBk % 4) == 0 : (q.sBk == 1 && (q.sBn % 4) == 0)) &&
-                   ((uintptr_t)q.A % 16) == 0 && ((uintptr_t)q.B % 16) == 0 && (q.B2 == nullptr || ((uintptr_t)q.B2 % 16) == 0);
-    }
-    if (gb.splits > 1) {
-        SED_CHECK_ARG(gb.part != nullptr, "split-K gemm needs a partial buffer");
-        gb.part_stride = (size_t)maxM * maxNx;
-        if ((size_t)gb.n_prob * gb.splits * gb.part_stride > gb.part_floats) {
-            sed_set_error("split-K gemm: partial buffer holds %zu floats, the batch needs %zu", gb.part_floats,
-                          (size_t)gb.n_prob * gb.splits * gb.part_stride);
-            return SED_ERR_WORKSPACE;
-        }
-    }
+    SED_TRY(gemm_batch_prepare(gb));
     dim3 grid((maxN + GT_N - 1) / GT_N, (maxM + GT_M - 1) / GT_M, gb.n_prob * gb.splits);
     const size_t lds = (size_t)(GT_M * (GT_K + 1) + GT_K * (GT_N + 1)) * sizeof(float);
     static thread_local SedAttrOnce attr_done;
diff --git a/dcase2019_task4_amd/csrc/gemmtile.h b/dcase2019_task4_amd/csrc/gemmtile.h
--- /dev/null
+++ b/dcase2019_task4_amd/csrc/gemmtile.h
@@ -0,0 +1,237 @@
+#pragma once
+#include "common.h"
+#include "kernels.h"
+
+#define GT_M 64
+#define GT_N 64
+#define GT_K 64
+
+typedef __attribute__((ext_vector_type(8))) __bf16 gemm_bf16x8;
+__device__ __forceinline__ int prob_nx(const GemmProb& p) { return p.N + (p.Cones ? 1 : 0); }
+
+
+template <int BF>
+__device__ __forceinline__ void gemm_batched_tile(const GemmBatch& gb, int bx, int by, int bz, int tid, float* As, float* Bs) {
+    const int pi = bz / gb.splits, split = bz % gb.splits;
+    const GemmProb& d = gb.p[pi];
+    const int Nx = prob_nx(d);
+    const int m0 = by * GT_M, n0 = bx * GT_N;
+    if (m0 >= d.M || n0 >= d.N) return;
+    const int lane = tid & 63, wv = tid >> 6;
+    const int n = lane & 31, kh = lane >> 5;
+    const int wm = wv >> 1, wn = wv & 1;
+    const bool ones_here = d.Cones != nullptr && bx == 0;
+    float rowsum = 0.f;
+    int kbeg = 0, kend = d.K;
+    if (gb.splits > 1) {
+        const int chunk = ((d.K + gb.splits - 1) / gb.splits + GT_K - 1) / GT_K * GT_K;
+        kbeg = split * chunk;
+        kend = min(d.K, kbeg + chunk);
+    }
+    f32x16 acc;
+#pragma unroll
+    for (int r = 0; r < 16; ++r) acc[r] = 0.f;
+    constexpr int NG = (GT_M * GT_K) / 256 / 4;
+    int am[NG], ak[NG], bk[NG], bn[NG];
+    const bool a_kc = (d.sAk == 1), b_nc = (d.sBn == 1);
+#pragma unroll
+    for (int it = 0; it < NG; ++it) {
+        const int e4 = (tid + 256 * it) * 4;
+        if (a_kc) { am[it] = e4 / GT_K; ak[it] = e4 % GT_K; } else { am[it] = e4 % GT_M; ak[it] = e4 / GT_M; }
+        if (b_nc) { bk[it] = e4 / GT_N; bn[it] = e4 % GT_N; } else { bk[it] = e4 % GT_K; bn[it] = e4 / GT_K; }
+    }
+    float ra[NG][4], rb[NG][4];
+    const bool interior = d.vec_ok && m0 + GT_M <= d.M && n0 + GT_N <= d.N;
+    (void)Nx;
+    auto load_tile = [&](int k0) {
+        if (interior && k0 + GT_K <= kend && (d.B2 == nullptr || k0 >= d.k2 || k0 + GT_K <= d.k2)) {
+            const float* bbase = (d.B2 != nullptr && k0 >= d.k2) ? d.B2 - (int64_t)d.k2 * d.sBk : d.B;
+#pragma unroll
+            for (int it = 0; it < NG; ++it) {
+                const f32x4 va = *(const f32x4*)(d.A + (int64_t)(m0 + am[it]) * d.sAm + (int64_t)(k0 + ak[it]) * d.sAk);
+                const f32x4 vb = *(const f32x4*)(bbase + (int64_t)(k0 + bk[it]) * d.sBk + (int64_t)(n0 + bn[it]) * d.sBn);
+#pragma unroll
+                for (int q = 0; q < 4; ++q) { ra[it][q] = va[q]; rb[it][q] = vb[q]; }
+            }
+            return;
+        }
+#pragma unroll
+        for (int it = 0; it < NG; ++it) {
+            {
+                const int m = m0 + am[it], k = k0 + ak[it];
+                const float* p = d.A + (int64_t)m * d.sAm + (int64_t)k * d.sAk;
+                const bool full = a_kc ? (m < d.M && k + 3 < kend) : (m + 3 < d.M && k < kend);
+                if (full && (((uintptr_t)p & 15) == 0)) {
+                    const float4 v = *(const float4*)p;
+                    ra[it][0] = v.x; ra[it][1] = v.y; ra[it][2] = v.z; ra[it][3] = v.w;
+                } else {
+#pragma unroll
+                    for (int q = 0; q < 4; ++q) {
+                        const int mm = a_kc ? m : m + q, kk = a_kc ? k + q : k;
+                        ra[it][q] = (mm < d.M && kk < kend) ? d.A[(int64_t)mm * d.sAm + (int64_t)kk * d.sAk] : 0.f;
+                    }
+                }
+            }
+            {
+                const int kk0 = k0 + bk[it], nn0 = n0 + bn[it];
+                const bool two = d.B2 != nullptr;
+                const float* base = (two && kk0 >= d.k2) ? d.B2 - (int64_t)d.k2 * d.sBk : d.B;
+                const float* p = base + (int64_t)kk0 * d.sBk + (int64_t)nn0 * d.sBn;
+                const bool same_src = !two || b_nc || (kk0 >= d.k2) == (kk0 + 3 >= d.k2);
+                const bool full = same_src && (b_nc ? (kk0 < kend && nn0 + 3 < d.N) : (kk0 + 3 < kend && nn0 < d.N));
+                if (full && (((uintptr_t)p & 15) == 0)) {
+                    const float4 v = *(const float4*)p;
+                    rb[it][0] = v.x; rb[it][1] = v.y; rb[it][2] = v.z; rb[it][3] = v.w;
+                } else {
+#pragma unroll
+                    for (int q = 0; q < 4; ++q) {
+                        const int kk = b_nc ? kk0 : kk0 + q, nn = b_nc ? nn0 + q : nn0;
+                        float w = 0.f;
+                        if (kk < kend) {
+                            if (nn < d.N) {
+                                w = (two && kk >= d.k2) ? d.B2[(int64_t)(kk - d.k2) * d.sBk + (int64_t)nn * d.sBn]
+                                                        : d.B[(int64_t)kk * d.sBk + (int64_t)nn * d.sBn];
+                            }
+                        }
+                        rb[it][q] = w;
+                    }
+                }
+            }
+        }
+    };
+    if (kbeg < kend) load_tile(kbeg);
+    for (int k0 = kbeg; k0 < kend; k0 += GT_K) {
+#pragma unroll
+        for (int it = 0; it < NG; ++it)
+#pragma unroll
+            for (int q = 0; q < 4; ++q) {
+                As[(a_kc ? am[it] : am[it] + q) * (GT_K + 1) + (a_kc ? ak[it] + q : ak[it])] = ra[it][q];
+                Bs[(b_nc ? bk[it] : bk[it] + q) * (GT_N + 1) + (b_nc ? bn[it] + q : bn[it])] = rb[it][q];
+            }
+        lds_barrier();
+        if (k0 + GT_K < kend) load_tile(k0 + GT_K);
+        if (ones_here) {
+            const float* ar = As + (tid >> 2) * (GT_K + 1) + 16 * (tid & 3);
+#pragma unroll
+            for (int kk = 0; kk < 16; ++kk) rowsum += ar[kk];
+        }
+        if constexpr (BF != 0) {
+#pragma unroll
+            for (int s = 0; s < GT_K / 16; ++s) {
+                gemm_bf16x8 a, b, al, bl;
+#pragma unroll
+                for (int e = 0; e < 8; ++e) {
+                    const float av = As[(32 * wm + n) * (GT_K + 1) + 16 * s + 8 * kh + e];
+                    const float bv = Bs[(16 * s + 8 * kh + e) * (GT_N + 1) + 32 * wn + n];
+                    a[e] = (__bf16)av;
+                    b[e] = (__bf16)bv;
+                    if constexpr (BF == 2) { al[e] = (__bf16)(av - (float)a[e]); bl[e] = (__bf16)(bv - (float)b[e]); }
+                }
+                acc = __builtin_amdgcn_mfma_f32_32x32x16_bf16(a, b, acc, 0, 0, 0);
+                if constexpr (BF == 2) {
+                    acc = __builtin_amdgcn_mfma_f32_32x32x16_bf16(a, bl, acc, 0, 0, 0);
+                    acc = __builtin_amdgcn_mfma_f32_32x32x16_bf16(al, b, acc, 0, 0, 0);
+                }
+            }
+        } else {
+#pragma unroll
+            for (int s = 0; s < GT_K / 2; ++s) {
+                const float a = As[(32 * wm + n) * (GT_K + 1) + 2 * s + kh];
+                const float b = Bs[(2 * s + kh) * (GT_N + 1) + 32 * wn + n];
+                acc = mfma32(a, b, acc);
+            }
+        }
+        lds_barrier();
+    }
+    if (ones_here) {
+        rowsum += __shfl_xor(rowsum, 1);
+        rowsum += __shfl_xor(rowsum, 2);
+        const int row = m0 + (tid >> 2);
+        if ((tid & 3) == 0 && row < d.M) {
+            if (gb.splits > 1) gb.part[(size_t)bz * gb.part_stride + (size_t)row * Nx + d.N] = rowsum;
+            else d.Cones[row] = rowsum;
+        }
+    }
+    const int col = n0 + 32 * wn + n;
+    if (col >= d.N) return;
+    if (gb.splits > 1) {
+        float* P = gb.part + ((size_t)bz * gb.part_stride);
+#pragma unroll
+        for (int r = 0; r < 16; ++r) {
+            const int row = m0 + 32 * wm + mfma32_row(r, lane);
+            if (row < d.M) P[(size_t)row * Nx + col] = acc[r];
+        }
+        return;
+    }
+#pragma unroll
+    for (int r = 0; r < 16; ++r) {
+        const int row = m0 + 32 * wm + mfma32_row(r, lane);
+        if (row >= d.M) continue;
+        float* c = d.C + (int64_t)row * d.ldc + col;
+        float v = acc[r] + (d.bias ? d.bias[col] : 0.f);
+        if (d.accumulate) v += *c;
+        *c = v;
+    }
+}
+
+__device__ __forceinline__ void gemm_reduce_elem(const GemmBatch& gb, int pi, int i) {
+    const GemmProb& d = gb.p[pi];
+    const int Nx = prob_nx(d);
+    if (i >= d.M * Nx) return;
+    const float* P = gb.part + (size_t)pi * gb.splits * gb.part_stride + i;
+    float s0 = 0.f, s1 = 0.f, s2 = 0.f, s3 = 0.f;
+    int z = 0;
+    for (; z + 4 <= gb.splits; z += 4) {
+        s0 += P[(size_t)(z + 0) * gb.part_stride];
+        s1 += P[(size_t)(z + 1) * gb.part_stride];
+        s2 += P[(size_t)(z + 2) * gb.part_stride];
+        s3 += P[(size_t)(z + 3) * gb.part_stride];
+    }
+    for (; z < gb.splits; ++z) s0 += P[(size_t)z * gb.part_stride];
+    float v = (s0 + s1) + (s2 + s3);
+    const int row = i / Nx, col = i % Nx;
+    if (col < d.N) {
+        float* c = d.C + (int64_t)row * d.ldc + col;
+        v += d.bias ? d.bias[col] : 0.f;
+        if (d.accumulate) v += *c;
+        *c = v;
+    } else {
+        d.Cones[row] = v;
+    }
+}
+
+__device__ __forceinline__ void heads_fin_block(const float* __restrict__ part, int B, int N, float* __restrict__ out,
+                                                const HeadsLoss& hl, int T, int NC, int blk, int nblk, float (*red)[64]) {
+    if (blk + 1 < nblk) {
+        const int c = threadIdx.x & 63, r = threadIdx.x >> 6;
+        const int col = blk * 64 + c;
+        float s = 0.f;
+        if (col < N)
+            for (int m = r; m < B; m += 4) s += part[(int64_t)m * N + col];
+        red[r][c] = s;
+        __syncthreads();
+        if (r == 0 && col < N) out[col] = red[0][c] + red[1][c] + red[2][c] + red[3][c];
+        return;
+    }
+    const int tid = threadIdx.x;
+    const float* lpart = hl.losses + 8;
+    if (tid < 6) {
+        float s2 = 0.f;
+        for (int bb = 0; bb < B; ++bb) s2 += lpart[8 * bb + tid];
+        red[0][tid] = s2;
+    }
+    __syncthreads();
+    if (tid == 0) {
+        const float cw = hl.state->cons_weight;
+        const float inv_nS = 1.0f / (float)(B * T * NC), inv_nW = 1.0f / (float)(B * NC);
+        const float inv_sb = (hl.shi > hl.slo) ? 1.0f / (float)((hl.shi - hl.slo) * T * NC) : 0.f;
+        const float inv_wb = (hl.whi > hl.wlo) ? 1.0f / (float)((hl.whi - hl.wlo) * NC) : 0.f;
+        const float* s6 = red[0];
+        const float wb = s6[0] * inv_wb, sb = s6[1] * inv_sb;
+        const float cs = cw * s6[2] * inv_nS, cwk = cw * s6[3] * inv_nW;
+        hl.losses[0] = wb + sb + cs + cwk;
+        hl.losses[1] = wb; hl.losses[2] = sb; hl.losses[3] = cs; hl.losses[4] = cwk;
+        hl.losses[5] = s6[4] * inv_wb; hl.losses[6] = s6[5] * inv_sb; hl.losses[7] = cw;
+        if (hl.advance) step_state_advance_early(hl.advance);
+    }
+}
diff --git a/dcase2019_task4_amd/csrc/heads.hip b/dcase2019_task4_amd/csrc/heads.hip
--- a/dcase2019_task4_amd/csrc/heads.hip
+++ b/dcase2019_task4_amd/csrc/heads.hip
@@ -2,6 +2,7 @@
 #include "philox.h"
 #include "kernels.h"
 #include "hfuse.h"
+#include "gemmtile.h"
 
 #define HD_THREADS 1024
 #define HD_CONSTS(HF) constexpr int HD_F = (HF), HD_TC = ((HF) == 128 ? 128 : 32), HD_SF = (HF) + 4, HD_SB = (HF) + 16, HD_GPF = (HF) / 16; \
@@ -487,38 +488,7 @@
 __global__ __launch_bounds__(256) void k_heads_fin(const float* __restrict__ part, int B, int N, float* __restrict__ out, HeadsLoss hl,
                                                    int T, int NC) {
     __shared__ float red[4][64];
-    if (blockIdx.x + 1 < gridDim.x) {
-        const int c = threadIdx.x & 63, r = threadIdx.x >> 6;
-        const int col = blockIdx.x * 64 + c;
-        float s = 0.f;
-        if (col < N)
-            for (int m = r; m < B; m += 4) s += part[(int64_t)m * N + col];
-        red[r][c] = s;
-        __syncthreads();
-        if (r == 0 && col < N) out[col] = red[0][c] + red[1][c] + red[2][c] + red[3][c];
-        return;
-    }
-    const int tid = threadIdx.x;
-    const float* lpart = hl.losses + 8;
-    if (tid < 6) {
-        float s2 = 0.f;
-        for (int bb = 0; bb < B; ++bb) s2 += lpart[8 * bb + tid];
-        red[0][tid] = s2;
-    }
-    __syncthreads();
-    if (tid == 0) {
-        const float cw = hl.state->cons_weight;
-        const float inv_nS = 1.0f / (float)(B * T * NC), inv_nW = 1.0f / (float)(B * NC);
-        const float inv_sb = (hl.shi > hl.slo) ? 1.0f / (float)((hl.shi - hl.slo) * T * NC) : 0.f;
-        const float inv_wb = (hl.whi > hl.wlo) ? 1.0f / (float)((hl.whi - hl.wlo) * NC) : 0.f;
-        const float* s6 = red[0];
-        const float wb = s6[0] * inv_wb, sb = s6[1] * inv_sb;
-        const float cs = cw * s6[2] * inv_nS, cwk = cw * s6[3] * inv_nW;
-        hl.losses[0] = wb + sb + cs + cwk;
-        hl.losses[1] = wb; hl.losses[2] = sb; hl.losses[3] = cs; hl.losses[4] = cwk;
-        hl.losses[5] = s6[4] * inv_wb; hl.losses[6] = s6[5] * inv_sb; hl.losses[7] = cw;
-        if (hl.advance) step_state_advance_early(hl.advance);
-    }
+    heads_fin_block(part, B, N, out, hl, T, NC, blockIdx.x, gridDim.x, red);
 }
 int launch_heads_fin(const float* part, float* g_wd, int B, int T, int NC, int n_cols, const HeadsLoss& hl, hipStream_t st) {
     k_heads_fin<<<(n_cols + 63) / 64 + 1, 256, 0, st>>>(part, B, n_cols, g_wd, hl, T, NC);
diff --git a/dcase2019_task4_amd/csrc/kernels.h b/dcase2019_task4_amd/csrc/kernels.h
--- a/dcase2019_task4_amd/csrc/kernels.h
+++ b/dcase2019_task4_amd/csrc/kernels.h
@@ -251,3 +251,22 @@
                          const float* w_ih_r, int nin, float* dgi, float* dgh, float* hprev, float* dx_planes, int B, int T,
                          const HeadsFuse& hf, hipStream_t st);
 int launch_heads_fin(const float* part, float* g_wd, int B, int T, int NC, int n_cols, const HeadsLoss& hl, hipStream_t st);
+
+#define SED_GRU_TILES_MAX 48
+struct GruWgradArgs {
+    GemmBatch gb[2];
+    int n_batch;
+    int tiles_per_split;
+    int tile[SED_GRU_TILES_MAX];
+    int n_gemm_wg;
+    int gemm_first;
+    int red_wg[2];
+    int n_red_wg;
+    const float* fin_part; float* fin_out; int fin_B, fin_N, fin_T, fin_NC;
+    int n_fin_wg;
+    HeadsLoss fin_hl;
+};
+int gemm_batch_prepare(GemmBatch& gb);
+bool conv_wgrad4_os_default();
+int launch_conv_wgrad_gru(const float* dz, const float* yin, const float* coef, const float* xin, float* part, int n_blocks,
+                          float* g_w, int B, int H, const BnBwdPrepArgs* prep, GruWgradArgs& ga, hipStream_t st);
```

After: 33590 (median of 6 runs). About the same (+0.1%).
